# tjhladish/AbcSmc

Hardware: AMD Instinct MI355X
Metric: particles/sec per SMC generation (PLS+weight+resample), 1/2/4/8 GPU (higher is better)
Workload: dtype f64 (inputs, model, distances, proposals, results; pair sums of the weight stage: fp64 operands as three f16 limbs on the matrix pipe + f32 v_exp_f32, weights <= 5e-7 rel of the fp64 oracle, largest seen 3.1e-7); 1 GPU; configs[2]: synthetic 1M particles x 16 params x 32 metrics, PLS 8 components, full generation; particles_per_gpu=1000000, particles_total=1000000, metrics=32, params=16, pls_components=8, pred_prior_size=100000, prev_pred_prior_size=100000, next_set_size=1000000, noise=MULTIVARIATE, ncomp_chosen=8, pls_component_rule=wilcoxon, parallelism=row-sharded x1, launcher=single GPU

## Files before the change

### abcsmc_amd/csrc/abc_internal.h

```cpp
#pragma once
#include <hip/hip_runtime.h>
#include <stddef.h>
#include <stdint.h>
#include <stdio.h>
#include <stdlib.h>
#include <string.h>

#include "../../include/abcsmc_hip.h"

#define ABC_WAVE 64

inline const char* abc_diag_env(const char* name) {
    static const bool on = [] { const char* d = getenv("ABC_DIAG"); return d && d[0] == '1'; }();
    return on ? getenv(name) : nullptr;
}

struct abc_wx_words {
    int left;
    int vmax_lo, vmax_hi;
    int ncomp;
    int changed;
    int decided;
    int n_rest;
    int n_level;
// ... 192 lines not shown
                            double* stats, size_t n_set = 0);
int launch_pls_model(abc_ctx*, const double* stats, const double* obs, size_t M, size_t P, size_t A,
                     int rule, double* model, hipEvent_t done = nullptr);
int launch_simple_model(abc_ctx*, const double* stats, const double* obs, size_t M, size_t P,
                        double* model);
int launch_project_distance(abc_ctx*, const double* X, size_t n, size_t ldx, size_t M, size_t P,
                            size_t A, const double* model, int simple, double* dist);
size_t launch_project_scores(abc_ctx*, const double* X, size_t n, size_t ldx, size_t M, size_t P, size_t A, const double* model, double* S);
int launch_project_distance_scores(abc_ctx*, const double* X, size_t n, size_t ldx, size_t M, size_t P, size_t A, const double* model,
                                   double* dist, double* S, size_t sld, size_t row_test, hipEvent_t done);
int launch_distance_from_scores(abc_ctx*, const double* S, size_t n, size_t sld, size_t M, size_t P, size_t A, const double* model, double* dist);
size_t abc_targets_need(size_t N, size_t A, size_t B, size_t K, bool any_excl);
struct abc_tg_scores { const double* S; size_t sld; const double* O; int KCO; };
int launch_rank_targets(abc_ctx*, const double* X, size_t ldx, const double* Y, size_t ldy, size_t N, size_t M, size_t P,
                        const double* model, size_t A, const double* targets, size_t ldt, size_t B, const uint64_t* exclude,
                        bool any_excl, size_t K, uint64_t* idx, double* dist, double* post_mean, abc_tg_scores* keep = nullptr);
size_t abc_adjust_need(size_t N, size_t A, size_t P, size_t B, size_t K);
int launch_rank_targets_adjust(abc_ctx*, const double* X, size_t ldx, const double* Y, size_t ldy, size_t N, size_t M, size_t P,
                               const double* model, size_t A, const double* targets, size_t ldt, size_t B, const uint64_t* exclude,
                               bool any_excl, size_t K, int kernel, uint64_t* idx, double* dist, const abc_adjust_out* out,
                               struct abc_adj_keep* keep = nullptr);
size_t abc_path_need(size_t N, size_t A, size_t P, size_t B, size_t K, size_t T);
int launch_rank_targets_path(abc_ctx*, const double* X, size_t ldx, const double* Y, size_t ldy, size_t N, size_t M, size_t P,
                             const double* model, size_t A, const double* targets, size_t ldt, size_t B, const uint64_t* exclude,
                             bool any_excl, int kernel, uint64_t* idx, double* dist, const abc_path* path);
struct SmValues {
    int method;
    const uint64_t* idx;
    const double* Y;
    size_t ldy;
    const struct abc_adj_keep* adj;
    int A;
    int kernel;
    const double* V;
    size_t ldv;
    const double* w;
};
size_t abc_summary_need(size_t B, size_t K, size_t P);
int launch_summary(abc_ctx*, const SmValues& sv, size_t B, size_t K, size_t P, const abc_summary* sum);
int abc_summary_check_weights(abc_ctx*, const double* w, size_t K, const char* fn);
size_t abc_density_need(size_t B, size_t K, size_t P, size_t G);
int launch_density(abc_ctx*, const SmValues& sv, size_t B, size_t K, size_t P, const abc_density* dn, const char* fn);
struct DnSeg;
size_t abc_density_segs_need(size_t B, size_t K, size_t P);
int launch_density_segs(abc_ctx*, const SmValues& sv, size_t B, size_t K, size_t P, const abc_density* dn, const DnSeg** segs,
                        const char* fn);
size_t abc_joint_pairs(const abc_joint* jt, size_t P);
size_t abc_joint_need(size_t B, size_t K, size_t P, size_t G, size_t npairs);
int launch_joint(abc_ctx*, const SmValues& sv, size_t B, size_t K, size_t P, const abc_joint* jt, const char* fn);
size_t abc_draws_need(size_t B, size_t K, size_t P, int smooth);
int launch_draws(abc_ctx*, const SmValues& sv, size_t B, size_t K, size_t P, const abc_draws* dr, const char* fn);
int launch_select_smallest(abc_ctx*, const double* dist, size_t n, size_t K, uint64_t idx_base,
                           uint64_t* idx, double* dist_out, bool defer_check = false);
int abc_select_check(abc_ctx* ctx, int* failed);
int abc_select_check_queue(abc_ctx* ctx, int* slot);
int abc_select_check_done(abc_ctx* ctx, const int* slot);
inline size_t abc_kde_slices(size_t kn, size_t Kp, int PP) {
    if (kn == 0 || Kp == 0) return 1;
    size_t rows_per_slice = 24576 / (size_t)PP;
    if (rows_per_slice < 256) rows_per_slice = 256;
    size_t s = (Kp + rows_per_slice - 1) / rows_per_slice;
    const size_t rb = (kn + 255) / 256;
    if (s * rb < 4096) s = (4096 + rb - 1) / rb;
    size_t cap = ((size_t)64 << 20) / (8 * kn);
    if (cap < 8) cap = 8;
    if (s > cap) s = cap;
    if (s > Kp / 64) s = Kp / 64;
    if (s < 1) s = 1;
    if (s > 1024) s = 1024;
    return s;
}
int launch_merge_runs(abc_ctx* ctx, const double* key, const uint64_t* idx, int W, size_t len, double* okey, uint64_t* oidx,
                      uint64_t* osrc = nullptr);
int launch_sort_pairs(abc_ctx*, double* key, uint64_t* idx, size_t n);
int launch_select_begin(abc_ctx*, uint64_t K, long long* state, int* hist);
int launch_select_hist(abc_ctx*, const double* dist, size_t n, const long long* state, int pass, int* hist);
int launch_select_pick(abc_ctx*, long long* state, int pass, int* hist, uint64_t K);
int launch_select_count(abc_ctx*, const double* dist, size_t n, const long long* state, long long* counts);
int launch_select_compact(abc_ctx*, const double* dist, size_t n, const long long* state, uint64_t n_less,
                          uint64_t ties_take, uint64_t idx_base, uint64_t* idx_out, double* dist_out);
int abc_sort_u64_bytes(abc_ctx*, unsigned long long* key0, unsigned long long* val0, unsigned long long* key1,
                       unsigned long long* val1, size_t n, int byte_lo, int byte_hi);
struct abc_wx_shard {
    size_t nv_total;
    const double* nv_ranks;
    size_t nv_stride;
};
bool abc_wx_cascade_applies(size_t nv_total, size_t P, size_t A);
int launch_wilcoxon(abc_ctx*, const double* X, const double* Y, size_t n, size_t ldx, size_t ldy, size_t M, size_t P,
                    size_t A, size_t row_test, double* model, const abc_wx_shard* sh = nullptr, double* dec = nullptr,
                    int* changed_host = nullptr, int stop_at_max = 0);
int launch_wilcoxon_commit(abc_ctx*, double* model, size_t M, size_t P, size_t A, const double* dec, int with_hdr);
struct abc_wx_run;
struct abc_wx_scores_hook { int (*fn)(void* arg, double** S, size_t* sld); void* arg; };
int launch_wilcoxon_begin(abc_ctx*, const double* X, const double* Y, size_t n, size_t ldx, size_t ldy, size_t M, size_t P, size_t A,
                          size_t row_test, double* model, double* dec, int stop_at_max, abc_wx_run** out,
                          const abc_wx_scores_hook* scores = nullptr, int hold_level0 = 0, const abc_wx_shard* sh = nullptr);
int launch_wilcoxon_level0(abc_ctx*, abc_wx_run* run);
int launch_wilcoxon_finish(abc_ctx*, abc_wx_run* run, int* changed_host);
void launch_wilcoxon_abandon(abc_ctx*, abc_wx_run* run, hipStream_t its_stream);
int abc_comm_all_reduce(abc_ctx* ctx, void* buf, size_t count, int dtype);
int abc_comm_all_gather(abc_ctx* ctx, const void* send, void* recv, size_t bytes);
int abc_xbuf_reserve(abc_ctx* ctx, size_t bytes);
int abc_giveups_ensure(abc_ctx* ctx);
int launch_gather_rows(abc_ctx*, const double* Y, size_t n_local, size_t ldy, size_t P,
                       const uint64_t* idx, size_t K, uint64_t idx_base, double* theta, size_t ldt,
                       const int* sel_fail = nullptr, int* sel_fail_pin = nullptr, hipEvent_t done = nullptr);
#define ABC_INTERNAL_RETRY (-2147483647)
int launch_doubled_variance(abc_ctx*, const double* theta, size_t K, size_t P, double* dv);
int launch_theta_stats(abc_ctx*, const double* theta, size_t K, size_t P, double** stats_out);
struct abc_theta_fused {
    double* dv; double* L; int* spd; double* rows ; double* Lpad ;
    const double* model_hdr; double* hdr_pin; int* spd_pin;
};
int launch_post_tail(abc_ctx*, const double* theta, size_t K, size_t P, const double* stats, const abc_theta_fused* f);
int launch_dv_from_stats(abc_ctx*, const double* stats, size_t P, double* dv);
int launch_mvn_from_stats(abc_ctx*, const double* stats, size_t P, double* L, int* status_dev);
struct abc_wprev {
    void* wc ; double* b; double* hb; unsigned short* bt; unsigned* far_list;
    unsigned* tmin;
    size_t Kp, P, kn_max; int split, ready;
};
int launch_weights_prev(abc_ctx*, size_t P, size_t kn_max, const double* theta_prev, size_t Kp, const double* w_prev,
                        const double* dv_prev, abc_wprev* out, hipStream_t st);
int launch_weights_raw(abc_ctx*, const abc_prior* priors, const double* theta, size_t K, size_t P,
                       size_t k0, size_t kn, const double* theta_prev, size_t Kp,
                       const double* w_prev, const double* dv_prev, double* w_raw, const abc_wprev* prev = nullptr,
                       const double** sumsq_out = nullptr);
int abc_weights_prev_early(abc_ctx* ctx, size_t P, size_t kn_max, const double* theta_prev, size_t Kp, const double* w_prev,
                           const double* dv_prev, abc_wprev* out);
int launch_fill(abc_ctx*, double* w, size_t K, double v, hipStream_t st = nullptr);
int launch_normalize_l2(abc_ctx*, double* w, size_t K, double* host_mirror = nullptr, const double* sumsq_parts = nullptr);
static inline size_t abc_alias_pin_bytes(size_t K) { return K * (sizeof(double) * 3 + sizeof(uint32_t) * 3) + 2 * sizeof(uint32_t) + 16; }
int launch_mvn_setup(abc_ctx*, const double* theta, size_t K, size_t P, double* L, int* status_host,
                     int* status_dev);
int launch_resample(abc_ctx*, const abc_rng* rng, const double* w, size_t K, uint64_t i0, size_t n,
                    uint64_t* parent, int (*while_host_builds)(void*) = nullptr, void* hook_arg = nullptr,
                    bool uniform_weights = false, const uint32_t* raw_ready = nullptr, bool weights_on_host = false,
                    const volatile int* abort_flag = nullptr, bool parents_ready = false, int* alias_check_deferred = nullptr);
int abc_rng_streams_early(abc_ctx* ctx, const abc_rng* rng, uint64_t i0, size_t n, uint64_t* seeds, uint64_t seed_stream_offset,
                          uint32_t** raw, uint64_t* parent_uniform = nullptr, size_t K_uniform = 0);
int abc_rng_seeds_early(abc_ctx* ctx, const abc_rng* rng, uint64_t i0, size_t n, uint64_t* seeds, uint64_t seed_stream_offset);
int abc_side_fork(abc_ctx* ctx);
int abc_uniform_alias(abc_ctx* ctx, size_t K);
struct abc_perturb_prep { double* rows; int seeds_done; double* Lpad; };
int launch_perturb_prepare(abc_ctx*, const abc_rng* rng, const double* theta, size_t K, size_t P, uint64_t i0, size_t n,
                           uint64_t* seeds, uint64_t seed_stream_offset, abc_perturb_prep* prep, int multivariate = 0,
                           const double* L_or_dv = nullptr);
static inline int abc_perturb_pp(size_t P) {
    int PP = 2;
    while (PP < (int)P) PP *= 2;
    return (P > 64) ? (int)((P + 63) / 64 * 64) : PP;
}
int launch_perturb(abc_ctx*, const abc_rng* rng, const double* theta, size_t K, size_t P,
                   const abc_prior* priors, const uint64_t* parent, uint64_t i0, size_t n,
                   int multivariate, const double* L_or_dv, double* out, uint64_t* seeds,
                   uint64_t seed_stream_offset, const abc_perturb_prep* prep = nullptr);

struct abc_side_moments { abc_theta_fused out; double* stats; double* L; };
int abc_moments_on_side(abc_ctx* ctx, const double* theta, size_t K, size_t P, bool multivariate, double* L_io, double* dv,
                        int* spd_dev, const double* model_hdr, bool theta_ev_bound, const char* who, abc_side_moments* m);
int abc_normalize_for_resample(abc_ctx* ctx, double* w, size_t K, size_t Nn, const double* sumsq, bool* w_on_host);
struct abc_prep_arg {
    abc_ctx* ctx; const abc_rng* rng; const double* theta; const double* theta_stats; size_t K, P, Nn;
    uint64_t i0, seed_off; uint64_t* seeds; abc_perturb_prep* prep; double* L; int* spd_dev; double* dv; bool moments;
    const double* model_hdr; double* hdr_pin; int* spd_pin;
};
int abc_prep_hook(void* prep_arg);
int abc_alias_repair(abc_ctx* ctx, const abc_rng* rng_entry, const double* w, size_t K, uint64_t i0, size_t Nn, uint64_t seed_off,
                     uint64_t* parent, const double* theta, size_t P, const abc_prior* priors, int multivariate, const double* L_or_dv,
                     double* next, abc_perturb_prep* prep, bool giveups_to_snapshot);

int launch_perturb_reference(abc_ctx*, abc_rng* rng_after_draws, const double* theta, size_t K, size_t P, const abc_prior* priors,
                             const uint64_t* parent, size_t n, int multivariate, const double* L_or_dv, double* out,
                             uint64_t* seeds);

void abc_alias_preproc(size_t K, const double* w, double* F, uint32_t* A, double* E, uint32_t* smalls, uint32_t* bigs, bool knuth = true);

int launch_alias_build_dev(abc_ctx*, const double* w, size_t K, double* F, uint32_t* A, int* fail_dev, int* fail_pin,
                           const int** verdict_src = nullptr);
size_t abc_alias_dev_need(size_t K);
constexpr size_t ABC_ALIAS_DEV_MAX_K = (size_t)2 << 20;
constexpr size_t ABC_ALIAS_DEV_MIN_K = 20000;
constexpr size_t ABC_ALIAS_DEV_SMALL_K = 300000;

size_t abc_ws_need(size_t N, size_t M, size_t P, size_t A, size_t K, size_t Kp, size_t Nnext);
size_t abc_wx_need(size_t n_validation, size_t P, size_t A);
int abc_timing_flush(abc_ctx* ctx);
void abc_comm_release(abc_ctx* ctx);

void taus2_set(abc_rng* r, unsigned long seed);
uint32_t taus2_get(abc_rng* r);
void taus2_jump(abc_rng* r, uint64_t n);
```

### abcsmc_amd/csrc/alias_dev.hip

```cpp
#include <stdlib.h>

#include "abc_internal.h"

namespace {

typedef __int128 i128;
typedef unsigned __int128 u128;
typedef unsigned long long u64;

#ifndef ABC_AL_I
#define ABC_AL_I 4
#endif
#define ABC_AL_CAT2(a, b) a##b
#define ABC_AL_CAT(a, b) ABC_AL_CAT2(a, b)
#define ABC_AL_FN(name) ABC_AL_CAT(name##_i, ABC_AL_I)
constexpr int AL_T = 256;
constexpr int AL_I = ABC_AL_I;
constexpr int AL_B = AL_T * AL_I;
constexpr int AL_MAXBLK = 8192;
constexpr int AL_SUM_BITS = 44;

struct RMap { i128 t0, t1, b; int k; int pad_[3]; };

__device__ __forceinline__ i128 shl(i128 v, int s) { return (i128)((u128)v << s); }
// ... 65 lines not shown
    const int t = threadIdx.x, lane = t & 63, wave = t >> 6;
    RMap inc = mine;
#pragma unroll
    for (int d = 1; d < 64; d <<= 1) {
        const RMap up = shfl_up_map(inc, d);
        if (lane >= d) inc = compose(up, inc);
    }
    RMap exw = shfl_up_map(inc, 1);
    if (lane == 0) exw = rmap_identity();
    if (lane == 63) buf[0][wave] = inc;
    __syncthreads();
    RMap before = rmap_identity();
    for (int w = 0; w < wave; w++) before = compose(before, buf[0][w]);
    __syncthreads();
    *excl = compose(before, exw);
    return compose(before, inc);
}
__device__ __forceinline__ RMap prefix_of_blocks(const RMap* __restrict__ agg, int nb, RMap (*buf)[AL_T]) {
    const int t = threadIdx.x;
    const int per = (nb + AL_T - 1) / AL_T;
    RMap m = rmap_identity();
    for (int j = 0; j < per; j++) { const int b = t * per + j; if (b < nb) m = compose(m, agg[b]); }
    RMap ex;
    (void)block_scan_maps(m, buf, &ex);
    __shared__ RMap s_tot;
    if (t == AL_T - 1) s_tot = compose(ex, m);
    __syncthreads();
    const RMap r = s_tot;
    __syncthreads();
    return r;
}

struct AlHead {
    double approx_total;
    double total;
    int e0_sum;
    int e0;
    unsigned ns, nb;
    unsigned nsteps;
    int fail;
    i128 MEAN;
};

__device__ __forceinline__ void al_fail(AlHead* h) { h->fail = 1; }

__device__ __forceinline__ double block_sum_d(double v, double* sm) {
#pragma unroll
    for (int o = 32; o >= 1; o >>= 1) v += __shfl_xor(v, o, 64);
    __syncthreads();
    if ((threadIdx.x & 63) == 0) sm[threadIdx.x >> 6] = v;
    __syncthreads();
    return (sm[0] + sm[1]) + (sm[2] + sm[3]);
}
__global__ __launch_bounds__(AL_T) void k_al_bsum(const double* __restrict__ w, size_t K, double* __restrict__ bsum, AlHead* __restrict__ head,
                                                  int force_fail) {
    __shared__ double sm[4];
    const size_t base = (size_t)blockIdx.x * AL_B + (size_t)threadIdx.x * AL_I;
    double s = 0.0;
    bool bad = false;
#pragma unroll
    for (int j = 0; j < AL_I; j++) if (base + j < K) { const double x = w[base + j]; s += x; bad = bad || !(x >= 0.0) || !(x < 1.0e300); }
    const double bs = block_sum_d(bad ? (double)NAN : s, sm);
    if (threadIdx.x == 0) bsum[blockIdx.x] = bs;
    if (blockIdx.x == 0 && threadIdx.x == 0) {
        head->approx_total = 0.0; head->total = 0.0; head->e0_sum = 0; head->e0 = 0; head->ns = 0; head->nb = 0; head->nsteps = 0;
        head->fail = force_fail; head->MEAN = 0;
    }
}

__device__ __forceinline__ void approx_prefix(const double* __restrict__ bsum, int nblk, int b, double* sm, double* before, double* all) {
    double pb = 0.0, pa = 0.0;
    for (int j = threadIdx.x; j < nblk; j += AL_T) { const double v = bsum[j]; pa += v; if (j < b) pb += v; }
    *before = block_sum_d(pb, sm);
    *all = block_sum_d(pa, sm);
}

struct SumCtx { double before, all; int e0; };
__device__ __forceinline__ RMap sum_map(double x, double s_approx, int e0, AlHead* head) {
    if (x == 0.0) return rmap_identity();
    int ex;
    (void)frexp(s_approx, &ex);
    int k = ex - e0 - 53;
    if (k < 0) k = 0;
    bool sticky = false;
    const i128 c = to_grid(x, e0, &sticky);
    if (k == 0 && sticky) al_fail(head);
    return rne_map(k, c, sticky);
}
__device__ __forceinline__ double block_excl_prefix_d(double mine, double* sd ) {
    const int t = threadIdx.x;
    sd[t] = mine;
    __syncthreads();
    for (int step = 1; step < AL_T; step <<= 1) {
        const double a = (t >= step) ? sd[t - step] : 0.0;
        __syncthreads();
        sd[t] += a;
        __syncthreads();
    }
    const double ex = t ? sd[t - 1] : 0.0;
    __syncthreads();
    return ex;
}

__global__ __launch_bounds__(AL_T) void k_al_sum_reduce(const double* __restrict__ w, size_t K, const double* __restrict__ bsum, int nblk,
                                                        RMap* __restrict__ agg, RMap* __restrict__ tpre, AlHead* __restrict__ head) {
    __shared__ RMap buf[2][AL_T];
    __shared__ double sd[AL_T];
    __shared__ double sm[4];
    double before, all;
    approx_prefix(bsum, nblk, blockIdx.x, sm, &before, &all);
    int etot;
    (void)frexp(all, &etot);
    const int e0 = etot - 53 - AL_SUM_BITS;
    if (!(all > 0.0) || !(all < 1.0e300)) { if (threadIdx.x == 0) al_fail(head); }
// ... 310 lines not shown
    const RMap ex = tpre[(size_t)blockIdx.x * AL_T + threadIdx.x];
    const int e0 = head->e0;
    i128 v = rapply(ex, rapply(pre, a.VI[0]));
    bool ok = true;
    double prev = from_grid(v, e0, &ok);
#pragma unroll
    for (int j = 0; j < AL_I; j++) {
        const size_t t = base + j;
        if (t >= n) break;
        v = rapply(mj[j], v);
        const double c = from_grid(v, e0, &ok);
        const uint32_t s = rec[j].idx;
        unsigned jcur;
        bool below, at_last_small;
        if (!(s & AL_HAND)) {
            const unsigned ii = s;
            jcur = a.jof[ii];
            const uint32_t sm = a.sidx[ii];
            const double es = a.E[sm];
            if (prev - (mean - es) != c) ok = false;
            below = (a.z[jcur - 1] == ii + 1);
            at_last_small = (ii + 1 == ns);
            A[sm] = a.bidx[jcur - 1];
            F[sm] = dK * es;
        } else {
            const unsigned j0 = (s & ~AL_HAND) + 1;
            jcur = j0 + 1;
            const uint32_t bo = a.bidx[j0 - 1], bn = a.bidx[j0];
            const double dd = mean - prev;
            if (a.E[bn] - dd != c) ok = false;
            const unsigned zz = a.z[j0 - 1];
            below = (a.z[j0] == zz);
            at_last_small = (zz == ns);
            A[bo] = bn;
            F[bo] = dK * prev;
        }
        if (!(jcur == nb && at_last_small)) {
            if (below) { if (!(c < mean)) ok = false; }
            else if (!(c > mean)) ok = false;
        }
        prev = c;
    }
    if (!ok) al_fail(head);
    (void)last_block;
}
__global__ void k_al_flag(const AlHead* __restrict__ head, int* __restrict__ fail_out, int* __restrict__ fail_pin) {
    if (threadIdx.x == 0) { *fail_out = head->fail; if (fail_pin) *fail_pin = head->fail; }
}

}

#if ABC_AL_I == 4
int launch_alias_build_dev_i2(abc_ctx* ctx, const double* w, size_t K, double* F, uint32_t* A, int* fail_dev, int* fail_pin,
                              const int** verdict_src);
int launch_alias_build_dev_i4(abc_ctx* ctx, const double* w, size_t K, double* F, uint32_t* A, int* fail_dev, int* fail_pin,
                              const int** verdict_src);
size_t abc_alias_dev_need(size_t K) {
    constexpr size_t B = AL_T * 2;
    const size_t nblk = (K + B - 1) / B + 1, nblk2 = (2 * K + B - 1) / B + 1;
    return K * (8 + 4 + 4 + 8 + 16 + 16 + 16 + 4 + 4 + 64) + nblk * (8 + 4 + 64 + 64) + nblk2 * 64 * (AL_T + 1) + sizeof(AlHead) + 64 * 256;
}
int launch_alias_build_dev(abc_ctx* ctx, const double* w, size_t K, double* F, uint32_t* A, int* fail_dev, int* fail_pin,
                           const int** verdict_src) {
    if (K <= ABC_ALIAS_DEV_SMALL_K) return launch_alias_build_dev_i2(ctx, w, K, F, A, fail_dev, fail_pin, verdict_src);
    return launch_alias_build_dev_i4(ctx, w, K, F, A, fail_dev, fail_pin, verdict_src);
}
#endif

int ABC_AL_FN(launch_alias_build_dev)(abc_ctx* ctx, const double* w, size_t K, double* F, uint32_t* A, int* fail_dev, int* fail_pin,
                                      const int** verdict_src) {
    if (K == 0 || K > (size_t)AL_MAXBLK * AL_B / 2) ABC_FAIL(ctx, ABC_ERR_UNSUPPORTED, "device alias build: K = %zu", K);
    const int nblk = (int)((K + AL_B - 1) / AL_B), nblk2 = (int)((2 * K + AL_B - 1) / AL_B);
    AlHead* head = (AlHead*)abc_ws_alloc(ctx, sizeof(AlHead));
    double* bsum = (double*)abc_ws_alloc(ctx, (size_t)nblk * 8);
    RMap* agg = (RMap*)abc_ws_alloc(ctx, (size_t)(nblk2 > nblk ? nblk2 : nblk) * sizeof(RMap));
    RMap* tpre = (RMap*)abc_ws_alloc(ctx, (size_t)(nblk2 > nblk ? nblk2 : nblk) * AL_T * sizeof(RMap));
    double* E = (double*)abc_ws_alloc(ctx, K * 8);
    unsigned* cnt = (unsigned*)abc_ws_alloc(ctx, (size_t)nblk * 4);
    uint32_t* sidx = (uint32_t*)abc_ws_alloc(ctx, K * 4);
    uint32_t* bidx = (uint32_t*)abc_ws_alloc(ctx, K * 4);
    u64* dI = (u64*)abc_ws_alloc(ctx, K * 8);
    i128* VI = (i128*)abc_ws_alloc(ctx, K * 16);
    i128* D = (i128*)abc_ws_alloc(ctx, K * 16);
    i128* X = (i128*)abc_ws_alloc(ctx, K * 16);
    i128* bs = (i128*)abc_ws_alloc(ctx, (size_t)4 * nblk * 16);
    i128* Dc = bs ? bs + (size_t)2 * nblk : nullptr;
    i128* Xc = bs ? bs + (size_t)3 * nblk : nullptr;
    uint32_t* z = (uint32_t*)abc_ws_alloc(ctx, K * 4);
    uint32_t* jof = (uint32_t*)abc_ws_alloc(ctx, K * 4);
    StepRec* step = (StepRec*)abc_ws_alloc(ctx, 2 * K * sizeof(StepRec));
    if (!head || !bsum || !agg || !tpre || !E || !cnt || !sidx || !bidx || !dI || !VI || !D || !X || !bs || !z || !jof || !step)
        ABC_FAIL(ctx, ABC_ERR_NOMEM, "device alias build: workspace exhausted");
    const double mean = 1.0 / (double)K, dK = (double)K;
    hipStream_t st = ctx->stream;
    const int force_fail = abc_diag_env("ABC_ALIAS_FORCE_FAIL") ? 1 : 0;
    hipLaunchKernelGGL(k_al_bsum, dim3(nblk), dim3(AL_T), 0, st, w, K, bsum, head, force_fail);
    hipLaunchKernelGGL(k_al_sum_reduce, dim3(nblk), dim3(AL_T), 0, st, w, K, (const double*)bsum, nblk, agg, tpre, head);
    hipLaunchKernelGGL(k_al_sum_apply, dim3(nblk), dim3(AL_T), 0, st, w, K, (const double*)bsum, nblk, (const RMap*)agg, (const RMap*)tpre, head);
    hipLaunchKernelGGL(k_al_classify, dim3(nblk), dim3(AL_T), 0, st, w, K, mean, head, E, cnt, F, A);
    hipLaunchKernelGGL(k_al_lists, dim3(nblk), dim3(AL_T), 0, st, (const double*)E, K, mean, (const unsigned*)cnt, nblk, head, sidx, dI, bidx, VI);
    hipLaunchKernelGGL(k_al_psum_reduce, dim3(nblk, 2), dim3(AL_T), 0, st, (const u64*)dI, (const i128*)VI, (const AlHead*)head, bs, nblk);
    hipLaunchKernelGGL(k_al_psum_apply, dim3(nblk, 2), dim3(AL_T), 0, st, (const u64*)dI, (const i128*)VI, (const AlHead*)head,
                       (const i128*)bs, nblk, D, X, Dc, Xc);
    hipLaunchKernelGGL(k_al_structure, dim3((unsigned)((K + AL_T - 1) / AL_T)), dim3(AL_T), 0, st, (const i128*)D, (const i128*)X, (const i128*)Dc, (const i128*)Xc, (const u64*)dI, (const i128*)VI, head, z, jof, step);
    ServeArgs a = {E, sidx, bidx, dI, VI, D, X, z, jof, step};
    hipLaunchKernelGGL(k_al_serve_reduce, dim3(nblk2), dim3(AL_T), 0, st, a, (const AlHead*)head, agg, tpre);
    hipLaunchKernelGGL(k_al_serve_apply, dim3(nblk2), dim3(AL_T), 0, st, a, head, (const RMap*)agg, (const RMap*)tpre, mean, dK, F, A, fail_dev, fail_pin);
    if (verdict_src) *verdict_src = &head->fail;
    else hipLaunchKernelGGL(k_al_flag, dim3(1), dim3(64), 0, st, (const AlHead*)head, fail_dev, fail_pin);
    ABC_HIP(ctx, hipGetLastError());
    return ABC_OK;
}
```

### abcsmc_amd/csrc/api.hip

```cpp
#include <math.h>
#include <stdlib.h>

#include <new>
#include <vector>

#include "abc_internal.h"
#include "adjust_dev.h"

int abc_ws_reserve(abc_ctx* ctx, size_t bytes) {
    bytes = abc_align(bytes, 1 << 20);
    if (bytes > ctx->ws_bytes) {
        ABC_HIP(ctx, hipStreamSynchronize(ctx->stream));
        if (ctx->ws) { ABC_HIP(ctx, hipFree(ctx->ws)); ctx->ws = nullptr; ctx->ws_bytes = 0; }
        ABC_HIP(ctx, hipMalloc((void**)&ctx->ws, bytes));
        ctx->ws_bytes = bytes;
    }
    ctx->ws_off = 0;
    static const char* poison = abc_diag_env("ABC_WS_POISON");
    if (poison && ctx->ws) ABC_HIP(ctx, hipMemsetAsync(ctx->ws, (int)strtol(poison, nullptr, 16), ctx->ws_bytes, ctx->stream));
    return ABC_OK;
}
void* abc_ws_alloc(abc_ctx* ctx, size_t bytes) {
    const size_t off = abc_align(ctx->ws_off, 256);
    if (off + bytes > ctx->ws_bytes) return nullptr;
// ... 538 lines not shown
    double* wx_dec = nullptr;
    abc_wx_run* wx_run = nullptr;
    struct WxGuard {
        abc_ctx* c; abc_wx_run** r;
        ~WxGuard() { if (*r) { launch_wilcoxon_abandon(c, *r, c->wx_stream); *r = nullptr; } }
    } wx_guard = {ctx, &wx_run};
    bool projected = false;
    const double* scores_all = nullptr;
    if (wx_spec) {
        wx_dec = (double*)abc_ws_alloc(ctx, (P + 1) * 8);
        if (!wx_dec) ABC_FAIL(ctx, ABC_ERR_NOMEM, "generation: workspace exhausted");
        ABC_HIP(ctx, hipStreamWaitEvent(ctx->wx_stream, ctx->ev_wx_fork, 0));
        struct ScoresArg { abc_ctx* ctx; hipStream_t main; const double* X; size_t N, M, P, A, ntrain; const double* model; double* dist; double* S_all; }
            sarg = {ctx, ctx->stream, io->X, N, M, P, A, (size_t)ntrain, model, dist, nullptr};
        if (!(N & 1)) sarg.S_all = (double*)abc_ws_alloc(ctx, N * A * 8);
        abc_wx_scores_hook hook = {
            [](void* a, double** S, size_t* sld) -> int {
                ScoresArg* q = (ScoresArg*)a;
                abc_ctx* c = q->ctx;
                hipStream_t wx = c->stream;
                double* S_half = nullptr;
                if (!q->S_all) {
                    S_half = (double*)abc_ws_alloc(c, (q->N - q->ntrain) * q->A * 8);
                    if (!S_half) { snprintf(c->err, sizeof(c->err), "generation: workspace exhausted"); return ABC_ERR_NOMEM; }
                }
                int rc;
                {
                    StreamScope on_main(c, q->main);
                    rc = q->S_all ? launch_project_distance_scores(c, q->X, q->N, q->N, q->M, q->P, q->A, q->model, q->dist, q->S_all, q->N, 0, c->ev_wx_scores)
                                  : launch_project_distance_scores(c, q->X, q->N, q->N, q->M, q->P, q->A, q->model, q->dist, S_half, q->N - q->ntrain, q->ntrain,
                                                                   c->ev_wx_scores);
                }
                if (rc == 0 && hipStreamWaitEvent(wx, c->ev_wx_scores, 0) != hipSuccess) rc = ABC_ERR_HIP;
                if (rc == 0) {
                    q->dist = nullptr;
                    *S = q->S_all ? q->S_all + q->ntrain : S_half;
                    *sld = q->S_all ? q->N : q->N - q->ntrain;
                } else if (rc == 1)
                    q->S_all = nullptr;
                return rc;
            },
            &sarg};
        {
            StreamScope on_wx(ctx, ctx->wx_stream);
            ABC_TRY(launch_wilcoxon_begin(ctx, io->X, io->Y, N, N, N, M, P, A, (size_t)ntrain, model, wx_dec, 1, &wx_run, &hook,
                                          1));
        }
        projected = sarg.dist == nullptr;
        scores_all = projected ? sarg.S_all : nullptr;
    } else if (wx_rule)
        ABC_TRY(launch_wilcoxon(ctx, io->X, io->Y, N, N, N, M, P, A, (size_t)ntrain, model));
    if (!projected) ABC_TRY(launch_project_distance(ctx, io->X, N, N, M, simple ? Pstat : P, A, model, simple, dist));
    if (K == 0) return ABC_OK;
    ABC_TRY(launch_select_smallest(ctx, dist, N, K, 0, io->idx, io->dist, io->w != nullptr));
    if (!simple && ncomp_host && !io->w) {
        double hdr[4];
        ABC_HIP(ctx, hipMemcpyAsync(hdr, model, sizeof(hdr), hipMemcpyDeviceToHost, ctx->stream));
        ABC_HIP(ctx, hipStreamSynchronize(ctx->stream));
        *ncomp_host = (int32_t)hdr[0];
    }
    if (!io->w) return ABC_OK;

    double* theta = io->theta ? io->theta : (double*)abc_ws_alloc(ctx, K * P * 8);
    if (!theta) ABC_FAIL(ctx, ABC_ERR_NOMEM, "generation: workspace exhausted");
    int* pfail_early = &ctx->status_pin->gather_sel_fail;
    *pfail_early = 0;
    volatile unsigned* pgaveup = &ctx->status_pin->giveup_flag;
    *pgaveup = 0u;
    double* const hdr_pin = ctx->status_pin->model_hdr;
    int* const spd_pin = &ctx->status_pin->spd;
    hdr_pin[0] = 0.0; *spd_pin = 0;
    bool status_early = false;
    bool bins_deferred = ctx->sel_bins_ran && ctx->sel_fail_dev && !ctx->sel_force_radix;
    ctx->side_early_waited = false;
    if (wprev.ready) {
        ABC_HIP(ctx, hipStreamWaitEvent(ctx->stream, ctx->ev_prev, 0));
        ctx->side_early_waited = true;
    }
    const bool defer_moments = Nn && P <= 64 && K >= 2;
    const bool moments_side_planned = defer_moments && !uniform_w && ctx->side && ctx->noise_mode != ABC_NOISE_REFERENCE_STREAM;
    if (moments_side_planned && !ctx->ev_theta) {
        ABC_HIP(ctx, hipEventCreateWithFlags(&ctx->ev_theta, abc_xstream_event_flags()));
        ABC_HIP(ctx, hipEventCreateWithFlags(&ctx->ev_moments, abc_xstream_event_flags()));
    }
    const bool theta_ev_bound = moments_side_planned;
    ABC_TRY(launch_gather_rows(ctx, io->Y, N, N, P, io->idx, K, 0, theta, K, bins_deferred ? ctx->sel_fail_dev : nullptr, pfail_early,
                               theta_ev_bound ? ctx->ev_theta : nullptr));
    if (wx_run) {
        StreamScope on_wx(ctx, ctx->wx_stream);
        ABC_TRY(launch_wilcoxon_level0(ctx, wx_run));
    }
    bool wx_tail_pending = false;
    if (wx_spec) {
        int changed = 2, rc;
        {
            StreamScope on_wx(ctx, ctx->wx_stream);
            rc = launch_wilcoxon_finish(ctx, wx_run, &changed);
            wx_run = nullptr;
            if (rc == ABC_OK && hipEventRecord(ctx->ev_wx_done, ctx->wx_stream) != hipSuccess) rc = ABC_ERR_HIP;
        }
        if (rc == ABC_INTERNAL_RETRY) {
            ABC_HIP(ctx, hipStreamSynchronize(ctx->wx_stream));
            ABC_HIP(ctx, hipStreamSynchronize(ctx->stream));
            rc = launch_wilcoxon(ctx, io->X, io->Y, N, N, N, M, P, A, (size_t)ntrain, model);
            changed = 2;
        }
        if (rc != ABC_OK) { if (!ctx->err[0]) snprintf(ctx->err, sizeof(ctx->err), "generation: the component rule's reduction failed"); return rc; }
        if (changed == 1) {
            ABC_HIP(ctx, hipStreamWaitEvent(ctx->stream, ctx->ev_wx_done, 0));
            ABC_TRY(launch_wilcoxon_commit(ctx, model, M, P, A, wx_dec, 1));
        } else if (changed == 0) {
            StreamScope on_wx(ctx, ctx->wx_stream);
            ABC_TRY(launch_wilcoxon_commit(ctx, model, M, P, A, wx_dec, 0));
            wx_tail_pending = true;
        }
        if (changed) {
            ctx->wx_moved_counts++;
            pfail_early = &ctx->status_pin->repeat_sel_fail;
            *pfail_early = 0;
            if (scores_all) ABC_TRY(launch_distance_from_scores(ctx, scores_all, N, N, M, P, A, model, dist));
            else ABC_TRY(launch_project_distance(ctx, io->X, N, N, M, P, A, model, 0, dist));
            ABC_TRY(launch_select_smallest(ctx, dist, N, K, 0, io->idx, io->dist, true));
            bins_deferred = ctx->sel_bins_ran && ctx->sel_fail_dev && !ctx->sel_force_radix;
            ABC_TRY(launch_gather_rows(ctx, io->Y, N, N, P, io->idx, K, 0, theta, K, bins_deferred ? ctx->sel_fail_dev : nullptr, pfail_early,
                                       theta_ev_bound ? ctx->ev_theta : nullptr));
        }
    }
    auto repeat_with_radix = [&]() -> int {
        ABC_HIP(ctx, hipStreamSynchronize(ctx->stream));
        if (ctx->side) ABC_HIP(ctx, hipStreamSynchronize(ctx->side));
        if (ctx->wx_stream) ABC_HIP(ctx, hipStreamSynchronize(ctx->wx_stream));
        if (ctx->giveups_dev)
            ABC_HIP(ctx, hipMemcpyAsync(ctx->giveups_dev, ctx->giveups_dev + 1, sizeof(unsigned long long), hipMemcpyDeviceToDevice, ctx->stream));
        ctx->sel_bins_ran = false;
        ctx->ws_off = ws_entry;
        if (rng) *rng = rng_entry;
        ctx->generation_repeats++;
        const bool radix0 = ctx->sel_force_radix;
        ctx->sel_force_radix = true;
        const int rc = generation_core(ctx, cfg, io, rng, ncomp_host, simple, model_out);
        ctx->sel_force_radix = radix0;
        return rc;
    };
    double* dv = io->dv ? io->dv : (double*)abc_ws_alloc(ctx, P * 8);
    double* theta_stats = nullptr;
    if (defer_moments) {
    } else if (P <= 64 && K >= 2) {
        StageTimer tm(ctx, ST_GATHER_DV);
        ABC_TRY(launch_theta_stats(ctx, theta, K, P, &theta_stats));
        ABC_TRY(launch_dv_from_stats(ctx, theta_stats, P, dv));
    } else {
        ABC_TRY(launch_doubled_variance(ctx, theta, K, P, dv));
    }
    bool w_on_host = false;
    if (Kp == 0 || !io->theta_prev) {
        if (!filled_early) ABC_TRY(launch_fill(ctx, io->w, K, 1.0 / (double)K));
    } else {
        if (wprev.ready && !ctx->side_early_waited) ABC_HIP(ctx, hipStreamWaitEvent(ctx->stream, ctx->ev_prev, 0));
        const double* sumsq = nullptr;
        ABC_TRY(launch_weights_raw(ctx, io->priors, theta, K, P, 0, K, io->theta_prev, Kp, io->w_prev, io->dv_prev,
                                   io->w, &wprev, &sumsq));
        ABC_TRY(abc_normalize_for_resample(ctx, io->w, K, Nn, sumsq, &w_on_host));
    }
    abc_side_moments side = {};
    bool moments_on_side = false, seeds_waited = false;
    if (moments_side_planned) {
        ABC_TRY(abc_moments_on_side(ctx, theta, K, P, cfg->multivariate != 0, io->L, dv, spd_dev, simple ? nullptr : model, theta_ev_bound,
                                    "generation", &side));
        theta_stats = side.stats;
        moments_on_side = status_early = true;
    }
    int spd = 0;
    bool have_spd = false;
    int alias_deferred = 0;
    uint64_t* parent_used = nullptr;
    double* L_used = nullptr;
    abc_perturb_prep prep_used = {nullptr, 0, nullptr};
    if (Nn) {
        uint64_t* parent = parent_early ? parent_early : (io->parent ? io->parent : (uint64_t*)abc_ws_alloc(ctx, Nn * 8));
        if (!parent) ABC_FAIL(ctx, ABC_ERR_NOMEM, "generation: workspace exhausted");
        double* L = nullptr;
        if (cfg->multivariate) {
            L = side.L ? side.L : (io->L ? io->L : (double*)abc_ws_alloc(ctx, P * P * 8));
            have_spd = true;
        }
        abc_perturb_prep prep = {side.out.rows, (early && io->seeds) ? 1 : 0, side.out.Lpad};
        if (moments_on_side) { ABC_HIP(ctx, hipStreamWaitEvent(ctx->stream, ctx->ev_moments, 0)); seeds_waited = true; }
        const bool hook_moments = defer_moments && !moments_on_side;
        abc_prep_arg pa = {ctx, rng, theta, theta_stats, K, P, Nn, 0, Nn, io->seeds, &prep, moments_on_side ? nullptr : L, spd_dev, dv,
                           hook_moments, nullptr, nullptr, nullptr};
        if (hook_moments) {
            pa.model_hdr = simple ? nullptr : model; pa.hdr_pin = hdr_pin; pa.spd_pin = L ? spd_pin : nullptr;
            status_early = true;
        }
        {
            const int rc = launch_resample(ctx, rng, io->w, K, 0, Nn, parent, abc_prep_hook, &pa, uniform_w, raw_early, w_on_host,
                                           bins_deferred ? pfail_early : nullptr, parent_early != nullptr,
                                           ctx->noise_mode == ABC_NOISE_REFERENCE_STREAM ? nullptr : &alias_deferred);
            if (rc == ABC_INTERNAL_RETRY) return repeat_with_radix();
            ABC_TRY(rc);
        }
        if (ctx->noise_mode == ABC_NOISE_REFERENCE_STREAM) {
            taus2_jump(rng, (uint64_t)Nn);
            ABC_TRY(launch_perturb_reference(ctx, rng, theta, K, P, io->priors, parent, Nn, cfg->multivariate,
                                             cfg->multivariate ? L : dv, io->next, io->seeds));
        } else {
            ABC_TRY(launch_perturb(ctx, rng, theta, K, P, io->priors, parent, 0, Nn, cfg->multivariate,
                                   cfg->multivariate ? L : dv, io->next, io->seeds, Nn, &prep));
            parent_used = parent; L_used = L; prep_used = prep;
            taus2_jump(rng, 2 * (uint64_t)Nn);
        }
    }
    {
        double* hdr = ctx->status_pin->model_hdr;
        int* pspd = &ctx->status_pin->spd;
        int* pfail = &ctx->status_pin->sel_fail;
        if (!status_early) { hdr[0] = 0.0; *pspd = 0; }
        *pfail = 0;
        if (seeds_late && !seeds_waited) ABC_HIP(ctx, hipStreamWaitEvent(ctx->stream, ctx->ev_side, 0));
        const int* fail_dev = (ctx->sel_bins_ran && ctx->sel_fail_dev) ? (const int*)ctx->sel_fail_dev : nullptr;
        unsigned long long* pgive = &ctx->status_pin->giveups;
        *pgive = 0;
        if (!status_early) {
            hipLaunchKernelGGL(k_status_words, dim3(1), dim3(64), 0, ctx->stream, simple ? (const double*)nullptr : (const double*)model,
                               have_spd ? (const int*)spd_dev : (const int*)nullptr, fail_dev, (const unsigned long long*)ctx->giveups_dev, hdr, pspd,
                               pfail, pgive);
            ABC_HIP(ctx, hipGetLastError());
        }
        ctx->side_early_waited = false;
        ABC_HIP(ctx, hipStreamSynchronize(ctx->stream));
        if (wx_tail_pending) ABC_HIP(ctx, hipStreamSynchronize(ctx->wx_stream));
        if (status_early) {
            *pfail = fail_dev ? *(volatile int*)pfail_early : 0;
        } else {
            ctx->giveups_dev_known = *(volatile unsigned long long*)pgive;
        }
        if (ncomp_host) *ncomp_host = (int32_t)hdr[0];
        spd = *pspd;
        const int failed = abc_select_check_done(ctx, pfail);
        if (failed && !ctx->sel_force_radix) return repeat_with_radix();
        if (alias_deferred && *(volatile int*)&ctx->status_pin->alias_fail && parent_used) {
            ABC_TRY(abc_alias_repair(ctx, &rng_entry, io->w, K, 0, Nn, Nn, parent_used, theta, P, io->priors, cfg->multivariate,
                                     cfg->multivariate ? L_used : dv, io->next, &prep_used, true));
        }
    }
    if (ctx->timing && ctx->nev > 128) ABC_TRY(abc_timing_flush(ctx));
    if (spd) ABC_FAIL(ctx, ABC_ERR_NOT_SPD, "covariance of the selected particles is not positive definite");
    {
        if (status_early) {
            if (*pgaveup && ctx->giveups_dev) {
                unsigned long long now = 0;
                ABC_HIP(ctx, hipMemcpyAsync(&now, ctx->giveups_dev, sizeof(now), hipMemcpyDeviceToHost, ctx->stream));
                ABC_HIP(ctx, hipStreamSynchronize(ctx->stream));
                ctx->giveups_dev_known = now;
            }
            *(volatile unsigned long long*)&ctx->status_pin->giveups = ctx->giveups_dev_known;
        }
        const unsigned long long gv = *(volatile unsigned long long*)&ctx->status_pin->giveups + ctx->giveups_host;
        const unsigned long long before = ctx->giveups_seen;
        ctx->giveups_seen = gv;
        ctx->giveups_last_call = (Nn && gv > before) ? gv - before : 0ull;
// ... 897 lines not shown
```

### abcsmc_amd/csrc/resample.hip

```cpp
#include <chrono>
#include <vector>

#include "abc_internal.h"
#include "philox_dev.h"
#include "refstream_host.h"

static inline uint32_t taus_c1(uint32_t s) { return ((s & 4294967294u) << 12) ^ (((s << 13) ^ s) >> 19); }
static inline uint32_t taus_c2(uint32_t s) { return ((s & 4294967288u) << 4) ^ (((s << 2) ^ s) >> 25); }
static inline uint32_t taus_c3(uint32_t s) { return ((s & 4294967280u) << 17) ^ (((s << 3) ^ s) >> 11); }

uint32_t taus2_get(abc_rng* r) {
    r->s1 = taus_c1(r->s1); r->s2 = taus_c2(r->s2); r->s3 = taus_c3(r->s3);
    return r->s1 ^ r->s2 ^ r->s3;
}
void taus2_set(abc_rng* r, unsigned long seed) {
    uint32_t s = (uint32_t)(seed & 0xffffffffUL);
    if (s == 0) s = 1;
    r->s1 = 69069u * s;     if (r->s1 < 2) r->s1 += 2;
    r->s2 = 69069u * r->s1; if (r->s2 < 8) r->s2 += 8;
    r->s3 = 69069u * r->s2; if (r->s3 < 16) r->s3 += 16;
    for (int i = 0; i < 6; i++) taus2_get(r);
}

struct BitMat { uint32_t col[32]; };
// ... 29 lines not shown
    for (int k = 0; k < 64; k++)
        if ((n >> k) & 1ull) {
            r->s1 = bm_apply(tab[k][0], r->s1); r->s2 = bm_apply(tab[k][1], r->s2); r->s3 = bm_apply(tab[k][2], r->s3);
        }
}

namespace {

constexpr int RUN = 64;
constexpr int RUN_LOG2 = 6;

__device__ __forceinline__ uint32_t d_apply(const uint32_t* __restrict__ col, uint32_t v) {
    uint32_t y = 0;
#pragma unroll
    for (int i = 0; i < 32; i++) y ^= (uint32_t)(-(int32_t)((v >> i) & 1u)) & col[i];
    return y;
}

__global__ __launch_bounds__(256) void k_taus_stream(abc_rng base, size_t n, const uint32_t* __restrict__ jt,
                                                     uint32_t* __restrict__ out) {
    __shared__ uint32_t sjt[24 * 96];
    for (int e = threadIdx.x; e < 24 * 96; e += blockDim.x) sjt[e] = jt[e];
    __syncthreads();
    const size_t t = (size_t)blockIdx.x * blockDim.x + threadIdx.x;
    const size_t first = t * RUN;
    if (first >= n) return;
    uint32_t s1 = base.s1, s2 = base.s2, s3 = base.s3;
    for (int k = 0; k < 32; k++)
        if ((t >> k) & 1) {
            const uint32_t* m = (k < 24) ? sjt + k * 96 : jt + (size_t)k * 96;
            s1 = d_apply(m, s1); s2 = d_apply(m + 32, s2); s3 = d_apply(m + 64, s3);
        }
    const size_t last = (first + RUN < n) ? first + RUN : n;
    for (size_t i = first; i < last; i++) {
        s1 = ((s1 & 4294967294u) << 12) ^ (((s1 << 13) ^ s1) >> 19);
        s2 = ((s2 & 4294967288u) << 4) ^ (((s2 << 2) ^ s2) >> 25);
        s3 = ((s3 & 4294967280u) << 17) ^ (((s3 << 3) ^ s3) >> 11);
        out[i] = s1 ^ s2 ^ s3;
    }
}

__global__ __launch_bounds__(256) void k_alias_draw(const uint32_t* __restrict__ raw, size_t n,
                                                    const double* __restrict__ F, const uint32_t* __restrict__ A,
                                                    size_t K, unsigned long long* __restrict__ parent,
                                                    const int* __restrict__ verdict_src = nullptr, int* __restrict__ verdict_dev = nullptr,
                                                    int* __restrict__ verdict_pin = nullptr) {
    const size_t i = (size_t)blockIdx.x * 256 + threadIdx.x;
    if (i == 0 && verdict_src) { const int v = *verdict_src; *verdict_dev = v; *verdict_pin = v; }
    if (i >= n) return;
    const double u = (double)raw[i] / 4294967296.0;
    const size_t c = (size_t)(u * (double)K);
    const double f = (F[c] + (double)c) / (double)K;
    parent[i] = (f == 1.0) ? c : ((u < f) ? c : (size_t)A[c]);
}

__global__ __launch_bounds__(256) void k_widen(const uint32_t* __restrict__ raw, size_t n,
                                               unsigned long long* __restrict__ out) {
    const size_t i = (size_t)blockIdx.x * 256 + threadIdx.x;
    if (i < n) out[i] = raw[i];
}


__device__ __forceinline__ double d_recast(const abc_prior& pr, double v) {
    return (pr.kind == ABC_PRIOR_UNIF_INT) ? round(v) : v;
}
__device__ __forceinline__ bool d_valid(const abc_prior& pr, double v) {
    if (pr.kind == ABC_PRIOR_GAUSS) {
        const double u = (v - pr.a) / fabs(pr.b);
        if (u * u < 1400.0 && fabs(pr.b) < 1e10) return true;
        return (1.0 / (sqrt(2.0 * M_PI) * fabs(pr.b))) * exp(-u * u / 2.0) != 0.0;
    }
    if (pr.kind == ABC_PRIOR_UNIF_INT) return (v == round(v)) && (pr.a <= v) && (v <= pr.b);
    return (pr.a <= v) && (v <= pr.b);
}
__device__ __forceinline__ double recast_valid(const abc_prior& pr, double inv_sigma, double v, bool& ok) {
    const int kind = __builtin_amdgcn_readfirstlane(pr.kind);
    if (kind == ABC_PRIOR_GAUSS) {
        const double t = (v - pr.a) * inv_sigma;
        if (!(t * t < 1399.0 && inv_sigma != 0.0)) ok = ok && d_valid(pr, v);
        return v;
    }
    if (kind == ABC_PRIOR_UNIF_INT) v = round(v);
    ok = ok && (pr.a <= v) && (v <= pr.b);
    return v;
}
__device__ __forceinline__ double d_prior_mean(const abc_prior& pr) {
    return (pr.kind == ABC_PRIOR_GAUSS) ? pr.a : (pr.b + pr.a) / 2.0;
}

__device__ __forceinline__ void note_giveup(unsigned long long* __restrict__ g) {
    atomicAdd(g, 1ull);
    unsigned* f = (unsigned*)(size_t)g[2];
    if (f) *f = 1u;
}

constexpr unsigned MVN_MAX_TRIES = 1u << 14;

template <int PP>
__global__ __launch_bounds__(256) void k_theta_rows(const double* __restrict__ theta, size_t K, int P,
                                                    double* __restrict__ rows, const double* __restrict__ L,
                                                    double* __restrict__ Lpad) {
    __shared__ double t[PP][65];
    if (blockIdx.x == 0 && L) {
        for (int e = threadIdx.x; e < PP * PP; e += 256) {
            const int a = e % PP, b = e / PP;
            Lpad[e] = (a < P && b < P && b <= a) ? L[a + (size_t)P * b] : 0.0;
// ... 12 lines not shown
}

template <int PP, int A0>
__device__ __forceinline__ void mv_cols4(const double* __restrict__ l, const double (&z)[4], double (&x)[PP]) {
#pragma unroll
    for (int a = A0; a < PP; a++) {
        x[a] = fma(l[a], z[0], x[a]); x[a] = fma(l[PP + a], z[1], x[a]);
        x[a] = fma(l[2 * PP + a], z[2], x[a]); x[a] = fma(l[3 * PP + a], z[3], x[a]);
    }
}
template <int PP>
__device__ __forceinline__ void mv_noise(const double* __restrict__ sL, unsigned long long gi, unsigned attempt, uint32_t k0,
                                         uint32_t k1, double (&x)[PP], int P) {
    const int nq = (P + 3) / 4;
#pragma unroll
    for (int a = 0; a < PP; a++) x[a] = 0.0;
    if constexpr (PP < 4) {
        U4 c; c.x = (uint32_t)gi; c.y = (uint32_t)(gi >> 32); c.z = attempt; c.w = 0u;
        double z[4];
        normal4(philox(c, k0, k1), z);
#pragma unroll
        for (int b = 0; b < PP; b++)
#pragma unroll
            for (int a = 0; a < PP; a++) x[a] = fma(sL[PP * b + a], z[b], x[a]);
    } else {
#pragma unroll 1
        for (int qd = 0; qd < nq; qd++) {
            U4 c; c.x = (uint32_t)gi; c.y = (uint32_t)(gi >> 32); c.z = attempt; c.w = (uint32_t)qd;
            double z[4];
            normal4(philox(c, k0, k1), z);
            const double* l = sL + PP * (4 * qd);
            if constexpr (PP >= 32) {
                const int g = (4 * qd) / (PP / 4);
                if (g == 0) mv_cols4<PP, 0>(l, z, x);
                else if (g == 1) mv_cols4<PP, PP / 4>(l, z, x);
                else if (g == 2) mv_cols4<PP, PP / 2>(l, z, x);
                else mv_cols4<PP, 3 * (PP / 4)>(l, z, x);
            } else {
                if (qd < (PP / 4 + 1) / 2) mv_cols4<PP, 0>(l, z, x);
                else mv_cols4<PP, PP / 2>(l, z, x);
            }
        }
    }
}
__device__ __forceinline__ double indep_noise(double sigma, unsigned long long gi, unsigned attempt, int p, uint32_t k0, uint32_t k1) {
    U4 c; c.x = (uint32_t)gi; c.y = (uint32_t)(gi >> 32); c.z = attempt; c.w = 0x80000000u | (uint32_t)p;
    double z[4];
    normal4(philox(c, k0, k1), z);
    return sigma * z[0];
}
template <int PP, bool MV>
__global__ __launch_bounds__(256, (MV && PP <= 16) ? 3 : (PP <= 16 ? 2 : 1)) void k_perturb(abc_rng key, const double* __restrict__ theta, size_t K, int P,
                                                 const abc_prior* __restrict__ priors,
                                                 const unsigned long long* __restrict__ parent,
                                                 unsigned long long i0, size_t n,
                                                 const double* __restrict__ L_or_dv , double* __restrict__ out,
                                                 unsigned long long* __restrict__ giveups) {
    __shared__ double sS[PP];
    __shared__ abc_prior sp[PP];
    __shared__ double sinv[PP];
    if (!MV) for (int p = threadIdx.x; p < PP; p += 256) sS[p] = (p < P) ? sqrt(L_or_dv[p]) : 0.0;
    for (int p = threadIdx.x; p < PP; p += 256) {
        abc_prior q; q.kind = ABC_PRIOR_UNIF_REAL; q.pad_ = 0; q.a = -1e300; q.b = 1e300;
        sp[p] = (p < P) ? priors[p] : q;
        sinv[p] = (p < P && priors[p].kind == ABC_PRIOR_GAUSS && fabs(priors[p].b) < 1e10 && fabs(priors[p].b) > 1e-300) ? 1.0 / fabs(priors[p].b) : 0.0;
    }
    __syncthreads();
    const size_t i = (size_t)blockIdx.x * 256 + threadIdx.x;
    if (i >= n) return;
    {
    const unsigned long long gi = i0 + i;
    const double* mrow = theta + (size_t)parent[i] * PP;
    const uint32_t k0 = key.s1 ^ 0x5bd1e995u, k1 = key.s2 ^ (key.s3 * 0x9E3779B1u);
    double x[PP];
    if (MV) {
        for (unsigned attempt = 0; attempt < MVN_MAX_TRIES; attempt++) {
            mv_noise<PP>(L_or_dv, gi, attempt, k0, k1, x, P);
            bool ok = true;
            asm volatile("" ::: "memory");
#pragma unroll
            for (int a = 0; a < PP; a += 2) {
                if (PP > 32 && a >= P) continue;
                const double2 m = *reinterpret_cast<const double2*>(mrow + a);
                x[a] = recast_valid(sp[a], sinv[a], x[a] + m.x, ok);
                x[a + 1] = recast_valid(sp[a + 1], sinv[a + 1], x[a + 1] + m.y, ok);
            }
            if (ok) break;
            if (attempt + 1 == MVN_MAX_TRIES) {
#pragma unroll
                for (int a = 0; a < PP; a++) x[a] = mrow[a];
                note_giveup(giveups);
            }
        }
    } else {
#pragma unroll
        for (int p = 0; p < PP; p++) {
            x[p] = 0.0;
            if (p < P) {
                const double m = mrow[p];
                double v = 0.0; bool ok = false;
                asm volatile("" ::: "memory");
                for (unsigned attempt = 0; attempt < 1000 && !ok; attempt++) {
                    v = d_recast(sp[p], indep_noise(sS[p], gi, attempt, p, k0, k1) + m);
                    ok = d_valid(sp[p], v);
                }
                x[p] = ok ? v : d_prior_mean(sp[p]);
                if (!ok) note_giveup(giveups);
            }
        }
    }
#pragma unroll
    for (int p = 0; p < PP; p++)
        if (p < P) __builtin_nontemporal_store(x[p], &out[i + n * (size_t)p]);
    }
}

template <int PP, bool MV>
__global__ __launch_bounds__(256) void k_perturb_stream(abc_rng key, const double* __restrict__ theta, size_t K, int P,
                                                        const abc_prior* __restrict__ priors,
                                                        const unsigned long long* __restrict__ parent,
                                                        unsigned long long i0, size_t n,
                                                        const double* __restrict__ L_or_dv, double* __restrict__ out,
                                                        unsigned long long* __restrict__ giveups) {
    extern __shared__ double smem[];
    double* sL = smem;
    abc_prior* sp = reinterpret_cast<abc_prior*>(smem + (MV ? PP * PP : PP));
    if (MV) {
        for (int e = threadIdx.x; e < PP * PP; e += 256) {
            const int a = e % PP, b = e / PP;
            sL[e] = (a < P && b < P && b <= a) ? L_or_dv[a + (size_t)P * b] : 0.0;
        }
    } else {
        for (int e = threadIdx.x; e < PP; e += 256) sL[e] = (e < P) ? sqrt(L_or_dv[e]) : 0.0;
    }
    for (int p = threadIdx.x; p < PP; p += 256) {
        abc_prior q; q.kind = ABC_PRIOR_UNIF_REAL; q.pad_ = 0; q.a = -1e300; q.b = 1e300;
        sp[p] = (p < P) ? priors[p] : q;
    }
    __syncthreads();
    const size_t i = (size_t)blockIdx.x * 256 + threadIdx.x;
    if (i >= n) return;
    const unsigned long long gi = i0 + i;
    const double* mu = theta + (size_t)parent[i] * PP;
    const uint32_t k0 = key.s1 ^ 0x5bd1e995u, k1 = key.s2 ^ (key.s3 * 0x9E3779B1u);
    if (MV) {
        bool ok = false;
        for (unsigned attempt = 0; attempt < MVN_MAX_TRIES && !ok; attempt++) {
            double x[PP];
#pragma unroll
            for (int a = 0; a < PP; a++) x[a] = 0.0;
#pragma unroll 1
            for (int qd = 0; qd < PP / 4; qd++) {
                U4 c; c.x = (uint32_t)gi; c.y = (uint32_t)(gi >> 32); c.z = attempt; c.w = (uint32_t)qd;
                double z[4];
                normal4(philox(c, k0, k1), z);
                const double* l = sL + PP * (4 * qd);
#pragma unroll
                for (int a = 0; a < PP; a++) {
                    x[a] = fma(l[a], z[0], x[a]); x[a] = fma(l[PP + a], z[1], x[a]);
                    x[a] = fma(l[2 * PP + a], z[2], x[a]); x[a] = fma(l[3 * PP + a], z[3], x[a]);
                }
            }
            ok = true;
#pragma unroll
            for (int a = 0; a < PP; a++) {
                if (a < P) {
                    const double v = d_recast(sp[a], x[a] + mu[a]);
                    out[i + n * (size_t)a] = v;
                    ok = ok && d_valid(sp[a], v);
                }
            }
        }
        if (!ok) {
            for (int p = 0; p < P; p++) out[i + n * (size_t)p] = mu[p];
            note_giveup(giveups);
        }
    } else {
        for (int p = 0; p < P; p++) {
            const double m = mu[p];
            double v = 0.0; bool ok = false;
            for (unsigned attempt = 0; attempt < 1000 && !ok; attempt++) {
                U4 c; c.x = (uint32_t)gi; c.y = (uint32_t)(gi >> 32); c.z = attempt; c.w = 0x80000000u | (uint32_t)p;
                double z[4];
                normal4(philox(c, k0, k1), z);
                v = d_recast(sp[p], sL[p] * z[0] + m);
                ok = d_valid(sp[p], v);
            }
            out[i + n * (size_t)p] = ok ? v : d_prior_mean(sp[p]);
            if (!ok) note_giveup(giveups);
        }
    }
}

__global__ __launch_bounds__(256) void k_theta_rows_gen(const double* __restrict__ theta, size_t K, int P, int PP,
                                                        double* __restrict__ rows, const double* __restrict__ L,
                                                        double* __restrict__ Lpad) {
    if (blockIdx.x == 0 && L) {
        for (size_t e = threadIdx.x; e < (size_t)PP * PP; e += 256) {
            const int a = (int)(e % PP), b = (int)(e / PP);
            Lpad[e] = (a < P && b < P && b <= a) ? L[a + (size_t)P * b] : 0.0;
        }
    }
    const size_t tot = K * (size_t)PP;
    for (size_t e = (size_t)blockIdx.x * 256 + threadIdx.x; e < tot; e += (size_t)gridDim.x * 256) {
        const size_t r = e / PP;
        const int p = (int)(e % PP);
        rows[e] = (p < P) ? theta[r + K * (size_t)p] : 0.0;
    }
}
template <bool MV>
__global__ __launch_bounds__(256) void k_perturb_gen(abc_rng key, const double* __restrict__ rows, int P, int PP,
                                                     const abc_prior* __restrict__ priors,
                                                     const unsigned long long* __restrict__ parent,
                                                     unsigned long long i0, size_t n, const double* __restrict__ L_or_dv,
                                                     double* __restrict__ out, unsigned long long* __restrict__ giveups) {
    extern __shared__ abc_prior spg[];
    for (int p = threadIdx.x; p < P; p += 256) spg[p] = priors[p];
    __syncthreads();
    const size_t i = (size_t)blockIdx.x * 256 + threadIdx.x;
    if (i >= n) return;
    const unsigned long long gi = i0 + i;
    const double* mu = rows + (size_t)parent[i] * PP;
    const uint32_t k0 = key.s1 ^ 0x5bd1e995u, k1 = key.s2 ^ (key.s3 * 0x9E3779B1u);
    if (MV) {
        bool ok = false;
        for (unsigned attempt = 0; attempt < MVN_MAX_TRIES && !ok; attempt++) {
            ok = true;
            for (int c = 0; c < PP / 64; c++) {
                double x[64];
#pragma unroll
                for (int a = 0; a < 64; a++) x[a] = 0.0;
                for (int qd = 0; qd < 16 * (c + 1); qd++) {
                    U4 cn; cn.x = (uint32_t)gi; cn.y = (uint32_t)(gi >> 32); cn.z = attempt; cn.w = (uint32_t)qd;
                    double z[4];
                    normal4(philox(cn, k0, k1), z);
                    const double* l = L_or_dv + (size_t)PP * (4 * qd) + 64 * c;
#pragma unroll
                    for (int a = 0; a < 64; a++) {
                        x[a] = fma(l[a], z[0], x[a]); x[a] = fma(l[PP + a], z[1], x[a]);
                        x[a] = fma(l[2 * (size_t)PP + a], z[2], x[a]); x[a] = fma(l[3 * (size_t)PP + a], z[3], x[a]);
                    }
                }
#pragma unroll
                for (int a = 0; a < 64; a++) {
                    const int p = 64 * c + a;
                    if (p < P) {
                        const double v = d_recast(spg[p], x[a] + mu[p]);
                        out[i + n * (size_t)p] = v;
                        ok = ok && d_valid(spg[p], v);
                    }
                }
            }
        }
        if (!ok) {
            for (int p = 0; p < P; p++) out[i + n * (size_t)p] = mu[p];
            note_giveup(giveups);
        }
    } else {
        for (int p = 0; p < P; p++) {
            const double m = mu[p], sg = sqrt(L_or_dv[p]);
            double v = 0.0; bool ok = false;
            for (unsigned attempt = 0; attempt < 1000 && !ok; attempt++) {
                v = d_recast(spg[p], indep_noise(sg, gi, attempt, p, k0, k1) + m);
                ok = d_valid(spg[p], v);
            }
            out[i + n * (size_t)p] = ok ? v : d_prior_mean(spg[p]);
            if (!ok) note_giveup(giveups);
        }
    }
}

int ensure_jump_tab(abc_ctx* ctx) {
    if (ctx->jump_tab) return ABC_OK;
    const BitMat(*tab)[3] = taus_pow2();
    std::vector<uint32_t> h(32 * 96);
// ... 62 lines not shown
        ABC_HIP(ctx, hipEventCreateWithFlags(&ctx->ev_side, abc_xstream_event_flags()));
    }
    if (hipStreamQuery(ctx->stream) != hipSuccess) {
        (void)hipGetLastError();
        ABC_HIP(ctx, hipEventRecord(ctx->ev_fork, ctx->stream));
        ABC_HIP(ctx, hipStreamWaitEvent(ctx->side, ctx->ev_fork, 0));
    }
    ctx->side_forked = true;
    return ABC_OK;
}

int abc_rng_streams_early(abc_ctx* ctx, const abc_rng* rng, uint64_t i0, size_t n, uint64_t* seeds, uint64_t seed_stream_offset,
                          uint32_t** raw_out, uint64_t* parent_uniform, size_t K_uniform) {
    *raw_out = nullptr;
    if (n == 0) return ABC_OK;
    uint32_t* raw = (uint32_t*)abc_ws_alloc(ctx, n * sizeof(uint32_t));
    if (!raw) ABC_FAIL(ctx, ABC_ERR_NOMEM, "resample: workspace exhausted");
    ABC_TRY(ensure_jump_tab(ctx));
    if (!ctx->side_forked) ABC_TRY(abc_side_fork(ctx));
    abc_rng base = *rng;
    taus2_jump(&base, i0);
    ABC_TRY(taus_stream(ctx, base, n, raw, ctx->side));
    if (parent_uniform && ctx->ualias_K == K_uniform && K_uniform) {
        hipLaunchKernelGGL(k_alias_draw, dim3((unsigned)((n + 255) / 256)), dim3(256), 0, ctx->side, raw, n, ctx->ualias_F,
                           ctx->ualias_A, K_uniform, (unsigned long long*)parent_uniform);
        ABC_HIP(ctx, hipGetLastError());
    }
    if (seeds) ABC_TRY(launch_seeds(ctx, rng, i0, n, seeds, seed_stream_offset, ctx->side));
    ABC_HIP(ctx, hipEventRecord(ctx->ev_side, ctx->side));
    *raw_out = raw;
    return ABC_OK;
}

int abc_rng_seeds_early(abc_ctx* ctx, const abc_rng* rng, uint64_t i0, size_t n, uint64_t* seeds, uint64_t seed_stream_offset) {
    if (n == 0 || !seeds) return ABC_OK;
    if (!ctx->side_forked) ABC_TRY(abc_side_fork(ctx));
    ABC_TRY(launch_seeds(ctx, rng, i0, n, seeds, seed_stream_offset, ctx->side));
    ABC_HIP(ctx, hipEventRecord(ctx->ev_side, ctx->side));
    return ABC_OK;
}

int abc_weights_prev_early(abc_ctx* ctx, size_t P, size_t kn_max, const double* theta_prev, size_t Kp, const double* w_prev,
                           const double* dv_prev, abc_wprev* out) {
    if (!ctx->side_forked) ABC_TRY(abc_side_fork(ctx));
    if (!ctx->ev_prev) ABC_HIP(ctx, hipEventCreateWithFlags(&ctx->ev_prev, abc_xstream_event_flags()));
    ABC_TRY(launch_weights_prev(ctx, P, kn_max, theta_prev, Kp, w_prev, dv_prev, out, ctx->side));
    ABC_HIP(ctx, hipEventRecord(ctx->ev_prev, ctx->side));
    return ABC_OK;
}

int launch_resample(abc_ctx* ctx, const abc_rng* rng, const double* w, size_t K, uint64_t i0, size_t n,
                    uint64_t* parent, int (*while_host_builds)(void*), void* hook_arg, bool uniform_weights,
                    const uint32_t* raw_ready, bool weights_on_host, const volatile int* abort_flag, bool parents_ready,
                    int* alias_check_deferred) {
    if (alias_check_deferred) *alias_check_deferred = 0;
    bool wait_side = raw_ready != nullptr;
    if (n == 0) return ABC_OK;
    if (K == 0 || K > 0xffffffffull) ABC_FAIL(ctx, ABC_ERR_INVALID, "resample: K = %zu", K);
    if (uniform_weights) {
        ABC_TRY(abc_uniform_alias(ctx, K));
        uint32_t* raw = const_cast<uint32_t*>(raw_ready);
        if (!raw) raw = (uint32_t*)abc_ws_alloc(ctx, n * sizeof(uint32_t));
        if (!raw) ABC_FAIL(ctx, ABC_ERR_NOMEM, "resample: workspace exhausted");
        abc_rng base = *rng;
        taus2_jump(&base, i0);
        StageTimer tm(ctx, ST_RESAMPLE);
        if (raw_ready) ABC_HIP(ctx, hipStreamWaitEvent(ctx->stream, ctx->ev_side, 0));
        else ABC_TRY(taus_stream(ctx, base, n, raw));
        if (while_host_builds) ABC_TRY(while_host_builds(hook_arg));
        if (!(parents_ready && raw_ready)) {
            hipLaunchKernelGGL(k_alias_draw, dim3((unsigned)((n + 255) / 256)), dim3(256), 0, ctx->stream, raw, n, ctx->ualias_F,
                               ctx->ualias_A, K, (unsigned long long*)parent);
            ABC_HIP(ctx, hipGetLastError());
        }
        return ABC_OK;
    }
    if (ctx->alias_K < K) {
        ABC_HIP(ctx, hipStreamSynchronize(ctx->stream));
        if (ctx->alias_F) { (void)hipFree(ctx->alias_F); ctx->alias_F = nullptr; ctx->alias_A = nullptr; }
        ABC_HIP(ctx, hipMalloc((void**)&ctx->alias_F, K * (sizeof(double) + sizeof(uint32_t))));
        ctx->alias_K = K;
    }
    ctx->alias_A = (uint32_t*)(ctx->alias_F + K);
    if (ctx->alias_mode == ABC_ALIAS_DEVICE && K >= ABC_ALIAS_DEV_MIN_K && K <= ABC_ALIAS_DEV_MAX_K && ctx->ws_off + abc_alias_dev_need(K) <= ctx->ws_bytes) {
        if (!ctx->alias_fail_dev) ABC_HIP(ctx, hipMalloc((void**)&ctx->alias_fail_dev, sizeof(int)));
        int* fail_pin = &ctx->status_pin->alias_fail;
        *fail_pin = 0;
        const int* verdict = nullptr;
        uint32_t* raw = const_cast<uint32_t*>(raw_ready);
        if (!raw) raw = (uint32_t*)abc_ws_alloc(ctx, n * sizeof(uint32_t));
        if (!raw) ABC_FAIL(ctx, ABC_ERR_NOMEM, "resample: workspace exhausted");
        abc_rng base = *rng;
        taus2_jump(&base, i0);
        if (raw_ready) {
            if (!ctx->side_early_waited) ABC_HIP(ctx, hipStreamWaitEvent(ctx->stream, ctx->ev_side, 0));
        } else {
            StageTimer tm(ctx, ST_RESAMPLE);
            ABC_TRY(taus_stream(ctx, base, n, raw));
        }
        {
            StageTimer tm(ctx, ST_ALIAS_HOST);
            ABC_TRY(launch_alias_build_dev(ctx, w, K, ctx->alias_F, ctx->alias_A, ctx->alias_fail_dev, fail_pin, &verdict));
        }
        ctx->alias_dev_builds++;
        if (while_host_builds) ABC_TRY(while_host_builds(hook_arg));
        {
            StageTimer tm(ctx, ST_RESAMPLE);
            hipLaunchKernelGGL(k_alias_draw, dim3((unsigned)((n + 255) / 256)), dim3(256), 0, ctx->stream, raw, n, ctx->alias_F,
                               ctx->alias_A, K, (unsigned long long*)parent, verdict, ctx->alias_fail_dev, fail_pin);
            ABC_HIP(ctx, hipGetLastError());
        }
        if (alias_check_deferred) { *alias_check_deferred = 1; return ABC_OK; }
        ABC_HIP(ctx, hipStreamSynchronize(ctx->stream));
        if (!*fail_pin) return ABC_OK;
        ctx->alias_dev_fallbacks++;
        while_host_builds = nullptr;
        raw_ready = raw;
        wait_side = false;
        weights_on_host = false;
    }
    ABC_TRY(abc_pin_reserve(ctx, abc_alias_pin_bytes(K)));
    double* hw = (double*)ctx->pin;
    double* hF = hw + K;
    uint32_t* hA = (uint32_t*)(hF + K);
    double* hE = (double*)(((uintptr_t)(hA + K) + 7) & ~(uintptr_t)7);
    uint32_t* hS = (uint32_t*)(hE + K);
    uint32_t* hB = hS + K + 1;
    if (!weights_on_host)
        ABC_HIP(ctx, hipMemcpyAsync(hw, w, K * sizeof(double), hipMemcpyDeviceToHost, ctx->stream));
    if (!ctx->ev_copy) ABC_HIP(ctx, hipEventCreateWithFlags(&ctx->ev_copy, hipEventDisableTiming));
    ABC_HIP(ctx, hipEventRecord(ctx->ev_copy, ctx->stream));
    uint32_t* raw = const_cast<uint32_t*>(raw_ready);
    if (!raw) raw = (uint32_t*)abc_ws_alloc(ctx, n * sizeof(uint32_t));
    if (!raw) ABC_FAIL(ctx, ABC_ERR_NOMEM, "resample: workspace exhausted");
    abc_rng base = *rng;
    taus2_jump(&base, i0);
    if (raw_ready) {
        if (wait_side && !ctx->side_early_waited) ABC_HIP(ctx, hipStreamWaitEvent(ctx->stream, ctx->ev_side, 0));
    } else {
        StageTimer tm(ctx, ST_RESAMPLE);
        ABC_TRY(taus_stream(ctx, base, n, raw));
    }
    if (while_host_builds) ABC_TRY(while_host_builds(hook_arg));
    ABC_HIP(ctx, hipEventSynchronize(ctx->ev_copy));
    if (abort_flag && *abort_flag) return ABC_INTERNAL_RETRY;
    {
        const auto t0 = std::chrono::steady_clock::now();
        abc_alias_preproc(K, hw, hF, hA, hE, hS, hB, false);
        if (ctx->timing) {
            ctx->stage_host_ms[ST_ALIAS_HOST] += std::chrono::duration<double, std::milli>(std::chrono::steady_clock::now() - t0).count();
            ctx->stage_cnt[ST_ALIAS_HOST] += 1;
        }
    }
    StageTimer tm(ctx, ST_RESAMPLE);
    ABC_HIP(ctx, hipMemcpyAsync(ctx->alias_F, hF, K * (sizeof(double) + sizeof(uint32_t)), hipMemcpyHostToDevice, ctx->stream));
    hipLaunchKernelGGL(k_alias_draw, dim3((unsigned)((n + 255) / 256)), dim3(256), 0, ctx->stream, raw, n, ctx->alias_F,
                       ctx->alias_A, K, (unsigned long long*)parent);
    ABC_HIP(ctx, hipGetLastError());
    return ABC_OK;
// ... 9 lines not shown
        ABC_HIP(ctx, hipGetLastError());
        return ABC_OK;
    }
    switch (PP) {
        case 2: hipLaunchKernelGGL((k_theta_rows<2>), dim3(grid), dim3(256), 0, ctx->stream, theta, K, (int)P, rows, L, Lpad); break;
        case 4: hipLaunchKernelGGL((k_theta_rows<4>), dim3(grid), dim3(256), 0, ctx->stream, theta, K, (int)P, rows, L, Lpad); break;
        case 8: hipLaunchKernelGGL((k_theta_rows<8>), dim3(grid), dim3(256), 0, ctx->stream, theta, K, (int)P, rows, L, Lpad); break;
        case 16: hipLaunchKernelGGL((k_theta_rows<16>), dim3(grid), dim3(256), 0, ctx->stream, theta, K, (int)P, rows, L, Lpad); break;
        case 32: hipLaunchKernelGGL((k_theta_rows<32>), dim3(grid), dim3(256), 0, ctx->stream, theta, K, (int)P, rows, L, Lpad); break;
        default: hipLaunchKernelGGL((k_theta_rows<64>), dim3(grid), dim3(256), 0, ctx->stream, theta, K, (int)P, rows, L, Lpad); break;
    }
    ABC_HIP(ctx, hipGetLastError());
    return ABC_OK;
}
static int launch_seeds(abc_ctx* ctx, const abc_rng* rng, uint64_t i0, size_t n, uint64_t* seeds, uint64_t seed_stream_offset,
                        hipStream_t st) {
    uint32_t* raw = (uint32_t*)abc_ws_alloc(ctx, n * sizeof(uint32_t));
    if (!raw) ABC_FAIL(ctx, ABC_ERR_NOMEM, "perturb: workspace exhausted");
    abc_rng base = *rng;
    taus2_jump(&base, seed_stream_offset + i0);
    ABC_TRY(taus_stream(ctx, base, n, raw, st));
    hipLaunchKernelGGL(k_widen, dim3((unsigned)((n + 255) / 256)), dim3(256), 0, st ? st : ctx->stream, raw, n, (unsigned long long*)seeds);
    ABC_HIP(ctx, hipGetLastError());
    return ABC_OK;
}
int launch_perturb_prepare(abc_ctx* ctx, const abc_rng* rng, const double* theta, size_t K, size_t P, uint64_t i0, size_t n,
                           uint64_t* seeds, uint64_t seed_stream_offset, abc_perturb_prep* prep, int multivariate,
                           const double* L_or_dv) {
    if (n == 0) { prep->rows = nullptr; prep->Lpad = nullptr; return ABC_OK; }
    const int PP = abc_perturb_pp(P);
    StageTimer tm(ctx, ST_PERTURB);
    if (!prep->rows) {
        double* rows = (double*)abc_ws_alloc(ctx, K * (size_t)PP * sizeof(double));
        double* Lpad = (multivariate && L_or_dv) ? (double*)abc_ws_alloc(ctx, (size_t)PP * PP * sizeof(double)) : nullptr;
        if (!rows || (multivariate && L_or_dv && !Lpad)) ABC_FAIL(ctx, ABC_ERR_NOMEM, "perturb: workspace exhausted");
        ABC_TRY(launch_theta_rows(ctx, theta, K, P, PP, rows, Lpad ? L_or_dv : nullptr, Lpad));
        prep->rows = rows;
        prep->Lpad = Lpad;
    }
    if (seeds && !prep->seeds_done) { ABC_TRY(launch_seeds(ctx, rng, i0, n, seeds, seed_stream_offset, nullptr)); prep->seeds_done = 1; }
    return ABC_OK;
}

int abc_giveups_ensure(abc_ctx* ctx) {
    if (ctx->giveups_dev) return ABC_OK;
    ABC_HIP(ctx, hipMalloc((void**)&ctx->giveups_dev, 3 * sizeof(unsigned long long)));
    const unsigned long long init[3] = {0ull, 0ull, (unsigned long long)(size_t)&ctx->status_pin->giveup_flag};
    ABC_HIP(ctx, hipMemcpy(ctx->giveups_dev, init, sizeof(init), hipMemcpyHostToDevice));
    return ABC_OK;
}

int launch_perturb(abc_ctx* ctx, const abc_rng* rng, const double* theta, size_t K, size_t P, const abc_prior* priors,
                   const uint64_t* parent, uint64_t i0, size_t n, int multivariate, const double* L_or_dv, double* out,
                   uint64_t* seeds, uint64_t seed_stream_offset, const abc_perturb_prep* prep) {
    if (n == 0) return ABC_OK;
    int PP = 2;
    while (PP < (int)P) PP *= 2;
    if (P > 64) PP = (int)((P + 63) / 64 * 64);
    ABC_TRY(abc_giveups_ensure(ctx));
    StageTimer tm(ctx, ST_PERTURB);
    const unsigned blocks = (unsigned)((n + 255) / 256);
    double* rows = (prep && prep->rows) ? prep->rows : (double*)abc_ws_alloc(ctx, K * (size_t)PP * sizeof(double));
    if (!rows) ABC_FAIL(ctx, ABC_ERR_NOMEM, "perturb: workspace exhausted");
    const double* Lpad = (prep && prep->rows) ? prep->Lpad : nullptr;
    if (!(prep && prep->rows)) {
        const bool need_lp = multivariate != 0;
        double* lp = need_lp ? (double*)abc_ws_alloc(ctx, (size_t)PP * PP * sizeof(double)) : nullptr;
        if (need_lp && !lp) ABC_FAIL(ctx, ABC_ERR_NOMEM, "perturb: workspace exhausted");
        ABC_TRY(launch_theta_rows(ctx, theta, K, P, PP, rows, lp ? L_or_dv : nullptr, lp));
        Lpad = lp;
    }
    theta = rows;
    if (multivariate && !Lpad) ABC_FAIL(ctx, ABC_ERR_INVALID, "perturb: the padded factor was not prepared");
    if (PP > 64) {
        const size_t lds = P * sizeof(abc_prior);
        if (multivariate)
            hipLaunchKernelGGL((k_perturb_gen<true>), dim3(blocks), dim3(256), lds, ctx->stream, *rng, theta, (int)P, PP, priors,
                               (const unsigned long long*)parent, (unsigned long long)i0, n, Lpad, out, ctx->giveups_dev);
        else
            hipLaunchKernelGGL((k_perturb_gen<false>), dim3(blocks), dim3(256), lds, ctx->stream, *rng, theta, (int)P, PP, priors,
                               (const unsigned long long*)parent, (unsigned long long)i0, n, L_or_dv, out, ctx->giveups_dev);
        ABC_HIP(ctx, hipGetLastError());
        if (seeds && !(prep && prep->seeds_done)) ABC_TRY(launch_seeds(ctx, rng, i0, n, seeds, seed_stream_offset, nullptr));
        return ABC_OK;
    }
#define LAUNCH_PT(PPV)                                                                                                 \
    do {                                                                                                               \
        if (multivariate)                                                                                              \
            hipLaunchKernelGGL((k_perturb<PPV, true>), dim3(blocks), dim3(256), 0, ctx->stream, *rng, theta, K, (int)P, \
                               priors, (const unsigned long long*)parent, (unsigned long long)i0, n, Lpad, out,       \
                               ctx->giveups_dev);                                                                     \
        else                                                                                                           \
            hipLaunchKernelGGL((k_perturb<PPV, false>), dim3(blocks), dim3(256), 0, ctx->stream, *rng, theta, K, (int)P, \
                               priors, (const unsigned long long*)parent, (unsigned long long)i0, n, L_or_dv, out,    \
                               ctx->giveups_dev);                                                                     \
    } while (0)
    switch (PP) {
        case 2: LAUNCH_PT(2); break;
        case 4: LAUNCH_PT(4); break;
        case 8: LAUNCH_PT(8); break;
        case 16: LAUNCH_PT(16); break;
        case 32: LAUNCH_PT(32); break;
        default:
            if (multivariate) {
                LAUNCH_PT(64);
            } else {
                const size_t lds = 64 * sizeof(double) + 64 * sizeof(abc_prior);
                hipLaunchKernelGGL((k_perturb_stream<64, false>), dim3(blocks), dim3(256), lds, ctx->stream, *rng, theta, K,
                                   (int)P, priors, (const unsigned long long*)parent, (unsigned long long)i0, n, L_or_dv, out,
                                   ctx->giveups_dev);
            }
            break;
    }
#undef LAUNCH_PT
    ABC_HIP(ctx, hipGetLastError());
    if (seeds && !(prep && prep->seeds_done)) ABC_TRY(launch_seeds(ctx, rng, i0, n, seeds, seed_stream_offset, nullptr));
    return ABC_OK;
}

int abc_moments_on_side(abc_ctx* ctx, const double* theta, size_t K, size_t P, bool multivariate, double* L_io, double* dv,
                        int* spd_dev, const double* model_hdr, bool theta_ev_bound, const char* who, abc_side_moments* m) {
    m->L = m->stats = nullptr;
    if (multivariate) {
        m->L = L_io ? L_io : (double*)abc_ws_alloc(ctx, P * P * 8);
        if (!m->L) ABC_FAIL(ctx, ABC_ERR_NOMEM, "%s: workspace exhausted", who);
    }
    const int PPr = abc_perturb_pp(P);
    abc_status_block* pin = ctx->status_pin;
    m->out = {dv, m->L, spd_dev, nullptr, nullptr, model_hdr, pin->model_hdr, m->L ? &pin->spd : nullptr};
    pin->model_hdr[0] = 0.0; pin->spd = 0;
    m->out.rows = (double*)abc_ws_alloc(ctx, K * (size_t)PPr * sizeof(double));
    if (m->L) m->out.Lpad = (double*)abc_ws_alloc(ctx, (size_t)PPr * PPr * sizeof(double));
    if (!m->out.rows || (m->L && !m->out.Lpad)) ABC_FAIL(ctx, ABC_ERR_NOMEM, "%s: workspace exhausted", who);
    if (!theta_ev_bound) ABC_HIP(ctx, hipEventRecord(ctx->ev_theta, ctx->stream));
    ABC_HIP(ctx, hipStreamWaitEvent(ctx->side, ctx->ev_theta, 0));
    {
        StreamScope on_side(ctx, ctx->side);
        ABC_TRY(launch_theta_stats(ctx, theta, K, P, &m->stats));
        ABC_TRY(launch_post_tail(ctx, theta, K, P, m->stats, &m->out));
    }
    ABC_HIP(ctx, hipEventRecord(ctx->ev_moments, ctx->side));
    return ABC_OK;
}

int abc_normalize_for_resample(abc_ctx* ctx, double* w, size_t K, size_t Nn, const double* sumsq, bool* w_on_host) {
    double* mirror = nullptr;
    const bool alias_on_device = ctx->alias_mode == ABC_ALIAS_DEVICE && K >= ABC_ALIAS_DEV_MIN_K && K <= ABC_ALIAS_DEV_MAX_K;
    if (Nn && !alias_on_device) {
        ABC_TRY(abc_pin_reserve(ctx, abc_alias_pin_bytes(K)));
        mirror = (double*)ctx->pin;
    }
    ABC_TRY(launch_normalize_l2(ctx, w, K, mirror, sumsq));
    *w_on_host = mirror != nullptr;
    return ABC_OK;
}

int abc_prep_hook(void* a) {
    abc_prep_arg* q = (abc_prep_arg*)a;
    int fused_done = 0;
    if (q->moments) {
        StageTimer tm(q->ctx, ST_GATHER_DV);
        double* st = nullptr;
        ABC_TRY(launch_theta_stats(q->ctx, q->theta, q->K, q->P, &st));
        q->theta_stats = st;
        abc_theta_fused f = {q->dv, q->L, q->spd_dev, nullptr, nullptr, q->model_hdr, q->hdr_pin, q->spd_pin};
        if (q->ctx->noise_mode != ABC_NOISE_REFERENCE_STREAM) {
            const int PP = abc_perturb_pp(q->P);
            f.rows = (double*)abc_ws_alloc(q->ctx, q->K * (size_t)PP * sizeof(double));
            if (q->L) f.Lpad = (double*)abc_ws_alloc(q->ctx, (size_t)PP * PP * sizeof(double));
            if (!f.rows || (q->L && !f.Lpad)) ABC_FAIL(q->ctx, ABC_ERR_NOMEM, "generation: workspace exhausted");
        }
        ABC_TRY(launch_post_tail(q->ctx, q->theta, q->K, q->P, st, &f));
        q->prep->rows = f.rows;
        q->prep->Lpad = f.Lpad;
        fused_done = 1;
    }
    if (q->L && !fused_done) {
        if (q->theta_stats) {
            StageTimer tm(q->ctx, ST_MVN);
            ABC_TRY(launch_mvn_from_stats(q->ctx, q->theta_stats, q->P, q->L, q->spd_dev));
        } else {
            ABC_TRY(launch_mvn_setup(q->ctx, q->theta, q->K, q->P, q->L, nullptr, q->spd_dev));
        }
    }
    if (q->ctx->noise_mode == ABC_NOISE_REFERENCE_STREAM) return ABC_OK;
    return launch_perturb_prepare(q->ctx, q->rng, q->theta, q->K, q->P, q->i0, q->Nn, q->seeds, q->seed_off, q->prep,
                                  q->L ? 1 : 0, q->L ? q->L : q->dv);
}

int abc_alias_repair(abc_ctx* ctx, const abc_rng* rng_entry, const double* w, size_t K, uint64_t i0, size_t Nn, uint64_t seed_off,
                     uint64_t* parent, const double* theta, size_t P, const abc_prior* priors, int multivariate, const double* L_or_dv,
                     double* next, abc_perturb_prep* prep, bool giveups_to_snapshot) {
    ctx->alias_dev_fallbacks++;
    const int mode = ctx->alias_mode;
    ctx->alias_mode = ABC_ALIAS_HOST;
    const int rc = launch_resample(ctx, rng_entry, w, K, i0, Nn, parent);
    ctx->alias_mode = mode;
    ABC_TRY(rc);
    prep->seeds_done = 1;
    if (giveups_to_snapshot && ctx->giveups_dev)
        ABC_HIP(ctx, hipMemcpyAsync(ctx->giveups_dev, ctx->giveups_dev + 1, sizeof(unsigned long long), hipMemcpyDeviceToDevice, ctx->stream));
    ABC_TRY(launch_perturb(ctx, rng_entry, theta, K, P, priors, parent, i0, Nn, multivariate, L_or_dv, next, nullptr, seed_off, prep));
    ABC_HIP(ctx, hipStreamSynchronize(ctx->stream));
// ... 34 lines not shown
```

### abcsmc_amd/csrc/select.hip

```cpp
#include "abc_internal.h"

namespace {

struct SelState {
    unsigned long long prefix;
    unsigned long long mask;
    unsigned long long krem;
    unsigned long long n_less;
    unsigned long long ties;
};

__device__ __forceinline__ unsigned long long key_of(double d) {
    const unsigned long long b = (unsigned long long)__double_as_longlong(d);
    return (b >> 63) ? ~b : (b | 0x8000000000000000ull);
}
__device__ __forceinline__ double dist_of(unsigned long long k) {
    const unsigned long long b = (k >> 63) ? (k & 0x7fffffffffffffffull) : ~k;
    return __longlong_as_double((long long)b);
}

constexpr int SEL_BITS = 11;
constexpr int SEL_BINS = 1 << SEL_BITS;

__global__ void k_sel_init(SelState* st, unsigned long long K, unsigned int* hist) {
    for (int i = threadIdx.x; i < SEL_BINS; i += blockDim.x) hist[i] = 0;
    if (threadIdx.x == 0) { st->prefix = 0; st->mask = 0; st->krem = K; st->n_less = 0; st->ties = 0; }
}

__global__ __launch_bounds__(256) void k_sel_hist(const double* __restrict__ dist, size_t n,
                                                  const SelState* __restrict__ st, int shift, int nbits,
                                                  unsigned int* __restrict__ hist) {
    __shared__ unsigned int lh[SEL_BINS];
    for (int i = threadIdx.x; i < SEL_BINS; i += 256) lh[i] = 0;
    __syncthreads();
    const unsigned long long prefix = st->prefix, mask = st->mask;
    const unsigned int dm = (1u << nbits) - 1u;
    const size_t stride = (size_t)gridDim.x * 256;
    const int lane = threadIdx.x & 63;
    const unsigned long long lt_mask = (lane == 0) ? 0ull : (~0ull >> (64 - lane));
    const size_t nround = (n + stride - 1) / stride;
    for (size_t it = 0; it < nround; it++) {
        const size_t i = it * stride + (size_t)blockIdx.x * 256 + threadIdx.x;
        const unsigned long long k = (i < n) ? key_of(dist[i]) : 0ull;
        const bool in = (i < n) && ((k & mask) == prefix);
        const unsigned int d = (unsigned int)(k >> shift) & dm;
        unsigned long long peers = __ballot(in);
        for (int b = 0; b < nbits; b++) {
            const unsigned long long m = __ballot((d >> b) & 1u);
            peers &= ((d >> b) & 1u) ? m : ~m;
        }
        if (in && (peers & lt_mask) == 0) atomicAdd(&lh[d], (unsigned int)__popcll(peers));
    }
    __syncthreads();
// ... 215 lines not shown
__global__ __launch_bounds__(1024) void k_bs_scan(BinSel* __restrict__ bs, unsigned int* __restrict__ hist, unsigned long long K,
                                                  int* __restrict__ fail_flag) {
    __shared__ unsigned int wsum[16];
    __shared__ int s_fail;
    const int t = threadIdx.x, lane = t & 63, wave = t >> 6;
    if (t == 0) s_fail = 0;
    unsigned int c[BPT], sum = 0;
#pragma unroll
    for (int j = 0; j < BPT; j++) { c[j] = hist[BPT * t + j]; sum += c[j]; }
    unsigned int inc = sum;
#pragma unroll
    for (int o = 1; o < 64; o <<= 1) { const unsigned int u = __shfl_up(inc, o, 64); if (lane >= o) inc += u; }
    if (lane == 63) wsum[wave] = inc;
    __syncthreads();
    unsigned int run = inc - sum;
    for (int w = 0; w < wave; w++) run += wsum[w];
    unsigned int tot = 0;
    for (int w = 0; w < 16; w++) tot += wsum[w];
#pragma unroll
    for (int j = 0; j < BPT; j++) {
        const unsigned int off = run;
        hist[BPT * t + j] = off;
        if ((unsigned long long)off < K && K <= (unsigned long long)off + c[j]) { bs->bstar = BPT * t + j; bs->need = K - off; }
        if ((unsigned long long)off < K && c[j] > (unsigned int)BS_CAP) s_fail = 1;
        run += c[j];
    }
    if (t == 0) hist[BPT * 1024] = tot;
    __syncthreads();
    if (t == 0) {
        const int fail = (s_fail || (unsigned long long)tot < K) ? 1 : 0;
        bs->fail = fail;
        *fail_flag = fail;
    }
}

__global__ __launch_bounds__(256) void k_bs_scatter(const double* __restrict__ dist, size_t n, const BinSel* __restrict__ bs,
                                                    const unsigned int* __restrict__ offs, unsigned int* __restrict__ cursor,
                                                    unsigned long long idx_base, unsigned long long* __restrict__ tkey,
                                                    unsigned long long* __restrict__ tidx) {
    if (bs->fail) return;
    const unsigned long long lo = bs->lo, hi = bs->hi;
    const int shift = bs->shift, bstar = bs->bstar;
    const size_t i = (size_t)blockIdx.x * 256 + threadIdx.x;
    if (i >= n) return;
    const unsigned long long k = key_of(dist[i]);
    if (k > hi) return;
    const int b = bs_bin(k, lo, shift);
    if (b > bstar) return;
    const unsigned int p = offs[b] + atomicAdd(&cursor[(size_t)b * BS_CSTRIDE], 1u);
    tkey[p] = k;
    tidx[p] = idx_base + i;
}

__global__ __launch_bounds__(256) void k_bs_sort(const BinSel* __restrict__ bs, const unsigned int* __restrict__ offs,
                                                 const unsigned long long* __restrict__ tkey,
                                                 const unsigned long long* __restrict__ tidx, unsigned long long K,
                                                 unsigned long long idx_base, unsigned long long* __restrict__ oidx,
                                                 double* __restrict__ odist) {
    __shared__ unsigned long long sk[BS_CAP];
    __shared__ unsigned long long si[BS_CAP];
    const int b = blockIdx.x, t = threadIdx.x;
    if (bs->fail) {
        for (unsigned long long i = (unsigned long long)b * 256 + t; i < K; i += (unsigned long long)gridDim.x * 256) {
            oidx[i] = idx_base + i;
            if (odist) odist[i] = 0.0;
        }
        return;
    }
    if (b > bs->bstar) return;
    const unsigned int o0 = offs[b], cnt = offs[b + 1] - o0;
    if (cnt == 0) return;
    const unsigned int keep = (b == bs->bstar) ? (unsigned int)bs->need : cnt;
    unsigned int n2 = 2;
    while (n2 < cnt) n2 <<= 1;
    for (unsigned int e = t; e < n2; e += 256) {
        sk[e] = (e < cnt) ? tkey[o0 + e] : ~0ull;
        si[e] = (e < cnt) ? tidx[o0 + e] : ~0ull;
    }
    __syncthreads();
    for (unsigned int k = 2; k <= n2; k <<= 1)
        for (unsigned int j = k >> 1; j > 0; j >>= 1) {
            for (unsigned int p = t; p < n2 / 2; p += 256) {
                const unsigned int i = ((p & ~(j - 1)) << 1) | (p & (j - 1));
                const unsigned long long ka = sk[i], kb = sk[i + j], ia = si[i], ib = si[i + j];
                const bool gt = (ka > kb) || (ka == kb && ia > ib);
                if (gt == ((i & k) == 0)) { sk[i] = kb; sk[i + j] = ka; si[i] = ib; si[i + j] = ia; }
            }
            __syncthreads();
        }
    for (unsigned int e = t; e < keep; e += 256) {
        oidx[o0 + e] = si[e];
        if (odist) odist[o0 + e] = dist_of(sk[e]);
    }
}

constexpr int CP_ITEMS = 8;
constexpr int CP_CHUNK = 256 * CP_ITEMS;

__global__ __launch_bounds__(256) void k_cp_count(const double* __restrict__ dist, size_t n,
                                                  SelState* __restrict__ st,
                                                  unsigned int* __restrict__ cnt , int nb,
                                                  const unsigned int* __restrict__ last_hist = nullptr, int shift = 0,
                                                  int nbits = 0, unsigned long long K = 0) {
    __shared__ unsigned int sl[4], se[4];
    __shared__ unsigned long long csum[256];
    __shared__ int found_digit;
    __shared__ unsigned long long found_below;
    unsigned long long T;
    if (last_hist) {
        const SelState fin = sel_pick_block(last_hist, st[0], shift, nbits, 1, K, csum, &found_digit, &found_below);
        if (threadIdx.x == 0) st[1] = fin;
        T = fin.prefix;
    } else {
        T = st->prefix;
    }
    const size_t base = (size_t)blockIdx.x * CP_CHUNK + (size_t)threadIdx.x * CP_ITEMS;
    unsigned int l = 0, e = 0;
#pragma unroll
    for (int j = 0; j < CP_ITEMS; j++) {
        const size_t i = base + j;
        if (i < n) { const unsigned long long k = key_of(dist[i]); l += (k < T); e += (k == T); }
    }
#pragma unroll
    for (int o = 32; o >= 1; o >>= 1) { l += __shfl_xor(l, o, 64); e += __shfl_xor(e, o, 64); }
    if ((threadIdx.x & 63) == 0) { sl[threadIdx.x >> 6] = l; se[threadIdx.x >> 6] = e; }
    __syncthreads();
    if (threadIdx.x == 0) {
        cnt[blockIdx.x] = sl[0] + sl[1] + sl[2] + sl[3];
        cnt[nb + blockIdx.x] = se[0] + se[1] + se[2] + se[3];
    }
}

__global__ __launch_bounds__(256) void k_scan_u32(unsigned int* __restrict__ a, int m0, int m1,
                                                  unsigned long long* __restrict__ totals = nullptr) {
    __shared__ unsigned int s[256];
    __shared__ unsigned int carry;
    for (int seg = 0; seg < 2; seg++) {
        unsigned int* p = seg ? a + m0 : a;
        const int m = seg ? m1 : m0;
        if (threadIdx.x == 0) carry = 0;
        __syncthreads();
        for (int b0 = 0; b0 < m; b0 += 256) {
            const int i = b0 + threadIdx.x;
            const unsigned int v = (i < m) ? p[i] : 0u;
            s[threadIdx.x] = v;
// ... 302 lines not shown
    ABC_HIP(ctx, hipGetLastError());
    return ABC_OK;
}
int launch_select_hist(abc_ctx* ctx, const double* dist, size_t n, const long long* state, int pass, int* hist) {
    if (pass < 0 || pass > 5) ABC_FAIL(ctx, ABC_ERR_INVALID, "select: pass %d", pass);
    if (n == 0) return ABC_OK;
    StageTimer tm(ctx, ST_SELECT);
    size_t hb = (n + 255) / 256;
    if (hb > 512) hb = 512;
    hipLaunchKernelGGL(k_sel_hist, dim3((unsigned)hb), dim3(256), 0, ctx->stream, dist, n, (const SelState*)state,
                       kSelShift[pass], kSelWidth[pass], (unsigned int*)hist);
    ABC_HIP(ctx, hipGetLastError());
    return ABC_OK;
}
int launch_select_pick(abc_ctx* ctx, long long* state, int pass, int* hist, uint64_t K) {
    if (pass < 0 || pass > 5) ABC_FAIL(ctx, ABC_ERR_INVALID, "select: pass %d", pass);
    StageTimer tm(ctx, ST_SELECT);
    hipLaunchKernelGGL(k_sel_pick, dim3(1), dim3(256), 0, ctx->stream, (SelState*)state, kSelShift[pass], kSelWidth[pass],
                       (unsigned int*)hist, (int)(pass == 5), (unsigned long long)K);
    ABC_HIP(ctx, hipGetLastError());
    return ABC_OK;
}
int launch_select_count(abc_ctx* ctx, const double* dist, size_t n, const long long* state, long long* counts) {
    StageTimer tm(ctx, ST_SELECT);
    const int nb = (int)((n + CP_CHUNK - 1) / CP_CHUNK);
    unsigned int* cnt = (unsigned int*)abc_ws_alloc(ctx, (size_t)2 * (nb + 1) * sizeof(unsigned int));
    if (!cnt) ABC_FAIL(ctx, ABC_ERR_NOMEM, "select: workspace exhausted");
    if (nb) hipLaunchKernelGGL(k_cp_count, dim3(nb), dim3(256), 0, ctx->stream, dist, n, (SelState*)state, cnt, nb);
    hipLaunchKernelGGL(k_scan_u32, dim3(1), dim3(256), 0, ctx->stream, cnt, nb, nb, (unsigned long long*)counts);
    ABC_HIP(ctx, hipGetLastError());
    return ABC_OK;
}
int launch_select_compact(abc_ctx* ctx, const double* dist, size_t n, const long long* state, uint64_t n_less,
                          uint64_t ties_take, uint64_t idx_base, uint64_t* idx_out, double* dist_out) {
    StageTimer tm(ctx, ST_SELECT);
    const size_t nw = n_less + ties_take;
    if (nw == 0 || n == 0) return ABC_OK;
    const int nb = (int)((n + CP_CHUNK - 1) / CP_CHUNK);
    unsigned int* cnt = (unsigned int*)abc_ws_alloc(ctx, (size_t)2 * nb * sizeof(unsigned int));
    unsigned long long* lim = (unsigned long long*)abc_ws_alloc(ctx, 2 * sizeof(unsigned long long));
    unsigned long long* key = (unsigned long long*)abc_ws_alloc(ctx, nw * 8);
    if (!cnt || !lim || !key) ABC_FAIL(ctx, ABC_ERR_NOMEM, "select: workspace exhausted");
    const unsigned long long hl[2] = {n_less, ties_take};
    ABC_HIP(ctx, hipMemcpyAsync(lim, hl, sizeof(hl), hipMemcpyHostToDevice, ctx->stream));
    hipLaunchKernelGGL(k_cp_count, dim3(nb), dim3(256), 0, ctx->stream, dist, n, (SelState*)state, cnt, nb);
    hipLaunchKernelGGL(k_scan_u32, dim3(1), dim3(256), 0, ctx->stream, cnt, nb, nb, (unsigned long long*)nullptr);
    hipLaunchKernelGGL(k_cp_write, dim3(nb), dim3(256), 0, ctx->stream, dist, n, (const SelState*)state, cnt, nb,
                       (unsigned long long)idx_base, key, (unsigned long long*)idx_out, lim);
    hipLaunchKernelGGL(k_keys_to_dist, dim3((unsigned)((nw + 255) / 256)), dim3(256), 0, ctx->stream, key, nw, dist_out);
    ABC_HIP(ctx, hipGetLastError());
    return ABC_OK;
}

static int select_by_bins(abc_ctx* ctx, const double* dist, size_t n, size_t K, uint64_t idx_base, uint64_t* idx, double* dist_out) {
    if (!ctx->sel_fail_dev) ABC_HIP(ctx, hipMalloc((void**)&ctx->sel_fail_dev, sizeof(int)));
    int* const fail_dev = ctx->sel_fail_dev;
    const int nbins = K <= ((size_t)1 << 18) ? BS_NB : BS_NB_BIG;
    BinSel* bs = (BinSel*)abc_ws_alloc(ctx, sizeof(BinSel));
    unsigned int* hist = (unsigned int*)abc_ws_alloc(ctx, ((size_t)nbins + 1) * sizeof(unsigned int));
    unsigned int* cursor = (unsigned int*)abc_ws_alloc(ctx, (size_t)nbins * BS_CSTRIDE * sizeof(unsigned int));
    unsigned long long* tkey = (unsigned long long*)abc_ws_alloc(ctx, (K + BS_CAP) * 8);
    unsigned long long* tidx = (unsigned long long*)abc_ws_alloc(ctx, (K + BS_CAP) * 8);
    if (!bs || !hist || !cursor || !tkey || !tidx) ABC_FAIL(ctx, ABC_ERR_NOMEM, "select: workspace exhausted");
    StageTimer tm(ctx, ST_SELECT);
    hipLaunchKernelGGL(k_bs_sample, dim3(1), dim3(1024), 0, ctx->stream, dist, n, (unsigned long long)K, bs, hist, fail_dev, nbins);
    size_t hb = (n + 255) / 256;
    if (hb > 512) hb = 512;
    const size_t hl = (size_t)nbins * sizeof(unsigned int);
    if (hl > (48u << 10)) ABC_HIP(ctx, hipFuncSetAttribute((const void*)k_bs_hist, hipFuncAttributeMaxDynamicSharedMemorySize, (int)hl));
    hipLaunchKernelGGL(k_bs_hist, dim3((unsigned)hb), dim3(256), hl, ctx->stream, dist, n, (const BinSel*)bs, hist, cursor, nbins);
    if (nbins == BS_NB) hipLaunchKernelGGL(k_bs_scan<BS_NB / 1024>, dim3(1), dim3(1024), 0, ctx->stream, bs, hist, (unsigned long long)K, fail_dev);
    else hipLaunchKernelGGL(k_bs_scan<BS_NB_BIG / 1024>, dim3(1), dim3(1024), 0, ctx->stream, bs, hist, (unsigned long long)K, fail_dev);
    hipLaunchKernelGGL(k_bs_scatter, dim3((unsigned)((n + 255) / 256)), dim3(256), 0, ctx->stream, dist, n, (const BinSel*)bs,
                       (const unsigned int*)hist, cursor, (unsigned long long)idx_base, tkey, tidx);
    hipLaunchKernelGGL(k_bs_sort, dim3((unsigned)nbins), dim3(256), 0, ctx->stream, (const BinSel*)bs, (const unsigned int*)hist,
                       (const unsigned long long*)tkey, (const unsigned long long*)tidx, (unsigned long long)K,
                       (unsigned long long)idx_base, (unsigned long long*)idx, dist_out);
    ABC_HIP(ctx, hipGetLastError());
    return ABC_OK;
}

static int select_by_radix(abc_ctx* ctx, const double* dist, size_t n, size_t K, uint64_t idx_base, uint64_t* idx, double* dist_out) {
    unsigned long long* key0 = (unsigned long long*)abc_ws_alloc(ctx, K * 8);
    unsigned long long* key1 = (unsigned long long*)abc_ws_alloc(ctx, K * 8);
    unsigned long long* idx1 = (unsigned long long*)abc_ws_alloc(ctx, K * 8);
    if (!key0 || !key1 || !idx1) ABC_FAIL(ctx, ABC_ERR_NOMEM, "select: workspace exhausted");
    unsigned long long* idx0 = (unsigned long long*)idx;
    {
    StageTimer tm(ctx, ST_SELECT);
    if (K == n) {
        hipLaunchKernelGGL(k_init_pairs, dim3((unsigned)((n + 255) / 256)), dim3(256), 0, ctx->stream, dist, n,
                           (unsigned long long)idx_base, key0, idx0);
    } else {
        SelState* st = (SelState*)abc_ws_alloc(ctx, 7 * sizeof(SelState));
        unsigned int* hist = (unsigned int*)abc_ws_alloc(ctx, 6 * SEL_BINS * sizeof(unsigned int));
        const int nb = (int)((n + CP_CHUNK - 1) / CP_CHUNK);
        unsigned int* cnt = (unsigned int*)abc_ws_alloc(ctx, (size_t)2 * nb * sizeof(unsigned int));
        if (!st || !hist || !cnt) ABC_FAIL(ctx, ABC_ERR_NOMEM, "select: workspace exhausted");
        hipLaunchKernelGGL(k_sel_init_fused, dim3(1), dim3(256), 0, ctx->stream, st, (unsigned long long)K, hist);
        size_t hb = (n + 255) / 256;
        if (hb > 512) hb = 512;
        static const int shifts[6] = {53, 42, 31, 20, 9, 0};
        static const int widths[6] = {11, 11, 11, 11, 11, 9};
        for (int p = 0; p < 6; p++)
            hipLaunchKernelGGL(k_sel_hist_fused, dim3((unsigned)hb), dim3(256), 0, ctx->stream, dist, n, st, p,
                               p ? shifts[p - 1] : 0, p ? widths[p - 1] : 0, shifts[p], widths[p], hist, (unsigned long long)K);
        hipLaunchKernelGGL(k_cp_count, dim3(nb), dim3(256), 0, ctx->stream, dist, n, st + 5, cnt, nb,
                           (const unsigned int*)(hist + 5 * SEL_BINS), shifts[5], widths[5], (unsigned long long)K);
        hipLaunchKernelGGL(k_scan_u32, dim3(1), dim3(256), 0, ctx->stream, cnt, nb, nb, (unsigned long long*)nullptr);
        hipLaunchKernelGGL(k_cp_write, dim3(nb), dim3(256), 0, ctx->stream, dist, n, (const SelState*)(st + 6), cnt, nb,
                           (unsigned long long)idx_base, key0, idx0, (const unsigned long long*)nullptr);
    }
    }
    ABC_HIP(ctx, hipGetLastError());
    ABC_TRY(sort_pairs_u64(ctx, key0, idx0, key1, idx1, K));
    if (dist_out) {
        hipLaunchKernelGGL(k_keys_to_dist, dim3((unsigned)((K + 255) / 256)), dim3(256), 0, ctx->stream, key0, K,
                           dist_out);
        ABC_HIP(ctx, hipGetLastError());
    }
    return ABC_OK;
}

int launch_select_smallest(abc_ctx* ctx, const double* dist, size_t n, size_t K, uint64_t idx_base, uint64_t* idx,
                           double* dist_out, bool defer_check) {
    if (K == 0) return ABC_OK;
    if (K > n) ABC_FAIL(ctx, ABC_ERR_INVALID, "select: K = %zu > n = %zu", K, n);
    const bool bins = !ctx->sel_force_radix && n >= 4 * (size_t)BS_S && 2 * K <= n && K <= ((size_t)1 << 20);
    ctx->sel_bins_ran = bins;
    if (!bins) return select_by_radix(ctx, dist, n, K, idx_base, idx, dist_out);
    const size_t mark = ctx->ws_off;
    ABC_TRY(select_by_bins(ctx, dist, n, K, idx_base, idx, dist_out));
    if (defer_check) return ABC_OK;
    int failed = 0;
    ABC_TRY(abc_select_check(ctx, &failed));
    if (!failed) return ABC_OK;
    ctx->ws_off = mark;
    return select_by_radix(ctx, dist, n, K, idx_base, idx, dist_out);
}

int abc_select_check_queue(abc_ctx* ctx, int* slot) {
    *slot = 0;
    if (!ctx->sel_bins_ran || !ctx->sel_fail_dev) return ABC_OK;
    ABC_HIP(ctx, hipMemcpyAsync(slot, ctx->sel_fail_dev, sizeof(int), hipMemcpyDeviceToHost, ctx->stream));
    return ABC_OK;
}
int abc_select_check_done(abc_ctx* ctx, const int* slot) {
    const int f = (ctx->sel_bins_ran && ctx->sel_fail_dev) ? *slot : 0;
    ctx->sel_bins_ran = false;
    return f;
}

int abc_select_check(abc_ctx* ctx, int* failed) {
    *failed = 0;
    if (!ctx->sel_bins_ran || !ctx->sel_fail_dev) return ABC_OK;
    int f = 0;
    ABC_HIP(ctx, hipMemcpyAsync(&f, ctx->sel_fail_dev, sizeof(int), hipMemcpyDeviceToHost, ctx->stream));
    ABC_HIP(ctx, hipStreamSynchronize(ctx->stream));
    ctx->sel_bins_ran = false;
    *failed = f;
    return ABC_OK;
}

__global__ __launch_bounds__(256) void k_merge_runs(const double* __restrict__ key, const unsigned long long* __restrict__ idx,
                                                    int W, size_t len, double* __restrict__ okey,
                                                    unsigned long long* __restrict__ oidx,
                                                    unsigned long long* __restrict__ osrc ) {
    const size_t t = (size_t)blockIdx.x * 256 + threadIdx.x;
    if (t >= (size_t)W * len) return;
    const int q = (int)(t / len);
    const size_t i = t - (size_t)q * len;
    const double d = key[t];
    const unsigned long long x = key_of(d);
    size_t top = 1;
    while (top < len) top <<= 1;
    size_t pos = i;
    for (int r0 = 0; r0 < W; r0 += 8) {
        size_t lo[8];
#pragma unroll
        for (int u = 0; u < 8; u++) lo[u] = 0;
#pragma unroll 1
        for (size_t step = top; step >= 1; step >>= 1) {
            unsigned long long y[8];
#pragma unroll
            for (int u = 0; u < 8; u++) {
                const int r = (r0 + u < W) ? r0 + u : q;
                const size_t c = lo[u] + step;
                y[u] = key_of(key[(size_t)r * len + ((c <= len) ? c - 1 : 0)]);
            }
#pragma unroll
            for (int u = 0; u < 8; u++) {
                const int r = r0 + u;
                const size_t c = lo[u] + step;
// ... 38 lines not shown
```

### abcsmc_amd/csrc/weights.hip

```cpp
#include <stdlib.h>

#include "abc_internal.h"
#include <hip/hip_ext.h>

namespace {

__device__ __forceinline__ double wave_sum(double v) {
#pragma unroll
    for (int o = 32; o >= 1; o >>= 1) v += __shfl_xor(v, o, 64);
    return v;
}

__device__ __forceinline__ double block_sum_256(double v, double* sm ) {
    v = wave_sum(v);
    __syncthreads();
    if ((threadIdx.x & 63) == 0) sm[threadIdx.x >> 6] = v;
    __syncthreads();
    return (sm[0] + sm[1]) + (sm[2] + sm[3]);
}

__global__ __launch_bounds__(256) void k_gather_rows(const double* __restrict__ Y, size_t n_local, size_t ldy,
                                                     int P, const unsigned long long* __restrict__ idx, size_t K,
                                                     unsigned long long idx_base, double* __restrict__ theta,
                                                     size_t ldt, const int* __restrict__ sel_fail, int* __restrict__ sel_fail_pin,
                                                     unsigned long long* __restrict__ giveups) {
    const size_t e = (size_t)blockIdx.x * 256 + threadIdx.x;
    if (e == 0) { if (sel_fail) *sel_fail_pin = *sel_fail; if (giveups) giveups[1] = giveups[0]; }
    if (e >= K * (size_t)P) return;
    const size_t i = e % K, p = e / K;
    const unsigned long long g = idx[i];
    if (g >= idx_base && g - idx_base < n_local) theta[i + ldt * p] = Y[(g - idx_base) + ldy * p];
}

__global__ __launch_bounds__(256) void k_doubled_variance(const double* __restrict__ theta, size_t K,
                                                          double* __restrict__ dv) {
    __shared__ double sm[4];
    const double* col = theta + K * (size_t)blockIdx.x;
    double s = 0.0;
    for (size_t i = threadIdx.x; i < K; i += 256) s += col[i];
    const double mean = block_sum_256(s, sm) / (double)K;
    double ss = 0.0;
    for (size_t i = threadIdx.x; i < K; i += 256) { const double d = col[i] - mean; ss = fma(d, d, ss); }
    ss = block_sum_256(ss, sm);
    if (threadIdx.x == 0) dv[blockIdx.x] = (K > 1) ? 2.0 * (ss / (double)(K - 1)) : 0.0;
}

constexpr int W_MAXP = 1024;
struct WConst {
    double scale[W_MAXP];
    double logC;
    double C;
    int nzero;
    int zero_idx[W_MAXP];
    int far;
    int nfar_i, nfar_j;
    int lim_i;
    double centre[W_MAXP];
    unsigned long long hb_lo, hb_hi;
};

constexpr double W_SQRT_LOG2E = 1.2011224087864497825;
constexpr double W_COORD_BOUND = 2000.0;
constexpr double W_HB_MAX = 1.0e8;

constexpr int KS_MAX_FAR_J = 1024;
__device__ __forceinline__ bool ks_split_on(const WConst* wc) {
    return !(wc->nzero | wc->far) && wc->nfar_i <= wc->lim_i && wc->nfar_j <= KS_MAX_FAR_J;
}

__global__ __launch_bounds__(64) void k_wprep(const double* __restrict__ dv_prev, int P, WConst* __restrict__ wc, int lim_i) {
    __shared__ double fac[64];
    __shared__ int live[64];
    const int pmax = (P > 64) ? ((P + 63) / 64) * 64 : 64;
    double C = 1.0; int nz = 0;
    for (int p0 = 0; p0 < pmax; p0 += 64) {
        const int p = p0 + (int)threadIdx.x;
        double sc = 0.0, f = 1.0;
        int lv = 0;
        if (p < P) {
            const double dv = dv_prev[p];
            if (dv != 0.0) { const double sg = sqrt(dv); sc = 1.0 / sg; f = 1.0 / (sqrt(2.0 * M_PI) * sg); lv = 1; }
        }
        wc->scale[p] = sc * W_SQRT_LOG2E;
        fac[threadIdx.x] = f; live[threadIdx.x] = lv;
        __syncthreads();
        if (threadIdx.x == 0)
            for (int q = 0; q < 64 && p0 + q < P; q++) {
                if (live[q]) C *= fac[q]; else wc->zero_idx[nz++] = p0 + q;
            }
        __syncthreads();
    }
    if (threadIdx.x != 0) return;
    wc->C = C; wc->nzero = nz; wc->logC = 0.0; wc->far = 0; wc->nfar_i = 0; wc->nfar_j = 0; wc->lim_i = lim_i;
    wc->hb_lo = ~0ull; wc->hb_hi = 0ull;
}

__global__ __launch_bounds__(256) void k_wscale(const double* __restrict__ in, size_t rows, size_t ld, int P, int PP,
                                                WConst* __restrict__ wc, const double* __restrict__ centre,
                                                size_t ldc, const double* __restrict__ w, double* __restrict__ out,
                                                double* __restrict__ hb) {
    const size_t r = (size_t)blockIdx.x * 256 + threadIdx.x;
    if (r >= rows) return;
    double nn = 0.0;
    bool far = false;
    for (int p = 0; p < PP; p++) {
        const double v = (p < P) ? (in[r + ld * p] - centre[ldc * p]) * wc->scale[p] : 0.0;
        out[r * PP + p] = v;
        nn = fma(v, v, nn);
        far = far || (fabs(v) > W_COORD_BOUND);
    }
    if (hb) {
        const double lw = -log2(w[r]);
        hb[r] = 0.5 * nn + ((lw > W_HB_MAX) ? W_HB_MAX : lw);
    }
    if (far) atomicOr(&wc->far, 1);
}

template <bool SAFE>
__device__ __forceinline__ double exp2_neg(double x) {
    if (SAFE) x = fmax(x, -1100.0);
    const double tm = x + 6755399441055744.0;
    const double f = x - (tm - 6755399441055744.0);
    double p = 0x1.61afced541895p-20;
    p = fma(p, f, 0x1.00dad250bededp-16);
    p = fma(p, f, 0x1.430acca32fd76p-13);
    p = fma(p, f, 0x1.5d87483855455p-10);
    p = fma(p, f, 0x1.3b2ab5c529311p-7);
    p = fma(p, f, 0x1.c6b08dd46d38fp-5);
    p = fma(p, f, 0x1.ebfbdff9319e1p-3);
    p = fma(p, f, 0x1.62e42fef8615ep-1);
    p = fma(p, f, 0x1.ffffffffff7a3p-1);
    return ldexp(p, __double2loint(tm));
}

template <int PP>
__device__ __forceinline__ void kde_body(unsigned bx, unsigned by, unsigned ny, const double* __restrict__ a , size_t kn,
                                         const double* __restrict__ b , size_t Kp,
                                         const double* __restrict__ hb , const WConst* __restrict__ wc,
                                         const double* __restrict__ theta_raw, size_t K, size_t k0,
                                         const double* __restrict__ prev_raw, double* __restrict__ part,
                                         int fallback_of_split) {
    if (fallback_of_split && ks_split_on(wc)) return;
    const size_t i = (size_t)bx * 256 + threadIdx.x;
    const size_t slices = ny, sl = by;
    const unsigned j0 = __builtin_amdgcn_readfirstlane((unsigned)(Kp * sl / slices));
    const unsigned j1 = __builtin_amdgcn_readfirstlane((unsigned)(Kp * (sl + 1) / slices));
    const bool active = i < kn;
    double ai[PP];
    double ha = 0.0;
#pragma unroll
    for (int p = 0; p < PP; p++) { ai[p] = active ? a[i * PP + p] : 0.0; ha = fma(ai[p], ai[p], ha); }
    ha *= 0.5;
    const int nzero = wc->nzero;
    double acc = 0.0;
    if (nzero == 0 && wc->far == 0) {
        for (unsigned j = j0; j < j1; j++) {
            const double* bj = b + (size_t)j * PP;
            double bc[PP];
#pragma unroll
            for (int p = 0; p < PP; p++) bc[p] = bj[p];
            const double hc = hb[j];
            __builtin_amdgcn_sched_barrier(0);
            double e = -(ha + hc);
#pragma unroll
            for (int p = 0; p < PP; p++) e = fma(ai[p], bc[p], e);
            acc += exp2_neg<false>(e);
        }
    } else {
        for (unsigned j = j0; j < j1; j++) {
            const double* bj = b + (size_t)j * PP;
            double e = -(ha + hb[j]);
#pragma unroll
            for (int p = 0; p < PP; p++) e = fma(ai[p], bj[p], e);
            double term = exp2_neg<true>(e);
            for (int z = 0; z < nzero; z++) {
                const int p = wc->zero_idx[z];
                if (active && theta_raw[(k0 + i) + K * (size_t)p] != prev_raw[j + Kp * (size_t)p]) term = 0.0;
            }
            acc += term;
        }
    }
    if (active) part[sl * kn + i] = acc;
}
template <int PP>
__global__ __launch_bounds__(256) void k_kde(const double* __restrict__ a, size_t kn, const double* __restrict__ b, size_t Kp,
                                             const double* __restrict__ hb, const WConst* __restrict__ wc,
                                             const double* __restrict__ theta_raw, size_t K, size_t k0,
                                             const double* __restrict__ prev_raw, double* __restrict__ part, int fallback_of_split) {
    kde_body<PP>(blockIdx.x, blockIdx.y, gridDim.y, a, kn, b, Kp, hb, wc, theta_raw, K, k0, prev_raw, part, fallback_of_split);
}

template <int PP>
__global__ __launch_bounds__(256) void k_epan(const double* __restrict__ a, size_t kn, const double* __restrict__ b, size_t Kp,
                                              const double* __restrict__ w_prev, const WConst* __restrict__ wc, int P,
                                              double* __restrict__ part) {
    const size_t i = (size_t)blockIdx.x * 256 + threadIdx.x;
    const size_t slices = gridDim.y, sl = blockIdx.y;
    const unsigned j0 = __builtin_amdgcn_readfirstlane((unsigned)(Kp * sl / slices));
    const unsigned j1 = __builtin_amdgcn_readfirstlane((unsigned)(Kp * (sl + 1) / slices));
    const bool active = i < kn;
    double ai[PP];
#pragma unroll
    for (int p = 0; p < PP; p++) ai[p] = active ? a[i * PP + p] : 0.0;
    const double c = 1.0 / (1.4426950408889634 * (double)(P - wc->nzero + 4));
    double acc = 0.0;
    for (unsigned j = j0; j < j1; j++) {
        const double* bj = b + (size_t)j * PP;
        double d2 = 0.0;
// ... 135 lines not shown
                                               WConst* __restrict__ wc, const double* __restrict__ w, int is_prev,
                                               double* __restrict__ out, double* __restrict__ hb,
                                               unsigned short* __restrict__ tiles, int ops, unsigned char* __restrict__ far_flag,
                                               unsigned* __restrict__ far_list, int* __restrict__ ha_int, double* __restrict__ ha_frac,
                                               int fold ,
                                               const unsigned* __restrict__ rank ,
                                               float* __restrict__ topf ) {
    constexpr int G = 2 * NCH, RW = 64 / G;
    const int lane = threadIdx.x & 63, g = lane / RW, rr = lane % RW;
    const size_t wave = (size_t)blockIdx.x * 4 + (threadIdx.x >> 6);
    if (wave * RW >= rows_pad) return;
    const size_t r = wave * RW + rr;
    const bool inrange = r < rows;
    double v[8], nn = 0.0;
    bool far2k = false, far8 = false;
#pragma unroll
    for (int j = 0; j < 8; j++) {
        const int p = 8 * g + j;
        v[j] = (inrange && p < P) ? (in[r + ld * (size_t)p] - wc->centre[p]) * wc->scale[p] : 0.0;
        nn = fma(v[j], v[j], nn);
        far2k = far2k || (fabs(v[j]) > W_COORD_BOUND);
        far8 = far8 || !(fabs(v[j]) <= KS_BOUND);
    }
    if (inrange) {
#pragma unroll
        for (int j = 0; j < 8; j += 2) {
            const int p = 8 * g + j;
            if (p < PP) *reinterpret_cast<double2*>(out + r * (size_t)PP + p) = make_double2(v[j], v[j + 1]);
        }
    }
    double nrow = __shfl(nn, rr, 64);
#pragma unroll
    for (int gg = 1; gg < G; gg++) nrow += __shfl(nn, gg * RW + rr, 64);
    bool rfar2k = far2k, rfar8 = far8;
#pragma unroll
    for (int o = RW; o < 64; o <<= 1) {
        const int o2k = __shfl_xor((int)rfar2k, o, 64), o8 = __shfl_xor((int)rfar8, o, 64);
        rfar2k = rfar2k | (o2k != 0);
        rfar8 = rfar8 | (o8 != 0);
    }
    bool valid = inrange;
    double lw = 0.0;
    bool far = false;
    if (is_prev) {
        const double wr = inrange ? w[r] : 0.0;
        const double lwr = -log2(wr);
        if (inrange && g == 0) hb[r] = 0.5 * nrow + ((lwr > W_HB_MAX) ? W_HB_MAX : lwr);
        if (wr == 0.0) valid = false;
        else {
            lw = lwr;
            if (!(lw >= KS_LW_MIN && lw <= KS_LW_CAP)) far = true;
        }
    }
    if (rfar2k && inrange && g == 0) atomicOr(&wc->far, 1);
    if (valid) far = far || rfar8 || !(nrow <= KS_NORM2);
    if (far) {
        if (g == 0) {
            if (is_prev) { const int pos = atomicAdd(&wc->nfar_j, 1); if (pos < KS_MAX_FAR_J) far_list[pos] = (unsigned)r; }
            else atomicAdd(&wc->nfar_i, 1);
        }
        valid = false;
    }
    if (!is_prev && g == 0) far_flag[r] = far ? 1 : 0;
    const size_t spos = (rank && inrange) ? (size_t)rank[r] : r;
    unsigned short* tb = tiles + (spos >> 5) * (size_t)ops * 512;
    const unsigned r32 = (unsigned)(spos & 31);
    const int c = g >> 1, h = g & 1;
    unsigned pk[KS_NL][4];
    unsigned top_pc[3] = {0u, 0u, 0u}, low_pc[3] = {0u, 0u, 0u};
    const bool fold_lane = fold && g == 2 * NST - 1;
    if (fold_lane && is_prev) ks_pieces_f16(valid ? 0.5 * nrow + lw : KS_HB_ZERO, KS_XUNIT_INV, top_pc, low_pc);
#pragma unroll
    for (int j = 0; j < 8; j++) {
        const double x = valid ? v[j] : 0.0;
        const int n0 = (int)rint(x * KS_U0);
        const double r1 = x - (double)n0 * (1.0 / KS_U0);
        const int n1 = (int)rint(r1 * KS_UH);
        const double r2 = r1 - (double)n1 * (1.0 / KS_UH);
        unsigned b[KS_NL];
        b[0] = f16_of_int(n0, 7);
        b[1] = f16_of_int(n1, 18);
        b[2] = f16_of_int(n0, 18);
        b[3] = f16_bits(r2 * 0x1p11);
        if (fold_lane && j >= 5) {
            if (is_prev) { b[0] = top_pc[j - 5]; b[2] = low_pc[j - 5]; }
            else { b[0] = 0xBC00u; b[3] = 0x8001u; }
        }
#pragma unroll
        for (int k = 0; k < KS_NL; k++) {
            if (j & 1) pk[k][j >> 1] |= b[k] << 16; else pk[k][j >> 1] = b[k];
        }
    }
#pragma unroll
    for (int k = 0; k < KS_NL; k++)
        if (NST == NCH || c < NST)
            *(uint4*)(tb + (size_t)(c * KS_NL + k) * 512 + (h * 32 + r32) * 8) = make_uint4(pk[k][0], pk[k][1], pk[k][2], pk[k][3]);
    if (g == 0) {
        if (is_prev && !fold) {
            unsigned pc[6];
            unsigned short* ob = tb + (size_t)(NST * KS_NL) * 512;
            const double hbv = valid ? 0.5 * nrow + lw : KS_HB_ZERO;
            ks_pieces(hbv, KS_XUNIT_INV, pc);
            if (topf) topf[spos] = (float)(rint(hbv * KS_XUNIT_INV) / KS_XUNIT_INV);
            const unsigned ones = KS_MONE | (KS_MONE << 16);
            *(uint4*)(ob + r32 * 8) = make_uint4(pc[0] | (pc[1] << 16), pc[2] | (pc[3] << 16), pc[4] | (pc[5] << 16), (r32 & 4) ? 0u : ones);
            *(uint4*)(ob + (32 + r32) * 8) = make_uint4(0u, 0u, 0u, (r32 & 4) ? ones : 0u);
        } else if (!is_prev) {
// ... 732 lines not shown
    double* hbk = nullptr;
    unsigned* qh = nullptr;
    if (split) {
        bt = (unsigned short*)abc_ws_alloc(ctx, nbt * opb * 1024);
        far_list = (unsigned*)abc_ws_alloc(ctx, KS_MAX_FAR_J * sizeof(unsigned));
        if (!bt || !far_list) ABC_FAIL(ctx, ABC_ERR_NOMEM, "weights: workspace exhausted");
        if (topn) {
            rank = (unsigned*)abc_ws_alloc(ctx, Kp * sizeof(unsigned));
            tmin = (uint2*)abc_ws_alloc(ctx, nbt * sizeof(uint2));
            topf = (float*)abc_ws_alloc(ctx, nbt * 32 * sizeof(float));
            hbk = (double*)abc_ws_alloc(ctx, Kp * sizeof(double));
            qh = (unsigned*)abc_ws_alloc(ctx, (size_t)256 * ((Kp + WQ_CHUNK - 1) / WQ_CHUNK) * sizeof(unsigned));
            if (!rank || !tmin || !topf || !hbk || !qh) ABC_FAIL(ctx, ABC_ERR_NOMEM, "weights: workspace exhausted");
        }
    }
    if (!wc || !b || !hb || !cpart) ABC_FAIL(ctx, ABC_ERR_NOMEM, "weights: workspace exhausted");
    const double* centre = (const double*)((const char*)wc + offsetof(WConst, centre));
    hipLaunchKernelGGL(k_wprep, dim3(1), dim3(64), 0, s, dv_prev, (int)P, wc, (int)(kn_max / 16 + 32));
    hipLaunchKernelGGL(k_wcentre, dim3((unsigned)P, WC_NB), dim3(256), 0, s, theta_prev, Kp, wc, cpart);
    hipLaunchKernelGGL(k_wcentre_finish, dim3(1), dim3(P > 64 ? 1024 : 64), 0, s, theta_prev, Kp, (int)P, cpart, wc);
    if (topn) {
        const int nbq = (int)((Kp + WQ_CHUNK - 1) / WQ_CHUNK);
        hipLaunchKernelGGL(k_whb, dim3((unsigned)((Kp + 255) / 256)), dim3(256), 0, s, theta_prev, Kp, (int)P, wc, w_prev, hbk);
        hipLaunchKernelGGL(k_wq_hist, dim3(nbq), dim3(256), 0, s, (const double*)hbk, Kp, (const WConst*)wc, qh, nbq);
        hipLaunchKernelGGL(k_wq_scan, dim3(1), dim3(1024), 0, s, qh, 256 * nbq);
        hipLaunchKernelGGL(k_wq_rank, dim3(nbq), dim3(256), 0, s, (const double*)hbk, Kp, (const WConst*)wc, (const unsigned*)qh, nbq, rank);
        ABC_HIP(ctx, hipGetLastError());
    }
    if (split) {
        const size_t rbp = nbt * 32;
        if (NCH == 1)
            hipLaunchKernelGGL(k_wrows<1>, dim3((unsigned)((rbp / 32 + 3) / 4)), dim3(256), 0, s, theta_prev, Kp, Kp, (int)P, PP, rbp, wc,
                               w_prev, 1, b, hb, bt, opb, (unsigned char*)nullptr, far_list, (int*)nullptr, (double*)nullptr, fold ? 1 : 0, (const unsigned*)rank, topf);
        else if (NCH == 2)
            hipLaunchKernelGGL(k_wrows<2>, dim3((unsigned)((rbp / 16 + 3) / 4)), dim3(256), 0, s, theta_prev, Kp, Kp, (int)P, PP, rbp, wc,
                               w_prev, 1, b, hb, bt, opb, (unsigned char*)nullptr, far_list, (int*)nullptr, (double*)nullptr, fold ? 1 : 0, (const unsigned*)rank, topf);
        else if (NCH == 3)
            hipLaunchKernelGGL((k_wrows<4, 3>), dim3((unsigned)((rbp / 8 + 3) / 4)), dim3(256), 0, s, theta_prev, Kp, Kp, (int)P, PP, rbp, wc,
                               w_prev, 1, b, hb, bt, opb, (unsigned char*)nullptr, far_list, (int*)nullptr, (double*)nullptr, fold ? 1 : 0, (const unsigned*)rank, topf);
        else
            hipLaunchKernelGGL(k_wrows<4>, dim3((unsigned)((rbp / 8 + 3) / 4)), dim3(256), 0, s, theta_prev, Kp, Kp, (int)P, PP, rbp, wc,
                               w_prev, 1, b, hb, bt, opb, (unsigned char*)nullptr, far_list, (int*)nullptr, (double*)nullptr, fold ? 1 : 0, (const unsigned*)rank, topf);
    } else {
        hipLaunchKernelGGL(k_wscale, dim3((unsigned)((Kp + 255) / 256)), dim3(256), 0, s, theta_prev, Kp, Kp,
                           (int)P, PP, wc, centre, (size_t)1, w_prev, b, hb);
    }
    if (topn) hipLaunchKernelGGL(k_tile_tmin, dim3((unsigned)((nbt + 255) / 256)), dim3(256), 0, s, (const float*)topf, nbt, tmin);
    ABC_HIP(ctx, hipGetLastError());
    out->wc = wc; out->b = b; out->hb = hb; out->bt = bt; out->far_list = far_list; out->tmin = (unsigned*)tmin;
    out->Kp = Kp; out->P = P; out->kn_max = kn_max; out->split = split ? 1 : 0; out->ready = 1;
    return ABC_OK;
}

int launch_weights_raw(abc_ctx* ctx, const abc_prior* priors, const double* theta, size_t K, size_t P, size_t k0,
                       size_t kn, const double* theta_prev, size_t Kp, const double* w_prev, const double* dv_prev,
                       double* w_raw, const abc_wprev* prev, const double** sumsq_out) {
    if (sumsq_out) *sumsq_out = nullptr;
    if (P > (size_t)W_MAXP) ABC_FAIL(ctx, ABC_ERR_UNSUPPORTED, "weights: P = %zu > %d parameters", P, W_MAXP);
    if (kn == 0) return ABC_OK;
    ABC_TRY(abc_kde_words(ctx));
    if (Kp > 0xffffffffull) ABC_FAIL(ctx, ABC_ERR_UNSUPPORTED, "weights: K' = %zu >= 2^32", Kp);
    if (k0 + kn > K) ABC_FAIL(ctx, ABC_ERR_INVALID, "weights: row range [%zu,%zu) outside K=%zu", k0, k0 + kn, K);
    int PP = 2;
    while (PP < (int)P) PP *= 2;
    if (P > 64) PP = (int)((P + 63) / 64 * 64);
    const size_t rb = (kn + 255) / 256;
    size_t slices = abc_kde_slices(kn, Kp, PP);
    if (slices > Kp / 64) slices = Kp / 64;
    if (slices < 1) slices = 1;
    if (slices > 1024) slices = 1024;
    const int NCH = ks_chunks(P);
    const bool epan = ctx->weight_kernel == ABC_WEIGHT_EPANECHNIKOV;
    const bool split = (PP >= 8 && P <= 64 && ctx->kde_mode != ABC_KDE_FP64 && !epan);
    const size_t nbt = (Kp + 31) / 32, nat = rb * 8;
    const int opa = NCH * KS_NL;
    const bool fold = ks_fold_on(P, split);
    if (split) {
        size_t cap = 12288 / rb;
        if (cap < 8) cap = 8;
        if (slices > cap) slices = cap;
    }
    abc_wprev own;
    if (!prev || !prev->ready) {
        ABC_TRY(launch_weights_prev(ctx, P, kn, theta_prev, Kp, w_prev, dv_prev, &own, nullptr));
        prev = &own;
    }
    if (prev->Kp != Kp || prev->P != P || prev->kn_max < kn || (prev->split != 0) != split)
        ABC_FAIL(ctx, ABC_ERR_INVALID, "weights: the prepared previous set does not match this call");
    WConst* wc = (WConst*)prev->wc;
    double* b = prev->b;
    double* hb = prev->hb;
    unsigned short* bt = prev->bt;
    unsigned* far_list = prev->far_list;
    double* a = (double*)abc_ws_alloc(ctx, kn * PP * sizeof(double));
    double* part = (double*)abc_ws_alloc(ctx, slices * kn * sizeof(double));
    unsigned short* at = nullptr;
    unsigned char* far_flag = nullptr;
    double *fix_i = nullptr, *fix_j = nullptr, *ha_frac = nullptr;
    int* ha_int = nullptr;
    if (split) {
        at = (unsigned short*)abc_ws_alloc(ctx, nat * opa * 1024);
        far_flag = (unsigned char*)abc_ws_alloc(ctx, nat * 32);
        fix_i = (double*)abc_ws_alloc(ctx, kn * sizeof(double));
        fix_j = (double*)abc_ws_alloc(ctx, kn * sizeof(double));
        ha_frac = (double*)abc_ws_alloc(ctx, nat * 32 * sizeof(double));
        ha_int = (int*)abc_ws_alloc(ctx, nat * 32 * sizeof(int));
        if (!at || !far_flag || !fix_i || !fix_j || !ha_frac || !ha_int) ABC_FAIL(ctx, ABC_ERR_NOMEM, "weights: workspace exhausted");
    }
    if (!a || !part) ABC_FAIL(ctx, ABC_ERR_NOMEM, "weights: workspace exhausted");
    const double* centre = (const double*)((const char*)wc + offsetof(WConst, centre));
    StageTimer tm(ctx, ST_WEIGHTS_MISC);
    if (split) {
        const size_t ra = nat * 32;
        if (NCH == 1)
            hipLaunchKernelGGL(k_wrows<1>, dim3((unsigned)((ra / 32 + 3) / 4)), dim3(256), 0, ctx->stream, theta + k0, kn, K, (int)P, PP, ra,
                               wc, (const double*)nullptr, 0, a, (double*)nullptr, at, opa, far_flag, far_list, ha_int, ha_frac, fold ? 1 : 0, (const unsigned*)nullptr, (float*)nullptr);
        else if (NCH == 2)
            hipLaunchKernelGGL(k_wrows<2>, dim3((unsigned)((ra / 16 + 3) / 4)), dim3(256), 0, ctx->stream, theta + k0, kn, K, (int)P, PP, ra,
                               wc, (const double*)nullptr, 0, a, (double*)nullptr, at, opa, far_flag, far_list, ha_int, ha_frac, fold ? 1 : 0, (const unsigned*)nullptr, (float*)nullptr);
        else if (NCH == 3)
            hipLaunchKernelGGL((k_wrows<4, 3>), dim3((unsigned)((ra / 8 + 3) / 4)), dim3(256), 0, ctx->stream, theta + k0, kn, K, (int)P, PP, ra,
                               wc, (const double*)nullptr, 0, a, (double*)nullptr, at, opa, far_flag, far_list, ha_int, ha_frac, fold ? 1 : 0, (const unsigned*)nullptr, (float*)nullptr);
        else
            hipLaunchKernelGGL(k_wrows<4>, dim3((unsigned)((ra / 8 + 3) / 4)), dim3(256), 0, ctx->stream, theta + k0, kn, K, (int)P, PP, ra,
                               wc, (const double*)nullptr, 0, a, (double*)nullptr, at, opa, far_flag, far_list, ha_int, ha_frac, fold ? 1 : 0, (const unsigned*)nullptr, (float*)nullptr);
    } else {
        hipLaunchKernelGGL(k_wscale, dim3((unsigned)((kn + 255) / 256)), dim3(256), 0, ctx->stream, theta + k0, kn, K,
                           (int)P, PP, wc, centre, (size_t)1, (const double*)nullptr, a, (double*)nullptr);
    }
#define LAUNCH_KDE(PPV)                                                                                        \
    hipLaunchKernelGGL(k_kde<PPV>, dim3((unsigned)rb, (unsigned)slices), dim3(256), 0, ctx->stream, a, kn, b, \
                       Kp, hb, wc, theta, K, k0, theta_prev, part, split ? 1 : 0)
    if (epan) {
        StageTimer tk(ctx, ST_KDE);
#define LAUNCH_EPAN(PPV) hipLaunchKernelGGL(k_epan<PPV>, dim3((unsigned)rb, (unsigned)slices), dim3(256), 0, ctx->stream, a, kn, b, Kp, w_prev, wc, (int)P, part)
        if (PP > 64)
            hipLaunchKernelGGL(k_kde_gen, dim3((unsigned)rb, (unsigned)slices), dim3(256), 0, ctx->stream, a, kn, b, Kp, hb, wc, theta, K, k0,
                               theta_prev, part, PP, 1, (int)P, w_prev);
        else
        switch (PP) {
            case 2: LAUNCH_EPAN(2); break;
            case 4: LAUNCH_EPAN(4); break;
            case 8: LAUNCH_EPAN(8); break;
            case 16: LAUNCH_EPAN(16); break;
            case 32: LAUNCH_EPAN(32); break;
            default: LAUNCH_EPAN(64); break;
        }
#undef LAUNCH_EPAN
    } else {
        StageTimer tk(ctx, ST_KDE);
        if (split) {
            if (fold && NCH == 1)
                hipLaunchKernelGGL((k_kde_split<KS_FOLD + 1, 3, true, 1>), dim3((unsigned)rb, (unsigned)slices), dim3(256), 0, ctx->stream,
                                   (const uint4*)at, kn, (const uint4*)bt, (unsigned)nbt, wc, (const int*)ha_int, part, (const uint2*)prev->tmin);
            else if (fold && NCH == 2)
                hipLaunchKernelGGL((k_kde_split<KS_FOLD + 2, 2, false, 0>), dim3((unsigned)rb, (unsigned)slices), dim3(256), 0, ctx->stream,
                                   (const uint4*)at, kn, (const uint4*)bt, (unsigned)nbt, wc, (const int*)ha_int, part, (const uint2*)prev->tmin);
            else if (fold && NCH == 3)
                hipLaunchKernelGGL((k_kde_split_lds<KS_FOLD + 3, KDE_LDS_W3, KDE_LDS_F4>), dim3((unsigned)rb, (unsigned)slices), dim3(256), 0, ctx->stream,
                                   (const uint4*)at, kn, (const uint4*)bt, (unsigned)nbt, wc, (const int*)ha_int, part, (const uint2*)prev->tmin);
            else if (fold)
                hipLaunchKernelGGL((k_kde_split_lds<KS_FOLD + 4, 2, KDE_LDS_F4>), dim3((unsigned)rb, (unsigned)slices), dim3(256), 0, ctx->stream,
                                   (const uint4*)at, kn, (const uint4*)bt, (unsigned)nbt, wc, (const int*)ha_int, part, (const uint2*)prev->tmin);
            else if (prev->tmin && NCH == 1)
                hipLaunchKernelGGL((k_kde_split<KS_TOPN + 1, 3, true, 1>), dim3((unsigned)rb, (unsigned)slices), dim3(256), 0, ctx->stream,
                                   (const uint4*)at, kn, (const uint4*)bt, (unsigned)nbt, wc, (const int*)ha_int, part, (const uint2*)prev->tmin);
            else if (prev->tmin && NCH == 2)
                hipLaunchKernelGGL((k_kde_split<KS_TOPN + 2, 2, false, 0>), dim3((unsigned)rb, (unsigned)slices), dim3(256), 0, ctx->stream,
                                   (const uint4*)at, kn, (const uint4*)bt, (unsigned)nbt, wc, (const int*)ha_int, part, (const uint2*)prev->tmin);
            else if (prev->tmin && NCH == 3)
                hipLaunchKernelGGL((k_kde_split_lds<KS_TOPN + 3, KDE_LDS_W3, KDE_LDS_F4>), dim3((unsigned)rb, (unsigned)slices), dim3(256), 0, ctx->stream,
                                   (const uint4*)at, kn, (const uint4*)bt, (unsigned)nbt, wc, (const int*)ha_int, part, (const uint2*)prev->tmin);
            else if (prev->tmin)
                hipLaunchKernelGGL((k_kde_split_lds<KS_TOPN + 4, 2, KDE_LDS_F4>), dim3((unsigned)rb, (unsigned)slices), dim3(256), 0, ctx->stream,
                                   (const uint4*)at, kn, (const uint4*)bt, (unsigned)nbt, wc, (const int*)ha_int, part, (const uint2*)prev->tmin);
            else if (NCH == 1)
                hipLaunchKernelGGL((k_kde_split<1, 3, true, 1>), dim3((unsigned)rb, (unsigned)slices), dim3(256), 0, ctx->stream,
                                   (const uint4*)at, kn, (const uint4*)bt, (unsigned)nbt, wc, (const int*)ha_int, part, (const uint2*)prev->tmin);
            else if (NCH == 2)
                hipLaunchKernelGGL((k_kde_split<2, 2>), dim3((unsigned)rb, (unsigned)slices), dim3(256), 0, ctx->stream,
                                   (const uint4*)at, kn, (const uint4*)bt, (unsigned)nbt, wc, (const int*)ha_int, part, (const uint2*)prev->tmin);
            else if (NCH == 3)
                hipLaunchKernelGGL((k_kde_split_lds<3, KDE_LDS_W3, KDE_LDS_F4>), dim3((unsigned)rb, (unsigned)slices), dim3(256), 0, ctx->stream,
                                   (const uint4*)at, kn, (const uint4*)bt, (unsigned)nbt, wc, (const int*)ha_int, part, (const uint2*)prev->tmin);
            else
                hipLaunchKernelGGL((k_kde_split_lds<4, 2, KDE_LDS_F4>), dim3((unsigned)rb, (unsigned)slices), dim3(256), 0, ctx->stream,
                                   (const uint4*)at, kn, (const uint4*)bt, (unsigned)nbt, wc, (const int*)ha_int, part, (const uint2*)prev->tmin);
        }
        if (PP > 64)
            hipLaunchKernelGGL(k_kde_gen, dim3((unsigned)rb, (unsigned)slices), dim3(256), 0, ctx->stream, a, kn, b, Kp, hb, wc, theta, K, k0,
                               theta_prev, part, PP, 0, (int)P, w_prev);
        else if (split) {
#define LAUNCH_FIX(PPV)                                                                                                       \
    hipLaunchKernelGGL(k_kde_fixups<PPV>, dim3((unsigned)(nat + rb + rb * slices)), dim3(256), 0, ctx->stream, a, kn, b, Kp, hb, wc, \
                       far_flag, far_list, (unsigned)nat, (unsigned)rb, (unsigned)slices, fix_i, fix_j, theta, K, k0, theta_prev, part)
            switch (PP) {
                case 8: LAUNCH_FIX(8); break;
                case 16: LAUNCH_FIX(16); break;
                case 32: LAUNCH_FIX(32); break;
                default: LAUNCH_FIX(64); break;
            }
#undef LAUNCH_FIX
        } else
        switch (PP) {
            case 2: LAUNCH_KDE(2); break;
            case 4: LAUNCH_KDE(4); break;
            case 8: LAUNCH_KDE(8); break;
            case 16: LAUNCH_KDE(16); break;
            case 32: LAUNCH_KDE(32); break;
            default: LAUNCH_KDE(64); break;
        }
    }
#undef LAUNCH_KDE
    const unsigned fb = (unsigned)((kn + 63) / 64);
    double* sq_part = nullptr;
    if (sumsq_out && k0 == 0 && kn == K) {
        sq_part = (double*)abc_ws_alloc(ctx, ((size_t)fb + 1) * sizeof(double));
        if (!sq_part) ABC_FAIL(ctx, ABC_ERR_NOMEM, "weights: workspace exhausted");
        *sumsq_out = sq_part;
    }
    hipLaunchKernelGGL(k_wfinish, dim3(fb), dim3(256), 0, ctx->stream, priors, theta, K, (int)P, k0, kn, part,
                       (int)slices, wc, w_raw, split ? 1 : 0, epan ? 1 : 0, ctx->kde_which, far_flag, fix_i, fix_j, ha_frac, sq_part);
    ABC_HIP(ctx, hipGetLastError());
    return ABC_OK;
}

int abc_kde_words(abc_ctx* ctx) {
    if (ctx->kde_which) return ABC_OK;
    ABC_HIP(ctx, hipMalloc((void**)&ctx->kde_which, 2 * sizeof(int)));
    ABC_HIP(ctx, hipMemsetAsync(ctx->kde_which, 0, 2 * sizeof(int), ctx->stream));
    return ABC_OK;
}

int launch_fill(abc_ctx* ctx, double* w, size_t K, double v, hipStream_t st) {
    if (!K) return ABC_OK;
    hipLaunchKernelGGL(k_fill, dim3((unsigned)((K + 255) / 256)), dim3(256), 0, st ? st : ctx->stream, w, K, v);
    ABC_HIP(ctx, hipGetLastError());
    return ABC_OK;
}

int launch_normalize_l2(abc_ctx* ctx, double* w, size_t K, double* host_mirror, const double* sumsq_parts) {
    if (!K) return ABC_OK;
    StageTimer tm(ctx, ST_WEIGHTS_MISC);
    const unsigned fb = (unsigned)((K + 63) / 64);
    double* sq_part = const_cast<double*>(sumsq_parts);
    if (!sq_part) {
        sq_part = (double*)abc_ws_alloc(ctx, ((size_t)fb + 1) * sizeof(double));
        if (!sq_part) ABC_FAIL(ctx, ABC_ERR_NOMEM, "normalize: workspace exhausted");
        hipLaunchKernelGGL(k_sumsq_partial, dim3(fb), dim3(256), 0, ctx->stream, w, K, sq_part);
    }
    const unsigned db = (unsigned)((K + 255) / 256);
    if (fb <= SQ_INLINE_MAX) {
        hipLaunchKernelGGL(k_div_norm, dim3(db), dim3(256), 0, ctx->stream, w, K, sq_part, fb, host_mirror);
    } else {
        hipLaunchKernelGGL(k_sumsq_total, dim3(1), dim3(256), 0, ctx->stream, sq_part, fb, sq_part + fb);
        hipLaunchKernelGGL(k_div_norm, dim3(db), dim3(256), 0, ctx->stream, w, K, sq_part + fb, 0u, host_mirror);
    }
    ABC_HIP(ctx, hipGetLastError());
    return ABC_OK;
}
```

Before: 358.3 million particles/s.

## Fuse select with gather, split KDE weight tiles early, fold normalization into alias build

Top-K selection is merged with the theta row gather, and the weight stage is split into a tile-preparation phase and a sums phase. Tile preparation is launched right after the gather so it runs ahead of the Wilcoxon tail. L2 normalization of the weights is deferred and folded into the alias-table block-sum kernel, which divides the weights in place. A fused draw descriptor is also passed into perturb so resample and perturb can share work. The aim is to cut kernel launches and full passes over the 1M-weight vector and to overlap setup with earlier stages, at the cost of more complex state and of the alias kernel now writing to weights it previously only read.

Measured after the change: 357.2 million particles/s. Within noise of the previous version (-0.3%).

```diff
diff --git a/abcsmc_amd/csrc/abc_internal.h b/abcsmc_amd/csrc/abc_internal.h
--- a/abcsmc_amd/csrc/abc_internal.h
+++ b/abcsmc_amd/csrc/abc_internal.h
@@ -268,6 +268,9 @@
 int launch_draws(abc_ctx*, const SmValues& sv, size_t B, size_t K, size_t P, const abc_draws* dr, const char* fn);
 int launch_select_smallest(abc_ctx*, const double* dist, size_t n, size_t K, uint64_t idx_base,
                            uint64_t* idx, double* dist_out, bool defer_check = false);
+int launch_select_smallest_gather(abc_ctx* ctx, const double* dist, size_t n, size_t K, uint64_t idx_base, uint64_t* idx, double* dist_out,
+                                  const double* Y, size_t ldy, size_t P, double* theta, size_t ldt, int* sel_fail_pin,
+                                  hipEvent_t wait_first, hipEvent_t done, bool* bins_deferred);
 int abc_select_check(abc_ctx* ctx, int* failed);
 int abc_select_check_queue(abc_ctx* ctx, int* slot);
 int abc_select_check_done(abc_ctx* ctx, const int* slot);
@@ -343,17 +346,32 @@
                        size_t k0, size_t kn, const double* theta_prev, size_t Kp,
                        const double* w_prev, const double* dv_prev, double* w_raw, const abc_wprev* prev = nullptr,
                        const double** sumsq_out = nullptr);
+struct abc_wtiles {
+    abc_wprev prev;
+    double* a; double* part; unsigned short* at; unsigned char* far_flag; double* fix_i; double* fix_j; double* ha_frac; int* ha_int;
+    size_t K, P, k0, kn, Kp; int ready;
+};
+int launch_weights_tiles(abc_ctx*, const double* theta, size_t K, size_t P, size_t k0, size_t kn, const double* theta_prev, size_t Kp,
+                         const double* w_prev, const double* dv_prev, const abc_wprev* prev, abc_wtiles* t);
+int launch_weights_sums(abc_ctx*, const abc_prior* priors, const double* theta, size_t K, size_t P, size_t k0, size_t kn,
+                        const double* theta_prev, size_t Kp, const double* w_prev, double* w_raw, const abc_wtiles* t,
+                        const double** sumsq_out = nullptr);
 int abc_weights_prev_early(abc_ctx* ctx, size_t P, size_t kn_max, const double* theta_prev, size_t Kp, const double* w_prev,
                            const double* dv_prev, abc_wprev* out);
 int launch_fill(abc_ctx*, double* w, size_t K, double v, hipStream_t st = nullptr);
 int launch_normalize_l2(abc_ctx*, double* w, size_t K, double* host_mirror = nullptr, const double* sumsq_parts = nullptr);
+struct abc_norm_pending { double* w; size_t K; const double* sq; unsigned nparts; };
+int launch_normalize_l2_defer(abc_ctx*, double* w, size_t K, const double* sumsq_parts, abc_norm_pending* out);
+int launch_normalize_l2_apply(abc_ctx*, const abc_norm_pending* np);
 static inline size_t abc_alias_pin_bytes(size_t K) { return K * (sizeof(double) * 3 + sizeof(uint32_t) * 3) + 2 * sizeof(uint32_t) + 16; }
 int launch_mvn_setup(abc_ctx*, const double* theta, size_t K, size_t P, double* L, int* status_host,
                      int* status_dev);
+struct abc_draw_fused { const uint32_t* raw; const double* F; const uint32_t* A; size_t K; const int* verdict_src; int* verdict_dev; int* verdict_pin; };
 int launch_resample(abc_ctx*, const abc_rng* rng, const double* w, size_t K, uint64_t i0, size_t n,
                     uint64_t* parent, int (*while_host_builds)(void*) = nullptr, void* hook_arg = nullptr,
                     bool uniform_weights = false, const uint32_t* raw_ready = nullptr, bool weights_on_host = false,
-                    const volatile int* abort_flag = nullptr, bool parents_ready = false, int* alias_check_deferred = nullptr);
+                    const volatile int* abort_flag = nullptr, bool parents_ready = false, int* alias_check_deferred = nullptr,
+                    abc_draw_fused* fuse_draw = nullptr, const abc_norm_pending* norm = nullptr);
 int abc_rng_streams_early(abc_ctx* ctx, const abc_rng* rng, uint64_t i0, size_t n, uint64_t* seeds, uint64_t seed_stream_offset,
                           uint32_t** raw, uint64_t* parent_uniform = nullptr, size_t K_uniform = 0);
 int abc_rng_seeds_early(abc_ctx* ctx, const abc_rng* rng, uint64_t i0, size_t n, uint64_t* seeds, uint64_t seed_stream_offset);
@@ -371,12 +389,13 @@
 int launch_perturb(abc_ctx*, const abc_rng* rng, const double* theta, size_t K, size_t P,
                    const abc_prior* priors, const uint64_t* parent, uint64_t i0, size_t n,
                    int multivariate, const double* L_or_dv, double* out, uint64_t* seeds,
-                   uint64_t seed_stream_offset, const abc_perturb_prep* prep = nullptr);
+                   uint64_t seed_stream_offset, const abc_perturb_prep* prep = nullptr, const abc_draw_fused* draw = nullptr);
 
 struct abc_side_moments { abc_theta_fused out; double* stats; double* L; };
 int abc_moments_on_side(abc_ctx* ctx, const double* theta, size_t K, size_t P, bool multivariate, double* L_io, double* dv,
                         int* spd_dev, const double* model_hdr, bool theta_ev_bound, const char* who, abc_side_moments* m);
-int abc_normalize_for_resample(abc_ctx* ctx, double* w, size_t K, size_t Nn, const double* sumsq, bool* w_on_host);
+int abc_normalize_for_resample(abc_ctx* ctx, double* w, size_t K, size_t Nn, const double* sumsq, bool* w_on_host,
+                               abc_norm_pending* defer = nullptr);
 struct abc_prep_arg {
     abc_ctx* ctx; const abc_rng* rng; const double* theta; const double* theta_stats; size_t K, P, Nn;
     uint64_t i0, seed_off; uint64_t* seeds; abc_perturb_prep* prep; double* L; int* spd_dev; double* dv; bool moments;
@@ -394,7 +413,7 @@
 void abc_alias_preproc(size_t K, const double* w, double* F, uint32_t* A, double* E, uint32_t* smalls, uint32_t* bigs, bool knuth = true);
 
 int launch_alias_build_dev(abc_ctx*, const double* w, size_t K, double* F, uint32_t* A, int* fail_dev, int* fail_pin,
-                           const int** verdict_src = nullptr);
+                           const int** verdict_src = nullptr, const double* sq_in = nullptr, unsigned nparts = 0);
 size_t abc_alias_dev_need(size_t K);
 constexpr size_t ABC_ALIAS_DEV_MAX_K = (size_t)2 << 20;
 constexpr size_t ABC_ALIAS_DEV_MIN_K = 20000;
diff --git a/abcsmc_amd/csrc/alias_dev.hip b/abcsmc_amd/csrc/alias_dev.hip
--- a/abcsmc_amd/csrc/alias_dev.hip
+++ b/abcsmc_amd/csrc/alias_dev.hip
@@ -141,14 +141,28 @@
     __syncthreads();
     return (sm[0] + sm[1]) + (sm[2] + sm[3]);
 }
-__global__ __launch_bounds__(AL_T) void k_al_bsum(const double* __restrict__ w, size_t K, double* __restrict__ bsum, AlHead* __restrict__ head,
-                                                  int force_fail) {
+__global__ __launch_bounds__(AL_T) void k_al_bsum(double* __restrict__ w, size_t K, double* __restrict__ bsum, AlHead* __restrict__ head,
+                                                  int force_fail, const double* __restrict__ sq_in, unsigned nparts) {
     __shared__ double sm[4];
+    static_assert(AL_T == 256, "the sum of squares' tree is the weight stage's: 256 threads");
+    double sq = 0.0;
+    if (sq_in) {
+        if (nparts) {
+            double t = 0.0;
+            for (unsigned j = threadIdx.x; j < nparts; j += 256) t += sq_in[j];
+            sq = block_sum_d(t, sm);
+        } else sq = *sq_in;
+    }
+    const bool divide = sq_in && sq > 0.0;
     const size_t base = (size_t)blockIdx.x * AL_B + (size_t)threadIdx.x * AL_I;
     double s = 0.0;
     bool bad = false;
 #pragma unroll
-    for (int j = 0; j < AL_I; j++) if (base + j < K) { const double x = w[base + j]; s += x; bad = bad || !(x >= 0.0) || !(x < 1.0e300); }
+    for (int j = 0; j < AL_I; j++) if (base + j < K) {
+        double x = w[base + j];
+        if (divide) { x = x / sqrt(sq); w[base + j] = x; }
+        s += x; bad = bad || !(x >= 0.0) || !(x < 1.0e300);
+    }
     const double bs = block_sum_d(bad ? (double)NAN : s, sm);
     if (threadIdx.x == 0) bsum[blockIdx.x] = bs;
     if (blockIdx.x == 0 && threadIdx.x == 0) {
@@ -565,23 +579,23 @@
 
 #if ABC_AL_I == 4
 int launch_alias_build_dev_i2(abc_ctx* ctx, const double* w, size_t K, double* F, uint32_t* A, int* fail_dev, int* fail_pin,
-                              const int** verdict_src);
+                              const int** verdict_src, const double* sq_in, unsigned nparts);
 int launch_alias_build_dev_i4(abc_ctx* ctx, const double* w, size_t K, double* F, uint32_t* A, int* fail_dev, int* fail_pin,
-                              const int** verdict_src);
+                              const int** verdict_src, const double* sq_in, unsigned nparts);
 size_t abc_alias_dev_need(size_t K) {
     constexpr size_t B = AL_T * 2;
     const size_t nblk = (K + B - 1) / B + 1, nblk2 = (2 * K + B - 1) / B + 1;
     return K * (8 + 4 + 4 + 8 + 16 + 16 + 16 + 4 + 4 + 64) + nblk * (8 + 4 + 64 + 64) + nblk2 * 64 * (AL_T + 1) + sizeof(AlHead) + 64 * 256;
 }
 int launch_alias_build_dev(abc_ctx* ctx, const double* w, size_t K, double* F, uint32_t* A, int* fail_dev, int* fail_pin,
-                           const int** verdict_src) {
-    if (K <= ABC_ALIAS_DEV_SMALL_K) return launch_alias_build_dev_i2(ctx, w, K, F, A, fail_dev, fail_pin, verdict_src);
-    return launch_alias_build_dev_i4(ctx, w, K, F, A, fail_dev, fail_pin, verdict_src);
+                           const int** verdict_src, const double* sq_in, unsigned nparts) {
+    if (K <= ABC_ALIAS_DEV_SMALL_K) return launch_alias_build_dev_i2(ctx, w, K, F, A, fail_dev, fail_pin, verdict_src, sq_in, nparts);
+    return launch_alias_build_dev_i4(ctx, w, K, F, A, fail_dev, fail_pin, verdict_src, sq_in, nparts);
 }
 #endif
 
 int ABC_AL_FN(launch_alias_build_dev)(abc_ctx* ctx, const double* w, size_t K, double* F, uint32_t* A, int* fail_dev, int* fail_pin,
-                                      const int** verdict_src) {
+                                      const int** verdict_src, const double* sq_in, unsigned nparts) {
     if (K == 0 || K > (size_t)AL_MAXBLK * AL_B / 2) ABC_FAIL(ctx, ABC_ERR_UNSUPPORTED, "device alias build: K = %zu", K);
     const int nblk = (int)((K + AL_B - 1) / AL_B), nblk2 = (int)((2 * K + AL_B - 1) / AL_B);
     AlHead* head = (AlHead*)abc_ws_alloc(ctx, sizeof(AlHead));
@@ -607,7 +621,7 @@
     const double mean = 1.0 / (double)K, dK = (double)K;
     hipStream_t st = ctx->stream;
     const int force_fail = abc_diag_env("ABC_ALIAS_FORCE_FAIL") ? 1 : 0;
-    hipLaunchKernelGGL(k_al_bsum, dim3(nblk), dim3(AL_T), 0, st, w, K, bsum, head, force_fail);
+    hipLaunchKernelGGL(k_al_bsum, dim3(nblk), dim3(AL_T), 0, st, const_cast<double*>(w), K, bsum, head, force_fail, sq_in, nparts);
     hipLaunchKernelGGL(k_al_sum_reduce, dim3(nblk), dim3(AL_T), 0, st, w, K, (const double*)bsum, nblk, agg, tpre, head);
     hipLaunchKernelGGL(k_al_sum_apply, dim3(nblk), dim3(AL_T), 0, st, w, K, (const double*)bsum, nblk, (const RMap*)agg, (const RMap*)tpre, head);
     hipLaunchKernelGGL(k_al_classify, dim3(nblk), dim3(AL_T), 0, st, w, K, mean, head, E, cnt, F, A);
diff --git a/abcsmc_amd/csrc/api.hip b/abcsmc_amd/csrc/api.hip
--- a/abcsmc_amd/csrc/api.hip
+++ b/abcsmc_amd/csrc/api.hip
@@ -614,7 +614,7 @@
         ABC_TRY(launch_wilcoxon(ctx, io->X, io->Y, N, N, N, M, P, A, (size_t)ntrain, model));
     if (!projected) ABC_TRY(launch_project_distance(ctx, io->X, N, N, M, simple ? Pstat : P, A, model, simple, dist));
     if (K == 0) return ABC_OK;
-    ABC_TRY(launch_select_smallest(ctx, dist, N, K, 0, io->idx, io->dist, io->w != nullptr));
+    if (!io->w) ABC_TRY(launch_select_smallest(ctx, dist, N, K, 0, io->idx, io->dist, false));
     if (!simple && ncomp_host && !io->w) {
         double hdr[4];
         ABC_HIP(ctx, hipMemcpyAsync(hdr, model, sizeof(hdr), hipMemcpyDeviceToHost, ctx->stream));
@@ -633,12 +633,8 @@
     int* const spd_pin = &ctx->status_pin->spd;
     hdr_pin[0] = 0.0; *spd_pin = 0;
     bool status_early = false;
-    bool bins_deferred = ctx->sel_bins_ran && ctx->sel_fail_dev && !ctx->sel_force_radix;
-    ctx->side_early_waited = false;
-    if (wprev.ready) {
-        ABC_HIP(ctx, hipStreamWaitEvent(ctx->stream, ctx->ev_prev, 0));
-        ctx->side_early_waited = true;
-    }
+    bool bins_deferred = false;
+    ctx->side_early_waited = wprev.ready != 0;
     const bool defer_moments = Nn && P <= 64 && K >= 2;
     const bool moments_side_planned = defer_moments && !uniform_w && ctx->side && ctx->noise_mode != ABC_NOISE_REFERENCE_STREAM;
     if (moments_side_planned && !ctx->ev_theta) {
@@ -646,11 +642,18 @@
         ABC_HIP(ctx, hipEventCreateWithFlags(&ctx->ev_moments, abc_xstream_event_flags()));
     }
     const bool theta_ev_bound = moments_side_planned;
-    ABC_TRY(launch_gather_rows(ctx, io->Y, N, N, P, io->idx, K, 0, theta, K, bins_deferred ? ctx->sel_fail_dev : nullptr, pfail_early,
-                               theta_ev_bound ? ctx->ev_theta : nullptr));
+    ABC_TRY(launch_select_smallest_gather(ctx, dist, N, K, 0, io->idx, io->dist, io->Y, N, P, theta, K, pfail_early,
+                                          wprev.ready ? ctx->ev_prev : nullptr, theta_ev_bound ? ctx->ev_theta : nullptr, &bins_deferred));
     if (wx_run) {
         StreamScope on_wx(ctx, ctx->wx_stream);
         ABC_TRY(launch_wilcoxon_level0(ctx, wx_run));
+    }
+    const bool kde_next = Kp != 0 && io->theta_prev;
+    abc_wtiles wtiles;
+    wtiles.ready = 0;
+    if (kde_next) {
+        if (wprev.ready && !ctx->side_early_waited) ABC_HIP(ctx, hipStreamWaitEvent(ctx->stream, ctx->ev_prev, 0));
+        ABC_TRY(launch_weights_tiles(ctx, theta, K, P, 0, K, io->theta_prev, Kp, io->w_prev, io->dv_prev, &wprev, &wtiles));
     }
     bool wx_tail_pending = false;
     if (wx_spec) {
@@ -682,10 +685,9 @@
             *pfail_early = 0;
             if (scores_all) ABC_TRY(launch_distance_from_scores(ctx, scores_all, N, N, M, P, A, model, dist));
             else ABC_TRY(launch_project_distance(ctx, io->X, N, N, M, P, A, model, 0, dist));
-            ABC_TRY(launch_select_smallest(ctx, dist, N, K, 0, io->idx, io->dist, true));
-            bins_deferred = ctx->sel_bins_ran && ctx->sel_fail_dev && !ctx->sel_force_radix;
-            ABC_TRY(launch_gather_rows(ctx, io->Y, N, N, P, io->idx, K, 0, theta, K, bins_deferred ? ctx->sel_fail_dev : nullptr, pfail_early,
-                                       theta_ev_bound ? ctx->ev_theta : nullptr));
+            ABC_TRY(launch_select_smallest_gather(ctx, dist, N, K, 0, io->idx, io->dist, io->Y, N, P, theta, K, pfail_early, nullptr,
+                                                  theta_ev_bound ? ctx->ev_theta : nullptr, &bins_deferred));
+            if (kde_next) ABC_TRY(launch_weights_tiles(ctx, theta, K, P, 0, K, io->theta_prev, Kp, io->w_prev, io->dv_prev, &wprev, &wtiles));
         }
     }
     auto repeat_with_radix = [&]() -> int {
@@ -715,14 +717,13 @@
         ABC_TRY(launch_doubled_variance(ctx, theta, K, P, dv));
     }
     bool w_on_host = false;
+    abc_norm_pending norm_pending = {};
     if (Kp == 0 || !io->theta_prev) {
         if (!filled_early) ABC_TRY(launch_fill(ctx, io->w, K, 1.0 / (double)K));
     } else {
-        if (wprev.ready && !ctx->side_early_waited) ABC_HIP(ctx, hipStreamWaitEvent(ctx->stream, ctx->ev_prev, 0));
         const double* sumsq = nullptr;
-        ABC_TRY(launch_weights_raw(ctx, io->priors, theta, K, P, 0, K, io->theta_prev, Kp, io->w_prev, io->dv_prev,
-                                   io->w, &wprev, &sumsq));
-        ABC_TRY(abc_normalize_for_resample(ctx, io->w, K, Nn, sumsq, &w_on_host));
+        ABC_TRY(launch_weights_sums(ctx, io->priors, theta, K, P, 0, K, io->theta_prev, Kp, io->w_prev, io->w, &wtiles, &sumsq));
+        ABC_TRY(abc_normalize_for_resample(ctx, io->w, K, Nn, sumsq, &w_on_host, &norm_pending));
     }
     abc_side_moments side = {};
     bool moments_on_side = false, seeds_waited = false;
@@ -755,10 +756,12 @@
             pa.model_hdr = simple ? nullptr : model; pa.hdr_pin = hdr_pin; pa.spd_pin = L ? spd_pin : nullptr;
             status_early = true;
         }
+        abc_draw_fused draw = {};
         {
             const int rc = launch_resample(ctx, rng, io->w, K, 0, Nn, parent, abc_prep_hook, &pa, uniform_w, raw_early, w_on_host,
                                            bins_deferred ? pfail_early : nullptr, parent_early != nullptr,
-                                           ctx->noise_mode == ABC_NOISE_REFERENCE_STREAM ? nullptr : &alias_deferred);
+                                           ctx->noise_mode == ABC_NOISE_REFERENCE_STREAM ? nullptr : &alias_deferred,
+                                           ctx->noise_mode == ABC_NOISE_REFERENCE_STREAM ? nullptr : &draw, &norm_pending);
             if (rc == ABC_INTERNAL_RETRY) return repeat_with_radix();
             ABC_TRY(rc);
         }
@@ -768,7 +771,7 @@
                                              cfg->multivariate ? L : dv, io->next, io->seeds));
         } else {
             ABC_TRY(launch_perturb(ctx, rng, theta, K, P, io->priors, parent, 0, Nn, cfg->multivariate,
-                                   cfg->multivariate ? L : dv, io->next, io->seeds, Nn, &prep));
+                                   cfg->multivariate ? L : dv, io->next, io->seeds, Nn, &prep, &draw));
             parent_used = parent; L_used = L; prep_used = prep;
             taus2_jump(rng, 2 * (uint64_t)Nn);
         }
diff --git a/abcsmc_amd/csrc/resample.hip b/abcsmc_amd/csrc/resample.hip
--- a/abcsmc_amd/csrc/resample.hip
+++ b/abcsmc_amd/csrc/resample.hip
@@ -105,6 +105,18 @@
     const size_t c = (size_t)(u * (double)K);
     const double f = (F[c] + (double)c) / (double)K;
     parent[i] = (f == 1.0) ? c : ((u < f) ? c : (size_t)A[c]);
+}
+
+struct DrawArgs { const uint32_t* raw; const double* F; const uint32_t* A; size_t K; const int* verdict_src; int* verdict_dev; int* verdict_pin; };
+__device__ __forceinline__ size_t parent_of(const DrawArgs& d, size_t i, unsigned long long* __restrict__ parent) {
+    if (!d.raw) return (size_t)parent[i];
+    if (i == 0 && d.verdict_src) { const int v = *d.verdict_src; *d.verdict_dev = v; *d.verdict_pin = v; }
+    const double u = (double)d.raw[i] / 4294967296.0;
+    const size_t c = (size_t)(u * (double)d.K);
+    const double f = (d.F[c] + (double)c) / (double)d.K;
+    const size_t par = (f == 1.0) ? c : ((u < f) ? c : (size_t)d.A[c]);
+    parent[i] = par;
+    return par;
 }
 
 __global__ __launch_bounds__(256) void k_widen(const uint32_t* __restrict__ raw, size_t n,
@@ -223,10 +235,10 @@
 template <int PP, bool MV>
 __global__ __launch_bounds__(256, (MV && PP <= 16) ? 3 : (PP <= 16 ? 2 : 1)) void k_perturb(abc_rng key, const double* __restrict__ theta, size_t K, int P,
                                                  const abc_prior* __restrict__ priors,
-                                                 const unsigned long long* __restrict__ parent,
+                                                 unsigned long long* __restrict__ parent,
                                                  unsigned long long i0, size_t n,
                                                  const double* __restrict__ L_or_dv , double* __restrict__ out,
-                                                 unsigned long long* __restrict__ giveups) {
+                                                 unsigned long long* __restrict__ giveups, DrawArgs draw) {
     __shared__ double sS[PP];
     __shared__ abc_prior sp[PP];
     __shared__ double sinv[PP];
@@ -241,7 +253,7 @@
     if (i >= n) return;
     {
     const unsigned long long gi = i0 + i;
-    const double* mrow = theta + (size_t)parent[i] * PP;
+    const double* mrow = theta + parent_of(draw, i, parent) * PP;
     const uint32_t k0 = key.s1 ^ 0x5bd1e995u, k1 = key.s2 ^ (key.s3 * 0x9E3779B1u);
     double x[PP];
     if (MV) {
@@ -289,10 +301,10 @@
 template <int PP, bool MV>
 __global__ __launch_bounds__(256) void k_perturb_stream(abc_rng key, const double* __restrict__ theta, size_t K, int P,
                                                         const abc_prior* __restrict__ priors,
-                                                        const unsigned long long* __restrict__ parent,
+                                                        unsigned long long* __restrict__ parent,
                                                         unsigned long long i0, size_t n,
                                                         const double* __restrict__ L_or_dv, double* __restrict__ out,
-                                                        unsigned long long* __restrict__ giveups) {
+                                                        unsigned long long* __restrict__ giveups, DrawArgs draw) {
     extern __shared__ double smem[];
     double* sL = smem;
     abc_prior* sp = reinterpret_cast<abc_prior*>(smem + (MV ? PP * PP : PP));
@@ -312,7 +324,7 @@
     const size_t i = (size_t)blockIdx.x * 256 + threadIdx.x;
     if (i >= n) return;
     const unsigned long long gi = i0 + i;
-    const double* mu = theta + (size_t)parent[i] * PP;
+    const double* mu = theta + parent_of(draw, i, parent) * PP;
     const uint32_t k0 = key.s1 ^ 0x5bd1e995u, k1 = key.s2 ^ (key.s3 * 0x9E3779B1u);
     if (MV) {
         bool ok = false;
@@ -382,16 +394,16 @@
 template <bool MV>
 __global__ __launch_bounds__(256) void k_perturb_gen(abc_rng key, const double* __restrict__ rows, int P, int PP,
                                                      const abc_prior* __restrict__ priors,
-                                                     const unsigned long long* __restrict__ parent,
+                                                     unsigned long long* __restrict__ parent,
                                                      unsigned long long i0, size_t n, const double* __restrict__ L_or_dv,
-                                                     double* __restrict__ out, unsigned long long* __restrict__ giveups) {
+                                                     double* __restrict__ out, unsigned long long* __restrict__ giveups, DrawArgs draw) {
     extern __shared__ abc_prior spg[];
     for (int p = threadIdx.x; p < P; p += 256) spg[p] = priors[p];
     __syncthreads();
     const size_t i = (size_t)blockIdx.x * 256 + threadIdx.x;
     if (i >= n) return;
     const unsigned long long gi = i0 + i;
-    const double* mu = rows + (size_t)parent[i] * PP;
+    const double* mu = rows + parent_of(draw, i, parent) * PP;
     const uint32_t k0 = key.s1 ^ 0x5bd1e995u, k1 = key.s2 ^ (key.s3 * 0x9E3779B1u);
     if (MV) {
         bool ok = false;
@@ -560,8 +572,13 @@
 int launch_resample(abc_ctx* ctx, const abc_rng* rng, const double* w, size_t K, uint64_t i0, size_t n,
                     uint64_t* parent, int (*while_host_builds)(void*), void* hook_arg, bool uniform_weights,
                     const uint32_t* raw_ready, bool weights_on_host, const volatile int* abort_flag, bool parents_ready,
-                    int* alias_check_deferred) {
+                    int* alias_check_deferred, abc_draw_fused* fuse_draw, const abc_norm_pending* norm) {
     if (alias_check_deferred) *alias_check_deferred = 0;
+    if (fuse_draw) fuse_draw->raw = nullptr;
+    const bool build_on_dev = n && !uniform_weights && K && K <= 0xffffffffull && ctx->alias_mode == ABC_ALIAS_DEVICE &&
+                              K >= ABC_ALIAS_DEV_MIN_K && K <= ABC_ALIAS_DEV_MAX_K && ctx->ws_off + abc_alias_dev_need(K) <= ctx->ws_bytes;
+    const bool norm_in_build = norm && norm->w && norm->w == w && norm->K == K && build_on_dev;
+    if (norm && norm->w && !norm_in_build) ABC_TRY(launch_normalize_l2_apply(ctx, norm));
     bool wait_side = raw_ready != nullptr;
     if (n == 0) return ABC_OK;
     if (K == 0 || K > 0xffffffffull) ABC_FAIL(ctx, ABC_ERR_INVALID, "resample: K = %zu", K);
@@ -590,7 +607,7 @@
         ctx->alias_K = K;
     }
     ctx->alias_A = (uint32_t*)(ctx->alias_F + K);
-    if (ctx->alias_mode == ABC_ALIAS_DEVICE && K >= ABC_ALIAS_DEV_MIN_K && K <= ABC_ALIAS_DEV_MAX_K && ctx->ws_off + abc_alias_dev_need(K) <= ctx->ws_bytes) {
+    if (build_on_dev) {
         if (!ctx->alias_fail_dev) ABC_HIP(ctx, hipMalloc((void**)&ctx->alias_fail_dev, sizeof(int)));
         int* fail_pin = &ctx->status_pin->alias_fail;
         *fail_pin = 0;
@@ -608,11 +625,14 @@
         }
         {
             StageTimer tm(ctx, ST_ALIAS_HOST);
-            ABC_TRY(launch_alias_build_dev(ctx, w, K, ctx->alias_F, ctx->alias_A, ctx->alias_fail_dev, fail_pin, &verdict));
+            ABC_TRY(launch_alias_build_dev(ctx, w, K, ctx->alias_F, ctx->alias_A, ctx->alias_fail_dev, fail_pin, &verdict,
+                                           norm_in_build ? norm->sq : nullptr, norm_in_build ? norm->nparts : 0u));
         }
         ctx->alias_dev_builds++;
         if (while_host_builds) ABC_TRY(while_host_builds(hook_arg));
-        {
+        if (fuse_draw && alias_check_deferred) {
+            *fuse_draw = {raw, ctx->alias_F, ctx->alias_A, K, verdict, ctx->alias_fail_dev, fail_pin};
+        } else {
             StageTimer tm(ctx, ST_RESAMPLE);
             hipLaunchKernelGGL(k_alias_draw, dim3((unsigned)((n + 255) / 256)), dim3(256), 0, ctx->stream, raw, n, ctx->alias_F,
                                ctx->alias_A, K, (unsigned long long*)parent, verdict, ctx->alias_fail_dev, fail_pin);
@@ -728,8 +748,13 @@
 
 int launch_perturb(abc_ctx* ctx, const abc_rng* rng, const double* theta, size_t K, size_t P, const abc_prior* priors,
                    const uint64_t* parent, uint64_t i0, size_t n, int multivariate, const double* L_or_dv, double* out,
-                   uint64_t* seeds, uint64_t seed_stream_offset, const abc_perturb_prep* prep) {
+                   uint64_t* seeds, uint64_t seed_stream_offset, const abc_perturb_prep* prep, const abc_draw_fused* draw) {
     if (n == 0) return ABC_OK;
+    DrawArgs da = {nullptr, nullptr, nullptr, 0, nullptr, nullptr, nullptr};
+    if (draw && draw->raw) {
+        if (draw->K != K) ABC_FAIL(ctx, ABC_ERR_INVALID, "perturb: the pending draws are over another set");
+        da = {draw->raw, draw->F, draw->A, draw->K, draw->verdict_src, draw->verdict_dev, draw->verdict_pin};
+    }
     int PP = 2;
     while (PP < (int)P) PP *= 2;
     if (P > 64) PP = (int)((P + 63) / 64 * 64);
@@ -752,10 +777,10 @@
         const size_t lds = P * sizeof(abc_prior);
         if (multivariate)
             hipLaunchKernelGGL((k_perturb_gen<true>), dim3(blocks), dim3(256), lds, ctx->stream, *rng, theta, (int)P, PP, priors,
-                               (const unsigned long long*)parent, (unsigned long long)i0, n, Lpad, out, ctx->giveups_dev);
+                               (unsigned long long*)parent, (unsigned long long)i0, n, Lpad, out, ctx->giveups_dev, da);
         else
             hipLaunchKernelGGL((k_perturb_gen<false>), dim3(blocks), dim3(256), lds, ctx->stream, *rng, theta, (int)P, PP, priors,
-                               (const unsigned long long*)parent, (unsigned long long)i0, n, L_or_dv, out, ctx->giveups_dev);
+                               (unsigned long long*)parent, (unsigned long long)i0, n, L_or_dv, out, ctx->giveups_dev, da);
         ABC_HIP(ctx, hipGetLastError());
         if (seeds && !(prep && prep->seeds_done)) ABC_TRY(launch_seeds(ctx, rng, i0, n, seeds, seed_stream_offset, nullptr));
         return ABC_OK;
@@ -764,12 +789,12 @@
     do {                                                                                                               \
         if (multivariate)                                                                                              \
             hipLaunchKernelGGL((k_perturb<PPV, true>), dim3(blocks), dim3(256), 0, ctx->stream, *rng, theta, K, (int)P, \
-                               priors, (const unsigned long long*)parent, (unsigned long long)i0, n, Lpad, out,       \
-                               ctx->giveups_dev);                                                                     \
+                               priors, (unsigned long long*)parent, (unsigned long long)i0, n, Lpad, out,             \
+                               ctx->giveups_dev, da);                                                                 \
         else                                                                                                           \
             hipLaunchKernelGGL((k_perturb<PPV, false>), dim3(blocks), dim3(256), 0, ctx->stream, *rng, theta, K, (int)P, \
-                               priors, (const unsigned long long*)parent, (unsigned long long)i0, n, L_or_dv, out,    \
-                               ctx->giveups_dev);                                                                     \
+                               priors, (unsigned long long*)parent, (unsigned long long)i0, n, L_or_dv, out,          \
+                               ctx->giveups_dev, da);                                                                 \
     } while (0)
     switch (PP) {
         case 2: LAUNCH_PT(2); break;
@@ -783,8 +808,8 @@
             } else {
                 const size_t lds = 64 * sizeof(double) + 64 * sizeof(abc_prior);
                 hipLaunchKernelGGL((k_perturb_stream<64, false>), dim3(blocks), dim3(256), lds, ctx->stream, *rng, theta, K,
-                                   (int)P, priors, (const unsigned long long*)parent, (unsigned long long)i0, n, L_or_dv, out,
-                                   ctx->giveups_dev);
+                                   (int)P, priors, (unsigned long long*)parent, (unsigned long long)i0, n, L_or_dv, out,
+                                   ctx->giveups_dev, da);
             }
             break;
     }
@@ -819,12 +844,18 @@
     return ABC_OK;
 }
 
-int abc_normalize_for_resample(abc_ctx* ctx, double* w, size_t K, size_t Nn, const double* sumsq, bool* w_on_host) {
+int abc_normalize_for_resample(abc_ctx* ctx, double* w, size_t K, size_t Nn, const double* sumsq, bool* w_on_host,
+                               abc_norm_pending* defer) {
+    if (defer) defer->w = nullptr;
     double* mirror = nullptr;
     const bool alias_on_device = ctx->alias_mode == ABC_ALIAS_DEVICE && K >= ABC_ALIAS_DEV_MIN_K && K <= ABC_ALIAS_DEV_MAX_K;
     if (Nn && !alias_on_device) {
         ABC_TRY(abc_pin_reserve(ctx, abc_alias_pin_bytes(K)));
         mirror = (double*)ctx->pin;
+    }
+    if (defer && Nn && alias_on_device && sumsq) {
+        *w_on_host = false;
+        return launch_normalize_l2_defer(ctx, w, K, sumsq, defer);
     }
     ABC_TRY(launch_normalize_l2(ctx, w, K, mirror, sumsq));
     *w_on_host = mirror != nullptr;
diff --git a/abcsmc_amd/csrc/select.hip b/abcsmc_amd/csrc/select.hip
--- a/abcsmc_amd/csrc/select.hip
+++ b/abcsmc_amd/csrc/select.hip
@@ -1,4 +1,5 @@
 #include "abc_internal.h"
+#include <hip/hip_ext.h>
 
 namespace {
 
@@ -320,18 +321,25 @@
     tidx[p] = idx_base + i;
 }
 
+struct BsPayload {
+    const double* Y; size_t ldy; int P; double* theta; size_t ldt;
+    const int* sel_fail; int* sel_fail_pin; unsigned long long* giveups;
+};
 __global__ __launch_bounds__(256) void k_bs_sort(const BinSel* __restrict__ bs, const unsigned int* __restrict__ offs,
                                                  const unsigned long long* __restrict__ tkey,
                                                  const unsigned long long* __restrict__ tidx, unsigned long long K,
                                                  unsigned long long idx_base, unsigned long long* __restrict__ oidx,
-                                                 double* __restrict__ odist) {
+                                                 double* __restrict__ odist, BsPayload pl) {
     __shared__ unsigned long long sk[BS_CAP];
     __shared__ unsigned long long si[BS_CAP];
     const int b = blockIdx.x, t = threadIdx.x;
+    if (pl.Y && b == 0 && t == 0) { if (pl.sel_fail) *pl.sel_fail_pin = *pl.sel_fail; if (pl.giveups) pl.giveups[1] = pl.giveups[0]; }
     if (bs->fail) {
         for (unsigned long long i = (unsigned long long)b * 256 + t; i < K; i += (unsigned long long)gridDim.x * 256) {
             oidx[i] = idx_base + i;
             if (odist) odist[i] = 0.0;
+            if (pl.Y)
+                for (int p = 0; p < pl.P; p++) pl.theta[i + pl.ldt * p] = pl.Y[i + pl.ldy * p];
         }
         return;
     }
@@ -359,6 +367,13 @@
     for (unsigned int e = t; e < keep; e += 256) {
         oidx[o0 + e] = si[e];
         if (odist) odist[o0 + e] = dist_of(sk[e]);
+    }
+    if (pl.Y) {
+        const unsigned int tot = keep * (unsigned int)pl.P;
+        for (unsigned int e = t; e < tot; e += 256) {
+            const unsigned int r = e % keep, p = e / keep;
+            pl.theta[(size_t)(o0 + r) + pl.ldt * p] = pl.Y[(size_t)(si[r] - idx_base) + pl.ldy * p];
+        }
     }
 }
 
@@ -767,7 +782,8 @@
     return ABC_OK;
 }
 
-static int select_by_bins(abc_ctx* ctx, const double* dist, size_t n, size_t K, uint64_t idx_base, uint64_t* idx, double* dist_out) {
+static int select_by_bins(abc_ctx* ctx, const double* dist, size_t n, size_t K, uint64_t idx_base, uint64_t* idx, double* dist_out,
+                          const BsPayload* payload = nullptr, hipEvent_t wait_first = nullptr, hipEvent_t done = nullptr) {
     if (!ctx->sel_fail_dev) ABC_HIP(ctx, hipMalloc((void**)&ctx->sel_fail_dev, sizeof(int)));
     int* const fail_dev = ctx->sel_fail_dev;
     const int nbins = K <= ((size_t)1 << 18) ? BS_NB : BS_NB_BIG;
@@ -788,9 +804,17 @@
     else hipLaunchKernelGGL(k_bs_scan<BS_NB_BIG / 1024>, dim3(1), dim3(1024), 0, ctx->stream, bs, hist, (unsigned long long)K, fail_dev);
     hipLaunchKernelGGL(k_bs_scatter, dim3((unsigned)((n + 255) / 256)), dim3(256), 0, ctx->stream, dist, n, (const BinSel*)bs,
                        (const unsigned int*)hist, cursor, (unsigned long long)idx_base, tkey, tidx);
-    hipLaunchKernelGGL(k_bs_sort, dim3((unsigned)nbins), dim3(256), 0, ctx->stream, (const BinSel*)bs, (const unsigned int*)hist,
-                       (const unsigned long long*)tkey, (const unsigned long long*)tidx, (unsigned long long)K,
-                       (unsigned long long)idx_base, (unsigned long long*)idx, dist_out);
+    BsPayload pl = {nullptr, 0, 0, nullptr, 0, nullptr, nullptr, nullptr};
+    if (payload) { pl = *payload; pl.sel_fail = pl.sel_fail_pin ? fail_dev : nullptr; }
+    if (wait_first) ABC_HIP(ctx, hipStreamWaitEvent(ctx->stream, wait_first, 0));
+    if (done)
+        hipExtLaunchKernelGGL(k_bs_sort, dim3((unsigned)nbins), dim3(256), 0, ctx->stream, nullptr, done, 0, (const BinSel*)bs,
+                              (const unsigned int*)hist, (const unsigned long long*)tkey, (const unsigned long long*)tidx, (unsigned long long)K,
+                              (unsigned long long)idx_base, (unsigned long long*)idx, dist_out, pl);
+    else
+        hipLaunchKernelGGL(k_bs_sort, dim3((unsigned)nbins), dim3(256), 0, ctx->stream, (const BinSel*)bs, (const unsigned int*)hist,
+                           (const unsigned long long*)tkey, (const unsigned long long*)tidx, (unsigned long long)K,
+                           (unsigned long long)idx_base, (unsigned long long*)idx, dist_out, pl);
     ABC_HIP(ctx, hipGetLastError());
     return ABC_OK;
 }
@@ -854,6 +878,26 @@
     return select_by_radix(ctx, dist, n, K, idx_base, idx, dist_out);
 }
 
+int launch_select_smallest_gather(abc_ctx* ctx, const double* dist, size_t n, size_t K, uint64_t idx_base, uint64_t* idx, double* dist_out,
+                                  const double* Y, size_t ldy, size_t P, double* theta, size_t ldt, int* sel_fail_pin,
+                                  hipEvent_t wait_first, hipEvent_t done, bool* bins_deferred) {
+    *bins_deferred = false;
+    if (K == 0) return ABC_OK;
+    if (K > n) ABC_FAIL(ctx, ABC_ERR_INVALID, "select: K = %zu > n = %zu", K, n);
+    const bool bins = !ctx->sel_force_radix && n >= 4 * (size_t)BS_S && 2 * K <= n && K <= ((size_t)1 << 20);
+    if (!bins || !P) {
+        ABC_TRY(launch_select_smallest(ctx, dist, n, K, idx_base, idx, dist_out, true));
+        *bins_deferred = ctx->sel_bins_ran && ctx->sel_fail_dev && !ctx->sel_force_radix;
+        if (wait_first) ABC_HIP(ctx, hipStreamWaitEvent(ctx->stream, wait_first, 0));
+        return launch_gather_rows(ctx, Y, n, ldy, P, idx, K, idx_base, theta, ldt, *bins_deferred ? ctx->sel_fail_dev : nullptr, sel_fail_pin, done);
+    }
+    ctx->sel_bins_ran = true;
+    const BsPayload pl = {Y, ldy, (int)P, theta, ldt, nullptr, sel_fail_pin, ctx->giveups_dev};
+    ABC_TRY(select_by_bins(ctx, dist, n, K, idx_base, idx, dist_out, &pl, wait_first, done));
+    *bins_deferred = true;
+    return ABC_OK;
+}
+
 int abc_select_check_queue(abc_ctx* ctx, int* slot) {
     *slot = 0;
     if (!ctx->sel_bins_ran || !ctx->sel_fail_dev) return ABC_OK;
diff --git a/abcsmc_amd/csrc/weights.hip b/abcsmc_amd/csrc/weights.hip
--- a/abcsmc_amd/csrc/weights.hip
+++ b/abcsmc_amd/csrc/weights.hip
@@ -53,7 +53,8 @@
     int nzero;
     int zero_idx[W_MAXP];
     int far;
-    int nfar_i, nfar_j;
+    int nfar_i, far_i;
+    int nfar_j;
     int lim_i;
     double centre[W_MAXP];
     unsigned long long hb_lo, hb_hi;
@@ -65,7 +66,7 @@
 
 constexpr int KS_MAX_FAR_J = 1024;
 __device__ __forceinline__ bool ks_split_on(const WConst* wc) {
-    return !(wc->nzero | wc->far) && wc->nfar_i <= wc->lim_i && wc->nfar_j <= KS_MAX_FAR_J;
+    return !(wc->nzero | wc->far | wc->far_i) && wc->nfar_i <= wc->lim_i && wc->nfar_j <= KS_MAX_FAR_J;
 }
 
 __global__ __launch_bounds__(64) void k_wprep(const double* __restrict__ dv_prev, int P, WConst* __restrict__ wc, int lim_i) {
@@ -91,7 +92,7 @@
         __syncthreads();
     }
     if (threadIdx.x != 0) return;
-    wc->C = C; wc->nzero = nz; wc->logC = 0.0; wc->far = 0; wc->nfar_i = 0; wc->nfar_j = 0; wc->lim_i = lim_i;
+    wc->C = C; wc->nzero = nz; wc->logC = 0.0; wc->far = 0; wc->nfar_i = 0; wc->far_i = 0; wc->nfar_j = 0; wc->lim_i = lim_i;
     wc->hb_lo = ~0ull; wc->hb_hi = 0ull;
 }
 
@@ -113,7 +114,7 @@
         const double lw = -log2(w[r]);
         hb[r] = 0.5 * nn + ((lw > W_HB_MAX) ? W_HB_MAX : lw);
     }
-    if (far) atomicOr(&wc->far, 1);
+    if (far) atomicOr(hb ? &wc->far : &wc->far_i, 1);
 }
 
 template <bool SAFE>
@@ -153,7 +154,7 @@
     ha *= 0.5;
     const int nzero = wc->nzero;
     double acc = 0.0;
-    if (nzero == 0 && wc->far == 0) {
+    if (nzero == 0 && (wc->far | wc->far_i) == 0) {
         for (unsigned j = j0; j < j1; j++) {
             const double* bj = b + (size_t)j * PP;
             double bc[PP];
@@ -395,7 +396,7 @@
             if (!(lw >= KS_LW_MIN && lw <= KS_LW_CAP)) far = true;
         }
     }
-    if (rfar2k && inrange && g == 0) atomicOr(&wc->far, 1);
+    if (rfar2k && inrange && g == 0) atomicOr(is_prev ? &wc->far : &wc->far_i, 1);
     if (valid) far = far || rfar8 || !(nrow <= KS_NORM2);
     if (far) {
         if (g == 0) {
@@ -1234,15 +1235,10 @@
     return ABC_OK;
 }
 
-int launch_weights_raw(abc_ctx* ctx, const abc_prior* priors, const double* theta, size_t K, size_t P, size_t k0,
-                       size_t kn, const double* theta_prev, size_t Kp, const double* w_prev, const double* dv_prev,
-                       double* w_raw, const abc_wprev* prev, const double** sumsq_out) {
-    if (sumsq_out) *sumsq_out = nullptr;
-    if (P > (size_t)W_MAXP) ABC_FAIL(ctx, ABC_ERR_UNSUPPORTED, "weights: P = %zu > %d parameters", P, W_MAXP);
-    if (kn == 0) return ABC_OK;
-    ABC_TRY(abc_kde_words(ctx));
-    if (Kp > 0xffffffffull) ABC_FAIL(ctx, ABC_ERR_UNSUPPORTED, "weights: K' = %zu >= 2^32", Kp);
-    if (k0 + kn > K) ABC_FAIL(ctx, ABC_ERR_INVALID, "weights: row range [%zu,%zu) outside K=%zu", k0, k0 + kn, K);
+namespace {
+struct WPlan { int PP; size_t rb, slices; int NCH; bool epan, split; size_t nbt, nat; int opa; bool fold; };
+WPlan w_plan(const abc_ctx* ctx, size_t P, size_t kn, size_t Kp) {
+    WPlan q;
     int PP = 2;
     while (PP < (int)P) PP *= 2;
     if (P > 64) PP = (int)((P + 63) / 64 * 64);
@@ -1254,42 +1250,63 @@
     const int NCH = ks_chunks(P);
     const bool epan = ctx->weight_kernel == ABC_WEIGHT_EPANECHNIKOV;
     const bool split = (PP >= 8 && P <= 64 && ctx->kde_mode != ABC_KDE_FP64 && !epan);
-    const size_t nbt = (Kp + 31) / 32, nat = rb * 8;
-    const int opa = NCH * KS_NL;
-    const bool fold = ks_fold_on(P, split);
     if (split) {
         size_t cap = 12288 / rb;
         if (cap < 8) cap = 8;
         if (slices > cap) slices = cap;
     }
-    abc_wprev own;
-    if (!prev || !prev->ready) {
-        ABC_TRY(launch_weights_prev(ctx, P, kn, theta_prev, Kp, w_prev, dv_prev, &own, nullptr));
-        prev = &own;
-    }
-    if (prev->Kp != Kp || prev->P != P || prev->kn_max < kn || (prev->split != 0) != split)
-        ABC_FAIL(ctx, ABC_ERR_INVALID, "weights: the prepared previous set does not match this call");
-    WConst* wc = (WConst*)prev->wc;
-    double* b = prev->b;
-    double* hb = prev->hb;
-    unsigned short* bt = prev->bt;
-    unsigned* far_list = prev->far_list;
-    double* a = (double*)abc_ws_alloc(ctx, kn * PP * sizeof(double));
-    double* part = (double*)abc_ws_alloc(ctx, slices * kn * sizeof(double));
-    unsigned short* at = nullptr;
-    unsigned char* far_flag = nullptr;
-    double *fix_i = nullptr, *fix_j = nullptr, *ha_frac = nullptr;
-    int* ha_int = nullptr;
-    if (split) {
-        at = (unsigned short*)abc_ws_alloc(ctx, nat * opa * 1024);
-        far_flag = (unsigned char*)abc_ws_alloc(ctx, nat * 32);
-        fix_i = (double*)abc_ws_alloc(ctx, kn * sizeof(double));
-        fix_j = (double*)abc_ws_alloc(ctx, kn * sizeof(double));
-        ha_frac = (double*)abc_ws_alloc(ctx, nat * 32 * sizeof(double));
-        ha_int = (int*)abc_ws_alloc(ctx, nat * 32 * sizeof(int));
-        if (!at || !far_flag || !fix_i || !fix_j || !ha_frac || !ha_int) ABC_FAIL(ctx, ABC_ERR_NOMEM, "weights: workspace exhausted");
-    }
-    if (!a || !part) ABC_FAIL(ctx, ABC_ERR_NOMEM, "weights: workspace exhausted");
+    q.PP = PP; q.rb = rb; q.slices = slices; q.NCH = NCH; q.epan = epan; q.split = split;
+    q.nbt = (Kp + 31) / 32; q.nat = rb * 8; q.opa = NCH * KS_NL; q.fold = ks_fold_on(P, split);
+    return q;
+}
+}
+
+int launch_weights_tiles(abc_ctx* ctx, const double* theta, size_t K, size_t P, size_t k0, size_t kn, const double* theta_prev,
+                         size_t Kp, const double* w_prev, const double* dv_prev, const abc_wprev* prev, abc_wtiles* t) {
+    if (P > (size_t)W_MAXP) ABC_FAIL(ctx, ABC_ERR_UNSUPPORTED, "weights: P = %zu > %d parameters", P, W_MAXP);
+    if (kn == 0) return ABC_OK;
+    ABC_TRY(abc_kde_words(ctx));
+    if (Kp > 0xffffffffull) ABC_FAIL(ctx, ABC_ERR_UNSUPPORTED, "weights: K' = %zu >= 2^32", Kp);
+    if (k0 + kn > K) ABC_FAIL(ctx, ABC_ERR_INVALID, "weights: row range [%zu,%zu) outside K=%zu", k0, k0 + kn, K);
+    const WPlan q = w_plan(ctx, P, kn, Kp);
+    const int PP = q.PP, NCH = q.NCH, opa = q.opa;
+    const size_t slices = q.slices, nat = q.nat;
+    const bool split = q.split, fold = q.fold;
+    if (!t->ready) {
+        memset(t, 0, sizeof(*t));
+        if (!prev || !prev->ready) ABC_TRY(launch_weights_prev(ctx, P, kn, theta_prev, Kp, w_prev, dv_prev, &t->prev, nullptr));
+        else t->prev = *prev;
+        prev = &t->prev;
+        if (prev->Kp != Kp || prev->P != P || prev->kn_max < kn || (prev->split != 0) != split)
+            ABC_FAIL(ctx, ABC_ERR_INVALID, "weights: the prepared previous set does not match this call");
+        t->a = (double*)abc_ws_alloc(ctx, kn * PP * sizeof(double));
+        t->part = (double*)abc_ws_alloc(ctx, slices * kn * sizeof(double));
+        if (split) {
+            t->at = (unsigned short*)abc_ws_alloc(ctx, nat * opa * 1024);
+            t->far_flag = (unsigned char*)abc_ws_alloc(ctx, nat * 32);
+            t->fix_i = (double*)abc_ws_alloc(ctx, kn * sizeof(double));
+            t->fix_j = (double*)abc_ws_alloc(ctx, kn * sizeof(double));
+            t->ha_frac = (double*)abc_ws_alloc(ctx, nat * 32 * sizeof(double));
+            t->ha_int = (int*)abc_ws_alloc(ctx, nat * 32 * sizeof(int));
+            if (!t->at || !t->far_flag || !t->fix_i || !t->fix_j || !t->ha_frac || !t->ha_int)
+                ABC_FAIL(ctx, ABC_ERR_NOMEM, "weights: workspace exhausted");
+        }
+        if (!t->a || !t->part) ABC_FAIL(ctx, ABC_ERR_NOMEM, "weights: workspace exhausted");
+        t->K = K; t->P = P; t->k0 = k0; t->kn = kn; t->Kp = Kp;
+        t->ready = 1;
+    } else {
+        if (t->K != K || t->P != P || t->k0 != k0 || t->kn != kn || t->Kp != Kp)
+            ABC_FAIL(ctx, ABC_ERR_INVALID, "weights: the prepared tiles do not match this call");
+        static_assert(offsetof(WConst, far_i) == offsetof(WConst, nfar_i) + sizeof(int), "the new rows' words are adjacent");
+        ABC_HIP(ctx, hipMemsetAsync((char*)t->prev.wc + offsetof(WConst, nfar_i), 0, 2 * sizeof(int), ctx->stream));
+    }
+    WConst* wc = (WConst*)t->prev.wc;
+    unsigned* far_list = t->prev.far_list;
+    double* a = t->a;
+    unsigned short* at = t->at;
+    unsigned char* far_flag = t->far_flag;
+    double* ha_frac = t->ha_frac;
+    int* ha_int = t->ha_int;
     const double* centre = (const double*)((const char*)wc + offsetof(WConst, centre));
     StageTimer tm(ctx, ST_WEIGHTS_MISC);
     if (split) {
@@ -1310,6 +1327,34 @@
         hipLaunchKernelGGL(k_wscale, dim3((unsigned)((kn + 255) / 256)), dim3(256), 0, ctx->stream, theta + k0, kn, K,
                            (int)P, PP, wc, centre, (size_t)1, (const double*)nullptr, a, (double*)nullptr);
     }
+    ABC_HIP(ctx, hipGetLastError());
+    return ABC_OK;
+}
+
+int launch_weights_sums(abc_ctx* ctx, const abc_prior* priors, const double* theta, size_t K, size_t P, size_t k0, size_t kn,
+                        const double* theta_prev, size_t Kp, const double* w_prev, double* w_raw, const abc_wtiles* t,
+                        const double** sumsq_out) {
+    if (sumsq_out) *sumsq_out = nullptr;
+    if (kn == 0) return ABC_OK;
+    if (!t->ready || t->K != K || t->P != P || t->k0 != k0 || t->kn != kn || t->Kp != Kp)
+        ABC_FAIL(ctx, ABC_ERR_INVALID, "weights: the prepared tiles do not match this call");
+    const WPlan q = w_plan(ctx, P, kn, Kp);
+    const int PP = q.PP, NCH = q.NCH;
+    const size_t rb = q.rb, slices = q.slices, nat = q.nat, nbt = q.nbt;
+    const bool split = q.split, fold = q.fold, epan = q.epan;
+    const abc_wprev* prev = &t->prev;
+    WConst* wc = (WConst*)prev->wc;
+    double* b = prev->b;
+    double* hb = prev->hb;
+    unsigned short* bt = prev->bt;
+    unsigned* far_list = prev->far_list;
+    double* a = t->a;
+    double* part = t->part;
+    unsigned short* at = t->at;
+    unsigned char* far_flag = t->far_flag;
+    double *fix_i = t->fix_i, *fix_j = t->fix_j, *ha_frac = t->ha_frac;
+    int* ha_int = t->ha_int;
+    StageTimer tm(ctx, ST_WEIGHTS_MISC);
 #define LAUNCH_KDE(PPV)                                                                                        \
     hipLaunchKernelGGL(k_kde<PPV>, dim3((unsigned)rb, (unsigned)slices), dim3(256), 0, ctx->stream, a, kn, b, \
                        Kp, hb, wc, theta, K, k0, theta_prev, part, split ? 1 : 0)
@@ -1407,6 +1452,18 @@
     return ABC_OK;
 }
 
+int launch_weights_raw(abc_ctx* ctx, const abc_prior* priors, const double* theta, size_t K, size_t P, size_t k0,
+                       size_t kn, const double* theta_prev, size_t Kp, const double* w_prev, const double* dv_prev,
+                       double* w_raw, const abc_wprev* prev, const double** sumsq_out) {
+    if (sumsq_out) *sumsq_out = nullptr;
+    if (P > (size_t)W_MAXP) ABC_FAIL(ctx, ABC_ERR_UNSUPPORTED, "weights: P = %zu > %d parameters", P, W_MAXP);
+    if (kn == 0) return ABC_OK;
+    abc_wtiles t;
+    t.ready = 0;
+    ABC_TRY(launch_weights_tiles(ctx, theta, K, P, k0, kn, theta_prev, Kp, w_prev, dv_prev, prev, &t));
+    return launch_weights_sums(ctx, priors, theta, K, P, k0, kn, theta_prev, Kp, w_prev, w_raw, &t, sumsq_out);
+}
+
 int abc_kde_words(abc_ctx* ctx) {
     if (ctx->kde_which) return ABC_OK;
     ABC_HIP(ctx, hipMalloc((void**)&ctx->kde_which, 2 * sizeof(int)));
@@ -1417,6 +1474,30 @@
 int launch_fill(abc_ctx* ctx, double* w, size_t K, double v, hipStream_t st) {
     if (!K) return ABC_OK;
     hipLaunchKernelGGL(k_fill, dim3((unsigned)((K + 255) / 256)), dim3(256), 0, st ? st : ctx->stream, w, K, v);
+    ABC_HIP(ctx, hipGetLastError());
+    return ABC_OK;
+}
+
+int launch_normalize_l2_defer(abc_ctx* ctx, double* w, size_t K, const double* sumsq_parts, abc_norm_pending* out) {
+    out->w = nullptr;
+    if (!K || !sumsq_parts) return ABC_OK;
+    const unsigned fb = (unsigned)((K + 63) / 64);
+    double* sq_part = const_cast<double*>(sumsq_parts);
+    if (fb <= SQ_INLINE_MAX) { out->sq = sq_part; out->nparts = fb; }
+    else {
+        StageTimer tm(ctx, ST_WEIGHTS_MISC);
+        hipLaunchKernelGGL(k_sumsq_total, dim3(1), dim3(256), 0, ctx->stream, sq_part, fb, sq_part + fb);
+        ABC_HIP(ctx, hipGetLastError());
+        out->sq = sq_part + fb; out->nparts = 0u;
+    }
+    out->w = w; out->K = K;
+    return ABC_OK;
+}
+int launch_normalize_l2_apply(abc_ctx* ctx, const abc_norm_pending* np) {
+    if (!np->w || !np->K) return ABC_OK;
+    StageTimer tm(ctx, ST_WEIGHTS_MISC);
+    hipLaunchKernelGGL(k_div_norm, dim3((unsigned)((np->K + 255) / 256)), dim3(256), 0, ctx->stream, np->w, np->K, np->sq, np->nparts,
+                       (double*)nullptr);
     ABC_HIP(ctx, hipGetLastError());
     return ABC_OK;
 }
```
